# Costava/heightmap-ray-marcher

Hardware: AMD Instinct MI355X
Metric: ray-steps/s at 3840x2160, 4096^2 heightmap (higher is better)
Workload: dtype f64; 1 GPU; C3: 4096x4096 heightmap, 3840x2160, spherical hfov 180, step_dist 0.25, grid_width 1; ray_steps_per_frame=1197030646, rays_per_frame=8294400, hits_per_frame=1006074, parallelism=1 GPU, launches back to back on one stream

## Files before the change

### heightmap-ray-marcher_amd/__init__.py

```python
from .lib import (
    Camera, Config, HmrmError, Scene, SceneParams, Stats,
    Ray, RayHit, TraceParams, SegmentParams, Sun, CellMapParams, CellRect, MAP_TOWARDS_POINT, MAP_WEIGHT, MAP_DIFFUSE, MAP_NO_SHADOWS, RAY_END, TRACE_INTERIOR, SHADE_DIFFUSE, SHADE_NO_SHADOWS, RAY_DTYPE, RAY_HIT_DTYPE, RAY_MISS, RAY_HIT, RAY_CAPPED, MAX_RAYS, as_rays,
    PERSPECTIVE, SPHERICAL, ORTHOGRAPHIC, NEAREST, BILINEAR, NEAREST_F32,
    HMRM_OK, HMRM_E_ARG, HMRM_E_IO, HMRM_E_IMAGE, HMRM_E_CONFIG, HMRM_E_DEVICE, HMRM_E_NOTERM,
    EXPORTED_SYMBOLS, LIB_PATH, NO_PROBE, AA_FACTORS, aa_flags,
    band_local_rows, debug_frame, degrees_to_rads, device_count, image_load, image_load_memory, kernel_src_sha,
    last_error, mip_layout, level_state, calibrate, pick_kernel, plan_order, rcp_error, orbit_camera, orbit_frame_owner, png_encode, record_orbit, record_orbit_multi, record_orbit_shaded, shade_flags, map_flags, render_multi, set_device, write_png, write_ppm,
)
from . import synth
```

### heightmap-ray-marcher_amd/csrc/api.cpp

```cpp
#include <hip/hip_runtime_api.h>

#include <algorithm>
#include <cmath>
#include <cstddef>
#include <cstdio>
#include <cstdlib>
#include <cstring>
#include <fstream>
#include <mutex>
#include <new>
#include <sstream>
#include <string>
#include <vector>

#include "../../include/hmrm.h"
#include "config.hpp"
#include "frame.hpp"
#include "host_pool.hpp"
#include "image_io.hpp"
#include "launch_order.hpp"
#include "render.hpp"

namespace {

thread_local std::string g_error;
thread_local double g_last_kernel_ms = -1.0;

int fail(int code, const std::string &msg) {
	g_error = msg;
	return code;
}

}

namespace hmrm {
int set_error(int code, const char *msg) { return fail(code, msg ? msg : ""); }
}

namespace {

#define HIP_TRY(expr)                                                                         \
	do {                                                                                      \
		hipError_t e_ = (expr);                                                               \
		if (e_ != hipSuccess)                                                                 \
			return fail(HMRM_E_DEVICE, std::string(#expr) + ": " + hipGetErrorString(e_));    \
	} while (0)

struct Knobs {
	int64_t step_cap = (int64_t)1 << 26;
	int kernel = 0;
	bool tile_order = true;
	int order_mode = 2;
	int diag_mode = 0;
	int min_level = -1;
	int finest_pause = -1;
	bool order_verbose = false;
	bool try_group = true;
	int min_plane_shift = 0;
	int seg_n = 0;
	int seg_b[3] = {0, 0, 0}, seg_c[3] = {0, 0, 0};
};

Knobs read_knobs() {
	Knobs k;
	if (const char *s = getenv("HMRM_STEP_CAP")) {
		const long long v = atoll(s);
		if (v > 0) k.step_cap = v > 0x7fffffffLL ? 0x7fffffffLL : (int64_t)v;
	}
	if (const char *s = getenv("HMRM_KERNEL")) k.kernel = strcmp(s, "simple") == 0 ? 2 : (strcmp(s, "group") == 0 ? 1 : (strcmp(s, "rec") == 0 ? 3 : 0));
	if (const char *s = getenv("HMRM_TILE_ORDER")) {
		k.tile_order = s[0] != '0';
		if (s[0] == '1' || s[0] == '2') k.order_mode = s[0] - '0';
	}
	if (const char *s = getenv("HMRM_DIAG_ITERS")) k.diag_mode = atoi(s);
	if (const char *s = getenv("HMRM_ORDER_VERBOSE")) k.order_verbose = s[0] == '1';
	if (const char *s = getenv("HMRM_TRY_GROUP")) k.try_group = s[0] != '0';
	if (const char *s = getenv("HMRM_TILE_SEGMENTS")) {
		int b = 0, c = 0, used = 0;
		while (k.seg_n < 3 && sscanf(s, "%d:%d%n", &b, &c, &used) == 2 && b >= 0 && c > 0) {
			k.seg_b[k.seg_n] = b;
			k.seg_c[k.seg_n] = c;
			++k.seg_n;
			s += used;
			if (*s != ',') break;
			++s;
		}
	}
	if (const char *s = getenv("HMRM_DEBUG_PLANE_SHIFT")) {
		const int v = atoi(s);
		if (v > 0 && v <= 28) k.min_plane_shift = v;
	}
	if (const char *s = getenv("HMRM_MIN_LEVEL"))
		if (s[0] >= '0' && s[0] < '0' + hmrm::kMipLevels) k.min_level = s[0] - '0';
	if (const char *s = getenv("HMRM_FINEST_PAUSE"))
		if (s[0] >= '0' && s[0] <= '9') k.finest_pause = s[0] - '0';
	return k;
}

}

using hmrm::kCostRows;
constexpr int kFrameSlots = 64;
constexpr int kMaxMeasRows = 512;
constexpr int kProbeAfterFrames = 6;
constexpr int kMaxStreamCtx = 32;

struct FrameSlot {
	bool valid = false;
	uint64_t stamp = 0;
	hmrm_camera cam{};
	hmrm_scene_params params{};
	uint64_t thr_max_bits = 0;
	hmrm::DevFrame frame{};
	std::vector<float> row_cost;
	double *d_tables = nullptr;
	double *h_tables = nullptr;
	hipEvent_t uploaded = nullptr;
	hmrm::OrderCalibration cal;
	int meas_rows = 0;
	hipEvent_t measured = nullptr;
};

struct StreamCtx {
	hipStream_t stream = nullptr;
	bool scene_owned = false;
	uint64_t stamp = 0;
	FrameSlot slots[kFrameSlots];
	double *d_arena = nullptr, *h_arena = nullptr;
	double *h_arena_dev = nullptr;
	unsigned long long *d_meas = nullptr, *h_meas = nullptr, *h_meas_dev = nullptr;
	FrameSlot *meas_owner = nullptr;
	size_t arena_n = 0;
	unsigned long long *d_counters = nullptr;
	bool probe_in_flight = false;
	unsigned long long capped_seen = 0;
};

struct RingFrame {
	StreamCtx *ctx = nullptr;
	uint32_t *d_frame = nullptr;
	uint8_t *h_frame = nullptr;
	unsigned long long *h_capped = nullptr;
	size_t px = 0;
	int32_t width = 0, height = 0;
	hipEvent_t kernel_done = nullptr, copy_done = nullptr;
	bool busy = false;
};
constexpr int kMaxRing = 64;
constexpr int kLanes = 3;
struct DevTicket {
	StreamCtx *ctx = nullptr;
	hipEvent_t done = nullptr;
	unsigned long long *h_capped = nullptr;
	bool busy = false;
};

struct hmrm_scene {
	int device = 0;
	int32_t map_w = 0, map_h = 0;
	hmrm_scene_params params{};
	Knobs knobs;
	uint8_t *d_rgb = nullptr;
	uint32_t *d_cmap = nullptr;
	double *d_thr = nullptr;
	float *d_thr32 = nullptr;
	double thr_max = 0.0;
	double thr_max_bil = 0.0;
	bool bil_valid = false;
	bool records_valid = false;
	float *d_mipbuf_bil = nullptr;
	float *d_mipbuf = nullptr;
	hmrm::WindowRecord *d_records = nullptr;
	int32_t mip_w[hmrm::kMipLevels] = {}, mip_h[hmrm::kMipLevels] = {};
	int32_t mip_row = 0, mip_plane_shift = 0;
	size_t mip_floats() const { return (size_t)(hmrm::kMipLevels + 1) << mip_plane_shift; }
	float *plane(float *buf, int l) const { return buf + ((size_t)l << mip_plane_shift); }
	hipStream_t stream = nullptr;
	hipStream_t copy_stream = nullptr;
	hipStream_t lanes[kLanes] = {};
	uint32_t lane_next = 0;
	std::vector<RingFrame *> ring;
	std::vector<DevTicket *> dev_tickets;
	hipEvent_t ev0 = nullptr, ev1 = nullptr;
	unsigned long long *d_maxkey = nullptr;
	uint32_t *d_frame = nullptr;
	size_t frame_px = 0;
	uint8_t *h_stage = nullptr;
	size_t h_stage_bytes = 0;
	uint32_t *d_steps = nullptr;
	double *d_entry = nullptr;
	size_t stats_px = 0;
	hmrm::BatchRay *d_rays = nullptr;
	hmrm::BatchHit *d_hits = nullptr;
	size_t batch_cap = 0;
	uint32_t *d_limits = nullptr;
	size_t limits_cap = 0;
	uint8_t *d_cells = nullptr;
	size_t cells_cap = 0;
	std::mutex mu;
	std::vector<StreamCtx *> ctxs;
	uint64_t clock = 0;
	struct SettledOrder {
		hmrm_camera cam;
		hmrm_scene_params params;
		uint64_t thr_max_bits;
		hmrm::OrderTrial order;
	};
	hmrm::KernelChoice choice;
	bool probe_pending = false;
	uint32_t probe_epoch = 0, probe_epoch_launched = 0;
	int probe_rows = 0;
	StreamCtx *probe_ctx = nullptr;
	hipEvent_t probe_done = nullptr;
	unsigned long long *h_probe = nullptr, *h_probe_dev = nullptr;
	hipEvent_t measure_fence = nullptr;
	StreamCtx *measure_fence_ctx = nullptr;
	std::vector<SettledOrder> settled;
};

static_assert(sizeof(hmrm_ray) == sizeof(hmrm::BatchRay) && sizeof(hmrm_ray_hit) == sizeof(hmrm::BatchHit) &&
                  offsetof(hmrm_ray_hit, entry_d) == offsetof(hmrm::BatchHit, entry_d) &&
                  offsetof(hmrm_ray_hit, steps) == offsetof(hmrm::BatchHit, steps) &&
                  offsetof(hmrm_ray_hit, rgba) == offsetof(hmrm::BatchHit, rgba) &&
                  offsetof(hmrm_ray_hit, status) == offsetof(hmrm::BatchHit, status) && sizeof(hmrm_trace_params) == 16 &&
                  sizeof(hmrm_segment_params) == 24 && offsetof(hmrm_segment_params, flags) == 12 &&
                  offsetof(hmrm_segment_params, max_steps) == 16 && offsetof(hmrm_segment_params, reserved) == 20,
              "the kernels' mirrors of hmrm_ray / hmrm_ray_hit (frame.hpp)");
static_assert(sizeof(hmrm_cell_map_params) == 56 && offsetof(hmrm_cell_map_params, max_steps) == 40 &&
                  offsetof(hmrm_cell_map_params, sampling) == 48 && sizeof(hmrm_cell_rect) == 16 &&
                  HMRM_MAP_TOWARDS_POINT == hmrm::kMapTowardsPoint && HMRM_MAP_WEIGHT == hmrm::kMapWeight &&
                  HMRM_MAP_DIFFUSE == hmrm::kMapDiffuse && HMRM_MAP_NO_SHADOWS == hmrm::kMapNoShadows,
              "hmrm_cell_map_params and the kernels' flag bits (frame.hpp CellRules)");
static_assert(sizeof(hmrm_sun) == 48, "hmrm_sun has padding");
static_assert(sizeof(hmrm_camera) == 3 * sizeof(int32_t) + 4 + 8 * sizeof(double), "hmrm_camera has padding");
static_assert(sizeof(hmrm_scene_params) == 6 * sizeof(double), "hmrm_scene_params has padding");

struct hmrm_config {
	hmrm::Config cfg;
	std::string log_cache, warn_cache;
};

namespace {

void destroy_ctx(StreamCtx *c) {
	if (!c) return;
	for (FrameSlot &sl : c->slots) {
		if (sl.uploaded) (void)hipEventDestroy(sl.uploaded);
		if (sl.measured) (void)hipEventDestroy(sl.measured);
	}
	if (c->d_meas) (void)hipFree(c->d_meas);
	if (c->h_meas) (void)hipHostFree(c->h_meas);
	if (c->d_arena) (void)hipFree(c->d_arena);
	if (c->h_arena) (void)hipHostFree(c->h_arena);
	if (c->d_counters) (void)hipFree(c->d_counters);
	delete c;
}

int ctx_for(hmrm_scene *s, hipStream_t stream, StreamCtx **out) {
	for (StreamCtx *c : s->ctxs)
		if (c->stream == stream) {
			c->stamp = ++s->clock;
			*out = c;
			return HMRM_OK;
		}
	if ((int)s->ctxs.size() >= kMaxStreamCtx) {
		size_t victim = 0;
		for (size_t i = 1; i < s->ctxs.size(); ++i)
			if (!s->ctxs[i]->scene_owned && (victim == 0 || s->ctxs[i]->stamp < s->ctxs[victim]->stamp)) victim = i;
		if (victim == 0) return fail(HMRM_E_ARG, "too many streams");
		(void)hipDeviceSynchronize();
		if (s->probe_ctx == s->ctxs[victim]) s->probe_ctx = nullptr;
		if (s->measure_fence_ctx == s->ctxs[victim]) s->measure_fence_ctx = nullptr;
		destroy_ctx(s->ctxs[victim]);
		s->ctxs.erase(s->ctxs.begin() + (long)victim);
	}
	StreamCtx *c = new (std::nothrow) StreamCtx();
	if (!c) return fail(HMRM_E_ARG, "out of memory");
	c->stream = stream;
	c->scene_owned = stream == s->stream;
	for (hipStream_t lane : s->lanes) c->scene_owned = c->scene_owned || (lane && stream == lane);
	c->stamp = ++s->clock;
	hipError_t e = hipMalloc((void **)&c->d_counters, 16 * sizeof(unsigned long long));
	if (e == hipSuccess) e = hipMemsetAsync(c->d_counters, 0, 16 * sizeof(unsigned long long), s->stream);
	if (e == hipSuccess) e = hipStreamSynchronize(s->stream);
	if (e != hipSuccess) {
		destroy_ctx(c);
		return fail(HMRM_E_DEVICE, std::string("stream context: ") + hipGetErrorString(e));
	}
	s->ctxs.push_back(c);
	*out = c;
	return HMRM_OK;
}

int check_camera(const hmrm_camera *cam) {
	if (!cam) return fail(HMRM_E_ARG, "camera is NULL");
	if (cam->width <= 0 || cam->height <= 0) return fail(HMRM_E_ARG, "resolution must be positive");
	if ((int64_t)cam->width * cam->height > ((int64_t)1 << 31) / 4)
		return fail(HMRM_E_ARG, "resolution too large (the reference indexes the framebuffer with int)");
	if (cam->projection < 1 || cam->projection > 3) return fail(HMRM_E_ARG, "projection must be 1, 2 or 3");
	if (cam->sampling > HMRM_NEAREST_F32) return fail(HMRM_E_ARG, "sampling must be 0 (nearest), 1 (bilinear) or 2 (nearest, float heights)");
	return HMRM_OK;
}

int check_antialias(const hmrm_camera *cam, int32_t factor, hmrm_camera *super, int *shift) {
	const int sh = factor == 1 ? 0 : factor == 2 ? 1 : factor == 4 ? 2 : factor == 8 ? 3 : -1;
	if (sh < 0) return fail(HMRM_E_ARG, "antialias factor must be 1, 2, 4 or 8 (got " + std::to_string(factor) + ")");
	if ((int64_t)cam->width * cam->height * ((int64_t)1 << (2 * sh)) > ((int64_t)1 << 31) / 4)
		return fail(HMRM_E_ARG, "antialias: the " + std::to_string(factor) + "x super frame has more than 2^29 samples (the reference "
		                        "indexes the framebuffer with int)");
	*super = *cam;
	super->width = cam->width << sh;
	super->height = cam->height << sh;
	*shift = sh;
	return HMRM_OK;
}

int antialias_of_flags(uint32_t flags, int32_t *factor) {
	if (flags & ~(HMRM_NO_PROBE | HMRM_AA_MASK))
		return fail(HMRM_E_ARG, "flags: unknown bits (defined: HMRM_NO_PROBE and the antialias factor HMRM_AA(n))");
	const int32_t n = (int32_t)((flags & HMRM_AA_MASK) >> 8);
	*factor = n == 0 ? 1 : n;
	return HMRM_OK;
}

int ensure_bilinear_pyramid(hmrm_scene *s);
int ensure_records(hmrm_scene *s);

void to_host_camera(const hmrm_camera *cam, hmrm::HostCamera *hc) {
	*hc = hmrm::HostCamera{};
	hc->width = cam->width;
	hc->height = cam->height;
	hc->projection = cam->projection;
	hc->bg_r = cam->bg_r;
	hc->bg_g = cam->bg_g;
// ... 41 lines not shown
				for (FrameSlot &sl : c->slots) {
					if (sl.cam.projection == HMRM_SPHERICAL) sl.valid = false;
					sl.d_tables = sl.h_tables = nullptr;
				}
				const size_t per = (n + 31) & ~(size_t)31;
				HIP_TRY(hipMalloc((void **)&c->d_arena, per * kFrameSlots * sizeof(double)));
				HIP_TRY(hipHostMalloc((void **)&c->h_arena, per * kFrameSlots * sizeof(double), hipHostMallocMapped));
				HIP_TRY(hipHostGetDevicePointer((void **)&c->h_arena_dev, c->h_arena, 0));
				c->arena_n = per;
			}
			const size_t idx = (size_t)(slot - c->slots);
			slot->d_tables = c->d_arena + idx * c->arena_n;
			slot->h_tables = c->h_arena + idx * c->arena_n;
			if (!slot->uploaded) HIP_TRY(hipEventCreateWithFlags(&slot->uploaded, hipEventDisableTiming));
			else HIP_TRY(hipEventSynchronize(slot->uploaded));
			cc = slot->h_tables;
			cs = cc + W;
			rs = cs + W;
			rc = rs + H;
		}
		hmrm::DevFrame &fr = slot->frame;
		hmrm::build_frame(hc, s->map_w, s->map_h, s->params.min_height, s->params.max_height, s->params.grid_width,
		                  &fr, nullptr, nullptr, nullptr, nullptr);
		if (cam->projection == HMRM_SPHERICAL) {
			const FrameSlot *row_donor = nullptr, *col_donor = nullptr;
			for (const FrameSlot &o : c->slots) {
				if (!o.valid || &o == slot || o.cam.projection != HMRM_SPHERICAL || !o.h_tables) continue;
				if (o.cam.width != cam->width || o.cam.hfov != cam->hfov) continue;
				if (!col_donor && o.cam.hang == cam->hang) col_donor = &o;
				if (!row_donor && o.cam.height == cam->height && o.cam.vang == cam->vang) row_donor = &o;
			}
			if (col_donor) memcpy(cc, col_donor->h_tables, 2 * W * sizeof(double));
			if (row_donor) memcpy(rs, row_donor->h_tables + 2 * (size_t)row_donor->cam.width, 2 * H * sizeof(double));
			const int nc = col_donor ? 0 : cam->width, nr = row_donor ? 0 : cam->height;
			if (nc + nr > 0)
				hmrm::parallel_ranges(nc + nr, 1024, [&](int b, int e) {
					if (b < nc) hmrm::fill_col_tables(hc, b, std::min(e, nc), cc, cs);
					if (e > nc) hmrm::fill_row_tables(hc, std::max(b, nc) - nc, e - nc, rs, rc);
				});
		}
		slot->row_cost.assign(((size_t)cam->height + kCostRows - 1) / kCostRows, 0.0f);
		hmrm::estimate_row_costs(fr, cc, cs, rs, rc, kCostRows, slot->row_cost.data());
		if (cam->projection == HMRM_SPHERICAL) {
			HIP_TRY(hmrm::launch_upload_tables(c->h_arena_dev + (slot->h_tables - c->h_arena), slot->d_tables, 2 * W + 2 * H, c->stream));
			HIP_TRY(hipEventRecord(slot->uploaded, c->stream));
			fr.col_cos_ha = slot->d_tables;
			fr.col_sin_ha = slot->d_tables + W;
			fr.row_sin_va = slot->d_tables + 2 * W;
			fr.row_cos_va = slot->d_tables + 2 * W + H;
		}
		if (cam->sampling == HMRM_BILINEAR) {
			const int rc2 = ensure_bilinear_pyramid(s);
			if (rc2 != HMRM_OK) return rc2;
		}
		fr.thr_max = cam->sampling == HMRM_BILINEAR ? s->thr_max_bil : s->thr_max;
		fr.min_level = 0;
		while (fr.min_level < hmrm::kMipLevels - 1 && hmrm::win_cells(fr.min_level) < fr.min_window)
			++fr.min_level;
		fr.mipbuf = s->d_mipbuf;
		fr.mipbuf_bil = s->d_mipbuf_bil;
		fr.mip_row = s->mip_row;
		fr.mip_plane_shift = s->mip_plane_shift;
		slot->cam = *cam;
		slot->params = s->params;
		slot->thr_max_bits = thr_bits;
		slot->valid = true;
		for (size_t k = s->settled.size(); k-- > 0;) {
			const hmrm_scene::SettledOrder &so = s->settled[k];
			if (memcmp(&so.cam, cam, sizeof *cam) != 0 || memcmp(&so.params, &s->params, sizeof s->params) != 0 || so.thr_max_bits != thr_bits) continue;
			slot->cal.adopt(so.order);
			break;
		}
	}
	slot->stamp = ++s->clock;
	*f = slot->frame;
	f->step_cap = s->knobs.step_cap;
	f->diag_mode = s->knobs.diag_mode;
	if (s->knobs.min_level >= 0) f->min_level = s->knobs.min_level;
	if (s->knobs.finest_pause >= 0) f->finest_pause = s->knobs.finest_pause;
	if (slot_out) *slot_out = slot;
	return HMRM_OK;
}

int ensure_meas(StreamCtx *c) {
	if (!c->d_meas) HIP_TRY(hipMalloc((void **)&c->d_meas, (size_t)kMaxMeasRows * hmrm::kMeasureStride * sizeof(unsigned long long)));
	if (!c->h_meas) {
		const size_t n = (size_t)kFrameSlots * 2 * kMaxMeasRows * sizeof(unsigned long long);
		HIP_TRY(hipHostMalloc((void **)&c->h_meas, n, hipHostMallocMapped));
		HIP_TRY(hipHostGetDevicePointer((void **)&c->h_meas_dev, c->h_meas, 0));
	}
	return HMRM_OK;
}

bool others_idle(hmrm_scene *s, StreamCtx *c) {
	for (StreamCtx *o : s->ctxs) {
		if (o == c || !o->scene_owned) continue;
		const hipError_t e = hipStreamQuery(o->stream);
		if (e == hipSuccess) continue;
		if (e == hipErrorNotReady) (void)hipGetLastError();
		return false;
	}
	return true;
}

int wait_for_measure_fence(hmrm_scene *s, StreamCtx *c) {
	if (!s->measure_fence_ctx || s->measure_fence_ctx == c) return HMRM_OK;
	if (hipEventQuery(s->measure_fence) == hipSuccess) s->measure_fence_ctx = nullptr;
	else HIP_TRY(hipStreamWaitEvent(c->stream, s->measure_fence, 0));
	return HMRM_OK;
}

int raise_measure_fence(hmrm_scene *s, StreamCtx *c) {
	if (!s->measure_fence) HIP_TRY(hipEventCreateWithFlags(&s->measure_fence, hipEventDisableTiming));
	HIP_TRY(hipEventRecord(s->measure_fence, c->stream));
	s->measure_fence_ctx = c;
	return HMRM_OK;
}

void poll_measured(hmrm_scene *s, StreamCtx *c, FrameSlot *slot, int tiles_y, int rot) {
	if (slot->cal.in_flight >= 0 && slot->meas_rows == tiles_y && hipEventQuery(slot->measured) == hipSuccess) {
		const int trial = slot->cal.in_flight;
		const unsigned long long *h_rec = c->h_meas + (size_t)(slot - c->slots) * 2 * kMaxMeasRows;
		const bool settled = slot->cal.on_measured(h_rec, tiles_y, rot, s->knobs.kernel == 0 && s->knobs.try_group, s->choice);
		if (s->knobs.order_verbose) {
			const hmrm::OrderTrial &t = slot->cal.trials[trial];
			fprintf(stderr, "hmrm order: trial %d of %d tile rows measured, makespan %.1f us:", trial, tiles_y, t.makespan / 100.0);
			for (int k = 0; k < t.n; ++k) fprintf(stderr, " [%d,%d)", t.b[k], t.b[k] + t.c[k]);
			fprintf(stderr, "%s\n", t.group ? " plain groups, rotation" : (t.n ? "" : " rotation"));
			if (settled) fprintf(stderr, "hmrm order: settled on trial %d\n", slot->cal.best);
		}
		if (settled) {
			if (s->settled.size() >= 256) s->settled.erase(s->settled.begin());
			s->settled.push_back(hmrm_scene::SettledOrder{slot->cam, slot->params, slot->thr_max_bits, slot->cal.trials[slot->cal.best]});
		}
	}
	if (c->meas_owner && (c->meas_owner->cal.in_flight < 0 || hipEventQuery(c->meas_owner->measured) == hipSuccess)) c->meas_owner = nullptr;
}

void poll_shadow_probe(hmrm_scene *s) {
	if (!s->probe_pending || hipEventQuery(s->probe_done) != hipSuccess) return;
	s->probe_pending = false;
	if (s->probe_ctx) s->probe_ctx->probe_in_flight = false;
	if (s->probe_epoch_launched != s->probe_epoch) return;
	hmrm::fold_shadow_probe(s->choice, s->h_probe, s->h_probe + 2 * kMaxMeasRows, s->probe_rows);
	if (s->knobs.order_verbose)
		fprintf(stderr, "hmrm probe: production kernel %.1f us, the other kernel %.1f us -> %s\n", hmrm::measured_makespan(s->h_probe, s->probe_rows) / 100.0,
		        hmrm::measured_makespan(s->h_probe + 2 * kMaxMeasRows, s->probe_rows) / 100.0, s->choice.use_group ? (s->choice.with_records ? "groups + window records" : "plain groups") : "production kernel");
}

int launch_shadow_probe(hmrm_scene *s, StreamCtx *c, const hmrm::DevFrame &f, const hmrm::RowMap &rows_in_order, int tiles_y,
                        uint32_t *d_out, int64_t out_stride_px) {
	if (!s->h_probe) {
		HIP_TRY(hipHostMalloc((void **)&s->h_probe, (size_t)4 * kMaxMeasRows * sizeof(unsigned long long), hipHostMallocMapped));
		HIP_TRY(hipHostGetDevicePointer((void **)&s->h_probe_dev, s->h_probe, 0));
		HIP_TRY(hipEventCreateWithFlags(&s->probe_done, hipEventDisableTiming));
	}
	const int rc_m = ensure_meas(c);
	if (rc_m) return rc_m;
	hmrm::RowMap measured = rows_in_order;
	measured.measure = c->d_meas;
	const bool records_ok = f.sampling == 0 && s->d_records;
	s->choice.with_records = records_ok;
	if (records_ok) {
		const int rc_r = ensure_records(s);
		if (rc_r) return rc_r;
	}
	for (int pass = 0; pass < 2; ++pass) {
		HIP_TRY(hmrm::launch_measure_init(measured.measure, tiles_y, c->stream));
		HIP_TRY(hmrm::launch_render_fast(f, measured, s->d_thr, s->d_thr32, s->d_cmap, d_out, out_stride_px,
		                                 c->d_counters + (pass ? 8 : 0), nullptr, nullptr, false,
		                                 pass == 0 ? hmrm::kLeaps : (records_ok ? hmrm::kRecords : hmrm::kPlainGroups), s->d_records, c->stream));
		HIP_TRY(hmrm::launch_measure_readback(measured.measure, s->h_probe_dev + (size_t)pass * 2 * kMaxMeasRows, tiles_y, c->stream));
	}
	HIP_TRY(hipEventRecord(s->probe_done, c->stream));
	s->probe_pending = true;
	s->choice.probed = true;
	s->probe_rows = tiles_y;
	s->probe_epoch_launched = s->probe_epoch;
	s->probe_ctx = c;
	c->probe_in_flight = true;
	return raise_measure_fence(s, c);
}

struct LitFrame {
	hmrm::SunRules sun;
	bool primary_interior;
	uint32_t shade_flags;
};
hmrm::SunRules shade_sun(const LitFrame &lit) {
	hmrm::SunRules sun = lit.sun;
	if (!(lit.shade_flags & HMRM_SHADE_DIFFUSE)) sun.ambient = 255u;
	return sun;
}
int launch_kernel(hmrm_scene *s, StreamCtx *c, const hmrm::DevFrame &f, const hmrm::RowMap &rows_in_order, uint32_t *d_out,
                  int64_t out_stride_px, uint32_t *d_steps, double *d_entry, bool stats, bool use_group, bool interior = false,
                  const LitFrame *lit = nullptr) {
	const bool huge_side = s->map_w >= (1 << 24) || s->map_h >= (1 << 24);
	if (huge_side && f.sampling != 0)
		return fail(HMRM_E_ARG, "maps with a side of 2^24 cells or more support nearest sampling only");
	if ((s->knobs.kernel == 2 || huge_side) && f.sampling == 0) {
		if (lit && lit->shade_flags) {
			const bool shadows = !(lit->shade_flags & HMRM_SHADE_NO_SHADOWS);
			if (f.aa_shift) {
				HIP_TRY(hmrm::launch_render_shaded_literal_aa(f, rows_in_order, s->d_thr, s->d_cmap, d_out, out_stride_px, c->d_counters,
				                                              shadows ? lit->sun : shade_sun(*lit), lit->primary_interior, shadows, c->stream));
				return HMRM_OK;
			}
			HIP_TRY(hmrm::launch_render_shaded_literal(f, rows_in_order, s->d_thr, s->d_cmap, d_out, out_stride_px, c->d_counters,
			                                           shadows ? lit->sun : shade_sun(*lit), lit->primary_interior, shadows, c->stream));
			return HMRM_OK;
		}
		if (lit && f.aa_shift) {
			HIP_TRY(hmrm::launch_render_lit_literal_aa(f, rows_in_order, s->d_thr, s->d_cmap, d_out, out_stride_px, c->d_counters, lit->sun,
			                                           lit->primary_interior, c->stream));
			return HMRM_OK;
		}
		if (lit) {
			HIP_TRY(hmrm::launch_render_lit_literal(f, rows_in_order, s->d_thr, s->d_cmap, d_out, out_stride_px, c->d_counters, lit->sun,
			                                        lit->primary_interior, c->stream));
			return HMRM_OK;
		}
		if (interior) {
			HIP_TRY(hmrm::launch_render_interior_literal(f, rows_in_order, s->d_thr, s->d_cmap, d_out, out_stride_px, c->d_counters, c->stream));
			return HMRM_OK;
		}
		HIP_TRY(hmrm::launch_render(f, rows_in_order, s->d_thr, s->d_cmap, d_out, out_stride_px, c->d_counters, d_steps,
		                            d_entry, stats, c->stream));
	} else {
		const hmrm::FastKernel k = (hmrm::FastKernel)hmrm::pick_fast_kernel(s->knobs.kernel, use_group, f.sampling == 0 && s->d_records, s->choice);
		if (k == hmrm::kRecords) {
			const int rc_r = ensure_records(s);
			if (rc_r) return rc_r;
		}
		if (lit && f.aa_shift) {
			const auto launch = (lit->shade_flags & HMRM_SHADE_NO_SHADOWS) ? hmrm::launch_render_shaded_aa
			                    : lit->shade_flags                         ? hmrm::launch_render_lit_shaded_aa
			                                                               : hmrm::launch_render_lit_aa;
			HIP_TRY(launch(f, rows_in_order, s->d_thr, s->d_thr32, s->d_cmap, d_out, out_stride_px, c->d_counters, k, s->d_records,
			               (lit->shade_flags & HMRM_SHADE_NO_SHADOWS) ? shade_sun(*lit) : lit->sun, lit->primary_interior, c->stream));
			return HMRM_OK;
		}
		if (lit && (lit->shade_flags & HMRM_SHADE_NO_SHADOWS)) {
			HIP_TRY(hmrm::launch_render_shaded(f, rows_in_order, s->d_thr, s->d_thr32, s->d_cmap, d_out, out_stride_px, c->d_counters, k,
			                                   s->d_records, shade_sun(*lit), lit->primary_interior, c->stream));
			return HMRM_OK;
		}
		if (lit && lit->shade_flags) {
			HIP_TRY(hmrm::launch_render_lit_shaded(f, rows_in_order, s->d_thr, s->d_thr32, s->d_cmap, d_out, out_stride_px, c->d_counters, k,
			                                       s->d_records, lit->sun, lit->primary_interior, c->stream));
			return HMRM_OK;
		}
		if (lit) {
			HIP_TRY(hmrm::launch_render_lit(f, rows_in_order, s->d_thr, s->d_thr32, s->d_cmap, d_out, out_stride_px, c->d_counters, k,
			                                s->d_records, lit->sun, lit->primary_interior, c->stream));
			return HMRM_OK;
		}
		if (interior) {
			HIP_TRY(hmrm::launch_render_interior(f, rows_in_order, s->d_thr, s->d_thr32, s->d_cmap, d_out, out_stride_px, c->d_counters, k,
			                                     s->d_records, c->stream));
			return HMRM_OK;
		}
		HIP_TRY(hmrm::launch_render_fast(f, rows_in_order, s->d_thr, s->d_thr32, s->d_cmap, d_out, out_stride_px,
		                                 c->d_counters, d_steps, d_entry, stats, k, s->d_records, c->stream));
	}
	return HMRM_OK;
}

int launch_maybe_measured(hmrm_scene *s, StreamCtx *c, const hmrm::DevFrame &f, FrameSlot *slot, hmrm::RowMap &rows_in_order, int tiles_y,
                          bool measure_now, uint32_t *d_out, int64_t out_stride_px, uint32_t *d_steps, double *d_entry, bool stats, bool use_group,
                          bool interior = false, const LitFrame *lit = nullptr) {
	if (measure_now) {
		const int rc_m = ensure_meas(c);
		if (rc_m) return rc_m;
		if (!slot->measured) HIP_TRY(hipEventCreateWithFlags(&slot->measured, hipEventDisableTiming));
		rows_in_order.measure = c->d_meas;
		HIP_TRY(hmrm::launch_measure_init(rows_in_order.measure, tiles_y, c->stream));
	}
	const int rc_k = launch_kernel(s, c, f, rows_in_order, d_out, out_stride_px, d_steps, d_entry, stats, use_group, interior, lit);
	if (rc_k || !measure_now) return rc_k;
	const size_t idx = (size_t)(slot - c->slots);
	HIP_TRY(hmrm::launch_measure_readback(rows_in_order.measure, c->h_meas_dev + idx * 2 * kMaxMeasRows, tiles_y, c->stream));
	HIP_TRY(hipEventRecord(slot->measured, c->stream));
	slot->meas_rows = tiles_y;
	c->meas_owner = slot;
	return raise_measure_fence(s, c);
}

int launch_frame(hmrm_scene *s, StreamCtx *c, const hmrm::DevFrame &f, FrameSlot *slot, const hmrm::RowMap &rows,
                 uint32_t *d_out, int64_t out_stride_px, uint32_t *d_steps, double *d_entry, bool stats, bool no_probe = false,
                 int interior = 0, const LitFrame *lit = nullptr) {
	hmrm::RowMap rows_in_order = rows;
	int tile_w = 1, tile_h = 1;
	hmrm::render_tile_shape(&tile_w, &tile_h);
	const int tiles_y = (rows.local_rows + tile_h - 1) / tile_h;
	const bool pieces = s->knobs.seg_n > 0 && rows.band_rows == 0 && rows.row_begin == 0;
	const int rot = hmrm::choose_tile_rot(s->knobs.tile_order, slot->row_cost, rows, tile_h);
	const bool may_probe = !stats && !interior && !lit && s->knobs.kernel == 0 && s->knobs.try_group;
	const bool eligible = !pieces && !stats && !interior && !lit && s->knobs.tile_order && s->knobs.order_mode == 2 && s->knobs.kernel != 2 &&
	                      rows.band_rows == 0 && rows.row_begin == 0 && rows.local_rows == f.screen_h && tiles_y >= 12 &&
	                      tiles_y <= kMaxMeasRows && s->map_w < (1 << 24) && s->map_h < (1 << 24);
	int rc = wait_for_measure_fence(s, c);
	if (rc) return rc;
	poll_shadow_probe(s);
	hmrm::OrderTrial order;
	if (pieces) {
		order.n = s->knobs.seg_n;
		for (int k = 0; k < 3; ++k) { order.b[k] = s->knobs.seg_b[k]; order.c[k] = s->knobs.seg_c[k]; }
	}
	bool use_group = may_probe && s->choice.use_group;
	if (interior || lit) use_group = s->knobs.kernel == 0 && s->knobs.try_group && s->choice.use_group;
	bool measure_now = false;
	if (eligible) {
		poll_measured(s, c, slot, tiles_y, rot);
		const bool probe_open = may_probe && !no_probe && !s->choice.probed && !s->probe_pending;
		const bool quiet = (slot->cal.wants_measure() || probe_open) && c->meas_owner == nullptr && !c->probe_in_flight && others_idle(s, c);
		const hmrm::LaunchPlan p = slot->cal.plan(quiet, s->choice);
		order = slot->cal.trials[p.trial];
		use_group = p.use_group;
		measure_now = p.measure;
		if (!measure_now && probe_open && quiet && slot->cal.in_flight < 0 && ++s->choice.unprobed_frames >= (unsigned)kProbeAfterFrames) {
			hmrm::set_tile_order(&rows_in_order, tiles_y, rot, order.n, order.b, order.c);
			return launch_shadow_probe(s, c, f, rows_in_order, tiles_y, d_out, out_stride_px);
		}
	}
	hmrm::set_tile_order(&rows_in_order, tiles_y, rot, order.n, order.b, order.c);
	if ((rc = launch_maybe_measured(s, c, f, slot, rows_in_order, tiles_y, measure_now, d_out, out_stride_px, d_steps, d_entry, stats, use_group, interior == 2, lit))) {
		if (measure_now) slot->cal.drop_in_flight();
		return rc;
	}
	return HMRM_OK;
}

bool mip_layout(int32_t map_w, int32_t map_h, int32_t *mip_w, int32_t *mip_h, int32_t *mip_row, int32_t *plane_shift, int32_t min_shift = 0) {
	for (int l = 0; l < hmrm::kMipLevels; ++l) {
		const int stride = 1 << hmrm::mip_stride_shift(l);
		mip_w[l] = (map_w + stride - 1) / stride;
		mip_h[l] = (map_h + stride - 1) / stride;
	}
	*mip_row = mip_w[0];
	*plane_shift = min_shift;
	while (((size_t)1 << *plane_shift) < (size_t)hmrm::mip_index(mip_w[0] - 1, mip_h[0] - 1, *mip_row) + 1) ++*plane_shift;
	return ((uint64_t)(hmrm::kMipLevels + 1) << *plane_shift) <= ((uint64_t)1 << 30);
}

int next_lane(hmrm_scene *s, StreamCtx **out) {
	const uint32_t i = s->lane_next++ % kLanes;
	if (!s->lanes[i]) HIP_TRY(hipStreamCreateWithFlags(&s->lanes[i], hipStreamNonBlocking));
	return ctx_for(s, s->lanes[i], out);
}

int ensure_frame(hmrm_scene *s, size_t px) {
	if (px <= s->frame_px) return HMRM_OK;
	if (s->d_frame) (void)hipFree(s->d_frame);
	s->d_frame = nullptr;
	s->frame_px = 0;
	HIP_TRY(hipMalloc((void **)&s->d_frame, px * sizeof(uint32_t)));
	s->frame_px = px;
	return HMRM_OK;
}

int ensure_stats(hmrm_scene *s, size_t px) {
	if (px <= s->stats_px) return HMRM_OK;
	if (s->d_steps) (void)hipFree(s->d_steps);
	if (s->d_entry) (void)hipFree(s->d_entry);
	s->d_steps = nullptr;
	s->d_entry = nullptr;
	s->stats_px = 0;
	HIP_TRY(hipMalloc((void **)&s->d_steps, px * sizeof(uint32_t)));
	HIP_TRY(hipMalloc((void **)&s->d_entry, px * sizeof(double)));
	s->stats_px = px;
	return HMRM_OK;
}

int ensure_records(hmrm_scene *s) {
	if (s->records_valid) return HMRM_OK;
	if (!s->d_records) return fail(HMRM_E_ARG, "this scene has no window records");
	HIP_TRY(hmrm::launch_build_records(s->d_thr, s->map_w, s->map_h, s->d_records, s->stream));
	HIP_TRY(hipStreamSynchronize(s->stream));
	s->records_valid = true;
	return HMRM_OK;
}

int ensure_bilinear_pyramid(hmrm_scene *s) {
	if (s->bil_valid) return HMRM_OK;
	const int64_t n = (int64_t)s->map_w * s->map_h;
	if (!s->d_mipbuf_bil) HIP_TRY(hipMalloc((void **)&s->d_mipbuf_bil, s->mip_floats() * sizeof(float)));
	double *tmp = nullptr;
	HIP_TRY(hipMalloc((void **)&tmp, (size_t)n * sizeof(double)));
	hipError_t e = hmrm::launch_dilate3x3(s->d_thr, s->map_w, s->map_h, tmp, s->stream);
	if (e == hipSuccess)
		e = hmrm::launch_build_mip0(tmp, s->map_w, s->map_h, s->plane(s->d_mipbuf_bil, 0), s->mip_w[0], s->mip_h[0],
		                            s->mip_row, s->stream);
	for (int l = 1; l < hmrm::kMipLevels && e == hipSuccess; ++l)
		e = hmrm::launch_build_mip_up(s->plane(s->d_mipbuf_bil, l - 1), s->mip_w[l - 1], s->mip_h[l - 1],
		                              s->plane(s->d_mipbuf_bil, l), s->mip_w[l], s->mip_h[l], s->mip_row, l - 1, s->stream);
	const int top = hmrm::kMipLevels - 1;
	const size_t top_span = (size_t)hmrm::mip_index(s->mip_w[top] - 1, s->mip_h[top] - 1, s->mip_row) + 1;
	std::vector<float> coarse(top_span);
	if (e == hipSuccess)
		e = hipMemcpyAsync(coarse.data(), s->plane(s->d_mipbuf_bil, top), top_span * sizeof(float), hipMemcpyDeviceToHost, s->stream);
	if (e == hipSuccess) e = hipStreamSynchronize(s->stream);
	(void)hipFree(tmp);
	if (e != hipSuccess) return fail(HMRM_E_DEVICE, std::string("bilinear pyramid: ") + hipGetErrorString(e));
	float m = -__builtin_huge_valf();
	for (int iy = 0; iy < s->mip_h[top]; ++iy)
		for (int ix = 0; ix < s->mip_w[top]; ++ix) {
			const float v = coarse[hmrm::mip_index(ix, iy, s->mip_row)];
			if (v > m) m = v;
		}
	e = hipMemcpyAsync(s->plane(s->d_mipbuf_bil, hmrm::kMipLevels), &m, sizeof m, hipMemcpyHostToDevice, s->stream);
	if (e == hipSuccess) e = hipStreamSynchronize(s->stream);
	if (e != hipSuccess) return fail(HMRM_E_DEVICE, std::string("bilinear pyramid: ") + hipGetErrorString(e));
	s->thr_max_bil = (double)m;
	s->bil_valid = true;
	return HMRM_OK;
}

int run_update_heights(hmrm_scene *s) {
	const int64_t n = (int64_t)s->map_w * s->map_h;
	for (StreamCtx *c : s->ctxs)
		if (c->scene_owned && c->stream != s->stream) HIP_TRY(hipStreamSynchronize(c->stream));
	if (s->copy_stream) HIP_TRY(hipStreamSynchronize(s->copy_stream));
	HIP_TRY(hipMemsetAsync(s->d_maxkey, 0, sizeof(unsigned long long), s->stream));
	HIP_TRY(hmrm::launch_prepare_heights(s->d_rgb, s->d_thr, n, s->params.lum_r, s->params.lum_g,
	                                     s->params.lum_b, s->params.min_height, s->params.max_height,
	                                     false, s->d_maxkey, s->stream));
	HIP_TRY(hmrm::launch_thr_to_float(s->d_thr, s->d_thr32, n, s->stream));
	HIP_TRY(hmrm::launch_build_mip0(s->d_thr, s->map_w, s->map_h, s->plane(s->d_mipbuf, 0), s->mip_w[0], s->mip_h[0],
	                                s->mip_row, s->stream));
	for (int l = 1; l < hmrm::kMipLevels; ++l)
		HIP_TRY(hmrm::launch_build_mip_up(s->plane(s->d_mipbuf, l - 1), s->mip_w[l - 1], s->mip_h[l - 1],
		                                  s->plane(s->d_mipbuf, l), s->mip_w[l], s->mip_h[l], s->mip_row, l - 1, s->stream));
	s->bil_valid = false;
	s->records_valid = false;
	for (StreamCtx *c : s->ctxs)
		for (FrameSlot &sl : c->slots) sl.valid = false;
	s->settled.clear();
	s->choice.reset();
	++s->probe_epoch;
	unsigned long long key = 0;
	HIP_TRY(hipMemcpyAsync(&key, s->d_maxkey, sizeof key, hipMemcpyDeviceToHost, s->stream));
	HIP_TRY(hipStreamSynchronize(s->stream));
	s->thr_max = key ? hmrm::max_key_to_double(key) : -__builtin_huge_val();
	const float top = hmrm::round_up_to_float_host(s->thr_max);
	HIP_TRY(hipMemcpyAsync(s->plane(s->d_mipbuf, hmrm::kMipLevels), &top, sizeof top, hipMemcpyHostToDevice, s->stream));
	HIP_TRY(hipStreamSynchronize(s->stream));
	return HMRM_OK;
}

constexpr int64_t kMaxBatch = (int64_t)1 << 29;
int noterm(unsigned long long capped);

int check_trace(const hmrm_trace_params *p, const void *rays, int64_t n, const void *hits) {
	if (n < 0) return fail(HMRM_E_ARG, "trace: n must not be negative (got " + std::to_string(n) + ")");
	if (n > kMaxBatch) return fail(HMRM_E_ARG, "trace: at most 2^29 rays per batch (got " + std::to_string(n) + ")");
	if (n > 0 && (!p || !rays || !hits)) return fail(HMRM_E_ARG, "trace: NULL params, rays or hits");
	if (p && p->sampling > HMRM_NEAREST_F32)
		return fail(HMRM_E_ARG, "trace: sampling must be 0 (nearest), 1 (bilinear) or 2 (nearest, float heights)");
	return HMRM_OK;
}

int check_segments(const hmrm_segment_params *p, const void *rays, int64_t n, const void *hits, hmrm_trace_params *plain) {
	if (p) *plain = hmrm_trace_params{p->step_dist, p->bg_r, p->bg_g, p->bg_b, p->sampling};
	const int rc = check_trace(p ? plain : nullptr, rays, n, hits);
	if (rc) return rc;
	if (p && (p->flags & ~(uint32_t)HMRM_TRACE_INTERIOR)) return fail(HMRM_E_ARG, "trace: unknown flag bits (defined: HMRM_TRACE_INTERIOR)");
	if (p && p->reserved != 0u) return fail(HMRM_E_ARG, "trace: hmrm_segment_params.reserved must be 0");
	return HMRM_OK;
}

int ensure_limits(hmrm_scene *s, size_t n) {
	if (n <= s->limits_cap) return HMRM_OK;
	if (s->d_limits) (void)hipFree(s->d_limits);
	s->d_limits = nullptr;
	s->limits_cap = 0;
	HIP_TRY(hipMalloc((void **)&s->d_limits, n * sizeof(uint32_t)));
	s->limits_cap = n;
	return HMRM_OK;
}

int ensure_batch(hmrm_scene *s, size_t n) {
	if (n <= s->batch_cap) return HMRM_OK;
	if (s->d_rays) (void)hipFree(s->d_rays);
	if (s->d_hits) (void)hipFree(s->d_hits);
	s->d_rays = nullptr;
	s->d_hits = nullptr;
	s->batch_cap = 0;
	HIP_TRY(hipMalloc((void **)&s->d_rays, n * sizeof(hmrm::BatchRay)));
	HIP_TRY(hipMalloc((void **)&s->d_hits, n * sizeof(hmrm::BatchHit)));
	s->batch_cap = n;
	return HMRM_OK;
}

int cameraless_frame(hmrm_scene *s, double step_dist, int sampling, hmrm::DevFrame *out) {
	const bool huge_side = s->map_w >= (1 << 24) || s->map_h >= (1 << 24);
	if (huge_side && sampling != 0) return fail(HMRM_E_ARG, "maps with a side of 2^24 cells or more support nearest sampling only");
	if (sampling == HMRM_BILINEAR) {
		const int rc_b = ensure_bilinear_pyramid(s);
		if (rc_b) return rc_b;
	}
	hmrm::DevFrame f = hmrm::DevFrame();
	hmrm::fill_scene_fields(s->map_w, s->map_h, s->params.min_height, s->params.max_height, s->params.grid_width, step_dist, &f);
	f.bg[3] = 255;
	f.sampling = sampling;
	f.thr_max = sampling == HMRM_BILINEAR ? s->thr_max_bil : s->thr_max;
	f.mipbuf = s->d_mipbuf;
	f.mipbuf_bil = s->d_mipbuf_bil;
	f.mip_row = s->mip_row;
	f.mip_plane_shift = s->mip_plane_shift;
	f.step_cap = s->knobs.step_cap;
	f.min_window = 4;
	f.min_level = s->knobs.min_level >= 0 ? s->knobs.min_level : 0;
	f.finest_pause = s->knobs.finest_pause >= 0 ? s->knobs.finest_pause : 0;
	*out = f;
	return HMRM_OK;
}
int cameraless_kernel(hmrm_scene *s, int sampling, bool *literal, hmrm::FastKernel *k) {
	const bool huge_side = s->map_w >= (1 << 24) || s->map_h >= (1 << 24);
	*literal = (s->knobs.kernel == 2 || huge_side) && sampling == 0;
	*k = hmrm::kLeaps;
// ... 147 lines not shown
	s->params = *params;
	s->knobs = read_knobs();
	int rc = HMRM_OK;
	auto body = [&]() -> int {
		HIP_TRY(hipGetDevice(&s->device));
		HIP_TRY(hipStreamCreateWithFlags(&s->stream, hipStreamNonBlocking));
		HIP_TRY(hipStreamCreateWithFlags(&s->copy_stream, hipStreamNonBlocking));
		HIP_TRY(hipEventCreate(&s->ev0));
		HIP_TRY(hipEventCreate(&s->ev1));
		HIP_TRY(hipMalloc((void **)&s->d_rgb, n * 3));
		HIP_TRY(hipMalloc((void **)&s->d_cmap, n * 4));
		HIP_TRY(hipMalloc((void **)&s->d_thr, n * (sizeof(double) + sizeof(float))));
		s->d_thr32 = reinterpret_cast<float *>(s->d_thr + n);
		(void)mip_layout(map_w, map_h, s->mip_w, s->mip_h, &s->mip_row, &s->mip_plane_shift, s->knobs.min_plane_shift);
		HIP_TRY(hipMalloc((void **)&s->d_mipbuf, s->mip_floats() * sizeof(float)));
		if ((map_h + 3) / 4 <= 65535 * 16)
			HIP_TRY(hipMalloc((void **)&s->d_records, (size_t)hmrm::rec_row(map_w) * (size_t)((map_h + 3) / 4) * sizeof(hmrm::WindowRecord)));
		HIP_TRY(hipMalloc((void **)&s->d_maxkey, sizeof(unsigned long long)));
		HIP_TRY(hipMemcpyAsync(s->d_rgb, height_rgb, n * 3, hipMemcpyHostToDevice, s->stream));
		HIP_TRY(hipMemcpyAsync(s->d_cmap, color_rgba, n * 4, hipMemcpyHostToDevice, s->stream));
		StreamCtx *own = nullptr;
		const int rc2 = ctx_for(s, s->stream, &own);
		if (rc2) return rc2;
		return run_update_heights(s);
	};
	rc = body();
	if (rc != HMRM_OK) {
		std::string keep = g_error;
		hmrm_scene_destroy(s);
		g_error = keep;
		return rc;
	}
	*out = s;
	return HMRM_OK;
}

int hmrm_scene_update(hmrm_scene *s, const hmrm_scene_params *params) {
	if (!s || !params) return fail(HMRM_E_ARG, "NULL argument");
	HIP_TRY(hipSetDevice(s->device));
	std::lock_guard<std::mutex> lk(s->mu);
	s->params = *params;
	return run_update_heights(s);
}

void hmrm_scene_destroy(hmrm_scene *s) {
	if (!s) return;
	(void)hipSetDevice(s->device);
	for (StreamCtx *c : s->ctxs) {
		if (c->scene_owned && c->stream) (void)hipStreamSynchronize(c->stream);
		destroy_ctx(c);
	}
	s->ctxs.clear();
	if (s->copy_stream) (void)hipStreamSynchronize(s->copy_stream);
	for (RingFrame *r : s->ring) {
		if (r->d_frame) (void)hipFree(r->d_frame);
		if (r->h_frame) (void)hipHostFree(r->h_frame);
		if (r->h_capped) (void)hipHostFree(r->h_capped);
		if (r->kernel_done) (void)hipEventDestroy(r->kernel_done);
		if (r->copy_done) (void)hipEventDestroy(r->copy_done);
		delete r;
	}
	s->ring.clear();
	for (DevTicket *t : s->dev_tickets) {
		if (t->done) (void)hipEventDestroy(t->done);
		if (t->h_capped) (void)hipHostFree(t->h_capped);
		delete t;
	}
	s->dev_tickets.clear();
	for (hipStream_t &lane : s->lanes)
		if (lane) {
			(void)hipStreamDestroy(lane);
			lane = nullptr;
		}
	if (s->copy_stream) (void)hipStreamDestroy(s->copy_stream);
	if (s->d_rgb) (void)hipFree(s->d_rgb);
	if (s->d_cmap) (void)hipFree(s->d_cmap);
	if (s->d_thr) (void)hipFree(s->d_thr);
	if (s->d_mipbuf) (void)hipFree(s->d_mipbuf);
	if (s->d_records) (void)hipFree(s->d_records);
	if (s->d_mipbuf_bil) (void)hipFree(s->d_mipbuf_bil);
	if (s->d_maxkey) (void)hipFree(s->d_maxkey);
	if (s->d_frame) (void)hipFree(s->d_frame);
	if (s->h_stage) (void)hipHostFree(s->h_stage);
	if (s->h_probe) (void)hipHostFree(s->h_probe);
	if (s->probe_done) (void)hipEventDestroy(s->probe_done);
	if (s->measure_fence) (void)hipEventDestroy(s->measure_fence);
	if (s->d_steps) (void)hipFree(s->d_steps);
	if (s->d_entry) (void)hipFree(s->d_entry);
	if (s->d_rays) (void)hipFree(s->d_rays);
	if (s->d_hits) (void)hipFree(s->d_hits);
	if (s->d_limits) (void)hipFree(s->d_limits);
	if (s->d_cells) (void)hipFree(s->d_cells);
	if (s->ev0) (void)hipEventDestroy(s->ev0);
	if (s->ev1) (void)hipEventDestroy(s->ev1);
	if (s->stream) (void)hipStreamDestroy(s->stream);
	delete s;
}

int hmrm_debug_kernel_choice(const hmrm_scene *s) {
	if (!s) return fail(HMRM_E_ARG, "NULL argument");
	std::lock_guard<std::mutex> lk(const_cast<hmrm_scene *>(s)->mu);
	if (s->knobs.kernel != 0) return s->knobs.kernel;
	return s->choice.use_group ? (s->choice.with_records ? 3 : 1) : 0;
}

int hmrm_debug_reload_env(hmrm_scene *s) {
	if (!s) return fail(HMRM_E_ARG, "NULL argument");
	HIP_TRY(hipSetDevice(s->device));
	std::lock_guard<std::mutex> lk(s->mu);
	s->knobs = read_knobs();
	s->settled.clear();
	s->choice.reset();
	++s->probe_epoch;
	for (StreamCtx *c : s->ctxs)
		for (FrameSlot &sl : c->slots) {
			if (sl.cal.in_flight >= 0 && sl.measured) HIP_TRY(hipEventSynchronize(sl.measured));
			sl.cal.reset();
			if (c->meas_owner == &sl) c->meas_owner = nullptr;
		}
	return HMRM_OK;
}

int hmrm_scene_read_heights(const hmrm_scene *cs, double *out) {
	hmrm_scene *s = const_cast<hmrm_scene *>(cs);
	if (!s || !out) return fail(HMRM_E_ARG, "NULL argument");
	HIP_TRY(hipSetDevice(s->device));
	const int64_t n = (int64_t)s->map_w * s->map_h;
	double *tmp = nullptr;
	HIP_TRY(hipMalloc((void **)&tmp, (size_t)n * sizeof(double)));
	hipError_t e = hmrm::launch_prepare_heights(s->d_rgb, tmp, n, s->params.lum_r, s->params.lum_g,
	                                            s->params.lum_b, s->params.min_height,
	                                            s->params.max_height, true, nullptr, s->stream);
	if (e == hipSuccess)
		e = hipMemcpyAsync(out, tmp, (size_t)n * sizeof(double), hipMemcpyDeviceToHost, s->stream);
	if (e == hipSuccess) e = hipStreamSynchronize(s->stream);
	(void)hipFree(tmp);
	if (e != hipSuccess) return fail(HMRM_E_DEVICE, std::string("read_heights: ") + hipGetErrorString(e));
	return HMRM_OK;
}

static int render_common(hmrm_scene *s, const hmrm_camera *cam, uint8_t *rgba, size_t stride_bytes,
                         hmrm_stats *stats, uint32_t *steps_pp, double *entry_d, bool want_stats, int32_t aa_factor = 1,
                         bool interior = false, const LitFrame *lit = nullptr) {
	int rc = check_camera(cam);
	if (rc) return rc;
	hmrm_camera super;
	int aa_shift = 0;
	if ((rc = check_antialias(cam, aa_factor, &super, &aa_shift))) return rc;
	if (!s || !rgba) return fail(HMRM_E_ARG, "NULL argument");
	const size_t W = (size_t)cam->width, H = (size_t)cam->height;
	if (stride_bytes < W * 4) return fail(HMRM_E_ARG, "stride_bytes < width*4");
	HIP_TRY(hipSetDevice(s->device));
	std::lock_guard<std::mutex> lk(s->mu);
	if ((rc = ensure_frame(s, W * H))) return rc;
	if (want_stats && aa_shift == 0 && (rc = ensure_stats(s, W * H))) return rc;
	StreamCtx *c = nullptr;
	if ((rc = ctx_for(s, s->stream, &c))) return rc;
	hmrm::DevFrame f;
	FrameSlot *slot = nullptr;
	if ((rc = prepare_frame(s, c, &super, &f, &slot))) return rc;
	f.aa_shift = aa_shift;
	hmrm::RowMap rows{0, super.height, 0, 0, 1, {}, {}, nullptr};
	int interior_mode = 0;
	if (interior) {
		const double *o = f.cam;
		const bool cam_inside = f.c0[0] < o[0] && o[0] < f.c1[0] && f.c1[1] < o[1] && o[1] < f.c0[1] && f.c0[2] < o[2] && o[2] < f.c1[2];
		interior_mode = (cam->projection == HMRM_ORTHOGRAPHIC || cam_inside) ? 2 : 1;
	}
	if (want_stats) {
		HIP_TRY(hipMemsetAsync(c->d_counters, 0, 2 * sizeof(unsigned long long), s->stream));
		HIP_TRY(hipMemsetAsync(c->d_counters + 4, 0, 4 * sizeof(unsigned long long), s->stream));
	}
	HIP_TRY(hipEventRecord(s->ev0, s->stream));
	const bool per_pixel = want_stats && aa_shift == 0;
	if ((rc = launch_frame(s, c, f, slot, rows, s->d_frame, (int64_t)W, per_pixel ? s->d_steps : nullptr,
	                       per_pixel ? s->d_entry : nullptr, want_stats, false, interior_mode, lit)))
		return rc;
	HIP_TRY(hipEventRecord(s->ev1, s->stream));
	HIP_TRY(hipMemcpy2DAsync(rgba, stride_bytes, s->d_frame, W * 4, W * 4, H, hipMemcpyDeviceToHost,
	                         s->stream));
	unsigned long long counters[8] = {0, 0, 0, 0, 0, 0, 0, 0};
	HIP_TRY(hipMemcpyAsync(counters, c->d_counters, sizeof counters, hipMemcpyDeviceToHost, s->stream));
	if (per_pixel && steps_pp)
		HIP_TRY(hipMemcpyAsync(steps_pp, s->d_steps, W * H * sizeof(uint32_t), hipMemcpyDeviceToHost, s->stream));
	if (per_pixel && entry_d)
		HIP_TRY(hipMemcpyAsync(entry_d, s->d_entry, W * H * sizeof(double), hipMemcpyDeviceToHost, s->stream));
	HIP_TRY(hipStreamSynchronize(s->stream));
	float ms = 0.f;
	HIP_TRY(hipEventElapsedTime(&ms, s->ev0, s->ev1));
	g_last_kernel_ms = ms;
	const unsigned long long capped = counters[2] - c->capped_seen;
	c->capped_seen = counters[2];
	if (stats) {
		stats->rays = (uint64_t)super.width * (uint64_t)super.height;
		stats->steps = counters[0];
		stats->hits = counters[1];
		stats->capped = capped;
		stats->leap_attempts = counters[4];
		stats->leaps = counters[5];
		stats->groups = counters[6];
		stats->leaped_steps = counters[7];
	}
// ... 773 lines not shown
	if (rc) return rc;
	if (!s) return fail(HMRM_E_ARG, "NULL argument");
	hmrm_cell_rect r;
	if ((rc = check_cell_rect(s, rect, stride_bytes, &r))) return rc;
	HIP_TRY(hipSetDevice(s->device));
	std::lock_guard<std::mutex> lk(s->mu);
	StreamCtx *c = nullptr;
	if ((rc = ctx_for(s, (hipStream_t)hip_stream, &c))) return rc;
	return launch_cells(s, c, p, r, static_cast<uint8_t *>(d_out), stride_bytes);
}

int hmrm_pick(const hmrm_scene *scene, const hmrm_camera *cam, int32_t px, int32_t py, hmrm_ray_hit *hit) {
	hmrm_scene *s = const_cast<hmrm_scene *>(scene);
	int rc = check_camera(cam);
	if (rc) return rc;
	if (!s || !hit) return fail(HMRM_E_ARG, "NULL argument");
	if (px < 0 || py < 0 || px >= cam->width || py >= cam->height) return fail(HMRM_E_ARG, "pixel out of range");
	HIP_TRY(hipSetDevice(s->device));
	std::lock_guard<std::mutex> lk(s->mu);
	const size_t W = (size_t)cam->width, H = (size_t)cam->height;
	const bool spherical = cam->projection == HMRM_SPHERICAL;
	if ((rc = ensure_stats(s, 8 + (spherical ? 2 * W + 2 * H : 0)))) return rc;
	if ((rc = ensure_batch(s, 1))) return rc;
	StreamCtx *c = nullptr;
	if ((rc = ctx_for(s, s->stream, &c))) return rc;
	hmrm::HostCamera hc;
	to_host_camera(cam, &hc);
	std::vector<double> tables(spherical ? 2 * W + 2 * H : 0);
	double *t = tables.data();
	hmrm::DevFrame f;
	hmrm::build_frame(hc, s->map_w, s->map_h, s->params.min_height, s->params.max_height, s->params.grid_width, &f,
	                  spherical ? t : nullptr, spherical ? t + W : nullptr, spherical ? t + 2 * W : nullptr,
	                  spherical ? t + 2 * W + H : nullptr);
	if (spherical) {
		double *d_t = s->d_entry + 8;
		HIP_TRY(hipMemcpyAsync(d_t, t, tables.size() * sizeof(double), hipMemcpyHostToDevice, s->stream));
		f.col_cos_ha = d_t;
		f.col_sin_ha = d_t + W;
		f.row_sin_va = d_t + 2 * W;
		f.row_cos_va = d_t + 2 * W + H;
	}
	HIP_TRY(hmrm::launch_probe(f, px, py, s->d_entry, s->stream));
	const uint8_t bg[3] = {cam->bg_r, cam->bg_g, cam->bg_b};
	if ((rc = launch_batch(s, c, cam->step_dist, bg, cam->sampling, reinterpret_cast<const hmrm::BatchRay *>(s->d_entry), 1, s->d_hits)))
		return rc;
	return finish_batch(s, c, hit, 1, nullptr);
}

int hmrm_debug_ray(const hmrm_scene *scene, const hmrm_camera *cam, int32_t px, int32_t py,
                   double pos[3], double dir[3], double *entry_d) {
	hmrm_scene *s = const_cast<hmrm_scene *>(scene);
	int rc = check_camera(cam);
	if (rc) return rc;
	if (!s || !pos || !dir || !entry_d) return fail(HMRM_E_ARG, "NULL argument");
	if (px < 0 || py < 0 || px >= cam->width || py >= cam->height) return fail(HMRM_E_ARG, "pixel out of range");
	HIP_TRY(hipSetDevice(s->device));
	std::lock_guard<std::mutex> lk(s->mu);
	if ((rc = ensure_stats(s, 8))) return rc;
	StreamCtx *c = nullptr;
	if ((rc = ctx_for(s, s->stream, &c))) return rc;
	hmrm::DevFrame f;
	if ((rc = prepare_frame(s, c, cam, &f, nullptr))) return rc;
	HIP_TRY(hmrm::launch_probe(f, px, py, s->d_entry, s->stream));
	double host[7];
	HIP_TRY(hipMemcpyAsync(host, s->d_entry, sizeof host, hipMemcpyDeviceToHost, s->stream));
	HIP_TRY(hipStreamSynchronize(s->stream));
	for (int i = 0; i < 3; ++i) { pos[i] = host[i]; dir[i] = host[3 + i]; }
	*entry_d = host[6];
	return HMRM_OK;
}

int hmrm_debug_plan_order(const uint64_t *records, int32_t tile_rows, int32_t rot, int32_t pieces_begin[3],
                          int32_t pieces_count[3], int32_t *tile_row_of_grid_row) {
	if (!records || !pieces_begin || !pieces_count || tile_rows <= 0 || rot < 0 || rot >= tile_rows) return fail(HMRM_E_ARG, "bad argument");
	int b[3] = {0, 0, 0}, c[3] = {0, 0, 0};
	const int n = hmrm::plan_order_from_measurement((const unsigned long long *)records, tile_rows, rot, b, c);
	for (int k = 0; k < 3; ++k) {
		pieces_begin[k] = k < n ? b[k] : 0;
		pieces_count[k] = k < n ? c[k] : 0;
	}
	if (tile_row_of_grid_row) {
		hmrm::RowMap r{};
		hmrm::set_tile_order(&r, tile_rows, rot, n, b, c);
		for (int gy = 0; gy < tile_rows; ++gy) {
			int delta = r.seg_delta[0];
			for (int k = 1; k < hmrm::kOrderSegs; ++k) delta = (unsigned)gy >= (unsigned)r.seg_first[k - 1] ? r.seg_delta[k] : delta;
			unsigned ty = (unsigned)gy + (unsigned)delta;
			if (ty >= (unsigned)tile_rows) ty -= (unsigned)tile_rows;
			tile_row_of_grid_row[gy] = (int32_t)ty;
		}
	}
	return n;
}

int hmrm_debug_rcp_error(int32_t mode, uint64_t count, uint64_t seed, int32_t exp_lo, int32_t exp_hi,
                         double *max_rel_err, uint64_t *hist64) {
	if (!max_rel_err) return fail(HMRM_E_ARG, "NULL argument");
	if (mode < 0 || mode > 2 || count == 0 || count > ((uint64_t)1 << 40) || exp_lo > exp_hi || exp_lo < -1000 || exp_hi > 1000)
		return fail(HMRM_E_ARG, "hmrm_debug_rcp_error: bad mode, count or exponent range");
	unsigned long long *d = nullptr, host[65] = {};
	HIP_TRY(hipMalloc((void **)&d, sizeof host));
	hipError_t e = hipMemset(d, 0, sizeof host);
	if (e == hipSuccess) e = hmrm::launch_rcp_error(mode, count, seed, exp_lo, exp_hi, d, nullptr);
	if (e == hipSuccess) e = hipMemcpy(host, d, sizeof host, hipMemcpyDeviceToHost);
	(void)hipFree(d);
	if (e != hipSuccess) return fail(HMRM_E_DEVICE, std::string("rcp probe: ") + hipGetErrorString(e));
	memcpy(max_rel_err, &host[0], sizeof(double));
	if (hist64)
		for (int i = 0; i < 64; ++i) hist64[i] = host[1 + i];
	return HMRM_OK;
}

int hmrm_debug_frame(const hmrm_camera *cam, const hmrm_scene_params *params, int32_t map_w,
                     int32_t map_h, double *out25, double *tables) {
	int rc = check_camera(cam);
	if (rc) return rc;
	if (!params || !out25) return fail(HMRM_E_ARG, "NULL argument");
	if (cam->projection == HMRM_SPHERICAL && !tables) return fail(HMRM_E_ARG, "tables required for spherical");
	hmrm::HostCamera hc{};
	hc.width = cam->width; hc.height = cam->height; hc.projection = cam->projection;
	hc.bg_r = cam->bg_r; hc.bg_g = cam->bg_g; hc.bg_b = cam->bg_b; hc.sampling = cam->sampling;
	hc.hfov = cam->hfov; hc.hang = cam->hang; hc.vang = cam->vang;
	hc.pos[0] = cam->pos[0]; hc.pos[1] = cam->pos[1]; hc.pos[2] = cam->pos[2];
	hc.ortho_width = cam->ortho_width; hc.step_dist = cam->step_dist;
	const size_t W = (size_t)cam->width, H = (size_t)cam->height;
	hmrm::DevFrame f;
	hmrm::build_frame(hc, map_w, map_h, params->min_height, params->max_height, params->grid_width, &f, nullptr, nullptr,
	                  nullptr, nullptr);
	if (cam->projection == HMRM_SPHERICAL) {
		double *cc = tables, *cs = tables + W, *rs = tables + 2 * W, *rc2 = tables + 2 * W + H;
		const int nc = cam->width, nr = cam->height;
		hmrm::parallel_ranges(nc + nr, 1024, [&](int b, int e) {
			if (b < nc) hmrm::fill_col_tables(hc, b, std::min(e, nc), cc, cs);
			if (e > nc) hmrm::fill_row_tables(hc, std::max(b, nc) - nc, e - nc, rs, rc2);
		});
	}
	double *o = out25;
	for (int i = 0; i < 3; ++i) *o++ = f.cam[i];
	for (int i = 0; i < 3; ++i) *o++ = f.upper_left[i];
	for (int i = 0; i < 3; ++i) *o++ = f.plane_right[i];
	for (int i = 0; i < 3; ++i) *o++ = f.plane_down[i];
	for (int i = 0; i < 3; ++i) *o++ = f.look[i];
	for (int i = 0; i < 3; ++i) *o++ = f.c0[i];
	for (int i = 0; i < 3; ++i) *o++ = f.c1[i];
	*o++ = f.nudge;
	*o++ = f.step_dist;
	*o++ = (double)f.grid_pow2;
	*o++ = f.inv_grid_width;
	return HMRM_OK;
}

int hmrm_debug_mip_layout(int32_t map_w, int32_t map_h, int32_t *mip_row, int32_t *plane_shift, int32_t *levels) {
	if (map_w <= 0 || map_h <= 0 || (int64_t)map_w * map_h > ((int64_t)1 << 31) / 4) return fail(HMRM_E_ARG, "bad map dimensions");
	int32_t w[hmrm::kMipLevels], h[hmrm::kMipLevels], row = 0, shift = 0;
	const bool fits = mip_layout(map_w, map_h, w, h, &row, &shift);
	if (mip_row) *mip_row = row;
	if (plane_shift) *plane_shift = shift;
	if (levels) *levels = hmrm::kMipLevels;
	return fits ? 1 : 0;
}

int hmrm_debug_pick_kernel(int32_t forced, int32_t use_other, int32_t records_ok, int32_t scene_verdict, int32_t scene_with_records,
                           int32_t *with_records_after) {
	hmrm::KernelChoice choice;
	choice.use_group = scene_verdict != 0;
	choice.probed = choice.use_group;
	choice.with_records = scene_with_records != 0;
	const int k = hmrm::pick_fast_kernel(forced, use_other != 0, records_ok != 0, choice);
	if (with_records_after) *with_records_after = choice.with_records ? 1 : 0;
	return k;
}

int hmrm_debug_read_records(const hmrm_scene *cs, void *records_out, double *thr_out) {
	hmrm_scene *s = const_cast<hmrm_scene *>(cs);
	if (!s) return fail(HMRM_E_ARG, "NULL argument");
	std::lock_guard<std::mutex> lk(s->mu);
	HIP_TRY(hipSetDevice(s->device));
	HIP_TRY(hipStreamSynchronize(s->stream));
	if (records_out) {
		if (!s->d_records) return fail(HMRM_E_ARG, "this scene has no window records (map too tall)");
		const int rc_r = ensure_records(s);
		if (rc_r) return rc_r;
		HIP_TRY(hipMemcpy(records_out, s->d_records, (size_t)hmrm::rec_row(s->map_w) * (size_t)((s->map_h + 3) / 4) * sizeof(hmrm::WindowRecord),
		                  hipMemcpyDeviceToHost));
	}
	if (thr_out) HIP_TRY(hipMemcpy(thr_out, s->d_thr, (size_t)s->map_w * (size_t)s->map_h * sizeof(double), hipMemcpyDeviceToHost));
	return HMRM_OK;
}

int hmrm_debug_level_state(int32_t level, int32_t young, int32_t min_level, int32_t out[8]) {
	if (!out || level < 0 || level > hmrm::kMipLevels || min_level < 0 || min_level >= hmrm::kMipLevels)
		return fail(HMRM_E_ARG, "hmrm_debug_level_state: bad argument");
	const uint32_t b = (uint32_t)(hmrm::level_state_table() >> (8 * level)) & 0xffu;
	const int hs = (int)(b & 31u), back = (int)(b >> 5);
	const int lstep = hmrm::level_step(young ? 0 : -1);
	out[0] = hs;
	out[1] = back;
	out[2] = (back + 1) << hs;
	out[3] = lstep;
	out[4] = hmrm::level_coarser(level, lstep);
	out[5] = hmrm::level_finer(level, lstep, min_level);
	out[6] = level == min_level ? 1 : 0;
	out[7] = (int32_t)b;
	return hmrm::kMipLevels;
}

int hmrm_debug_calibrate(const uint64_t *records, int32_t launches, int32_t tile_rows, int32_t rot, int32_t may_probe,
                         int32_t scene_already_probed, const uint8_t *can_measure, int32_t *trial_used, int32_t *measured,
                         int32_t *group_kernel, int32_t *n_trials, int32_t *best, int32_t *scene_use_group, int32_t *settled_at_launch) {
	if (!records || launches <= 0 || tile_rows <= 0 || tile_rows > kMaxMeasRows || rot < 0 || rot >= tile_rows)
		return fail(HMRM_E_ARG, "hmrm_debug_calibrate: bad argument");
	hmrm::OrderCalibration cal;
	hmrm::KernelChoice choice;
	choice.probed = scene_already_probed != 0;
	int settled_at = -1;
	for (int32_t i = 0; i < launches; ++i) {
		const hmrm::LaunchPlan p = cal.plan(!can_measure || can_measure[i] != 0, choice);
		if (trial_used) trial_used[i] = p.trial;
		if (measured) measured[i] = p.measure ? 1 : 0;
		if (group_kernel) group_kernel[i] = p.use_group ? 1 : 0;
		if (p.measure && cal.on_measured((const unsigned long long *)records + (size_t)i * 2 * (size_t)tile_rows, tile_rows, rot, may_probe != 0, choice))
			settled_at = i;
	}
	if (n_trials) *n_trials = cal.n_trials;
	if (best) *best = cal.best;
	if (scene_use_group) *scene_use_group = choice.use_group ? 1 : 0;
	if (settled_at_launch) *settled_at_launch = settled_at;
	return HMRM_OK;
}

int32_t hmrm_band_local_rows(int32_t height, int32_t band_rows, int32_t band_index, int32_t band_count) {
	if (height <= 0 || band_rows <= 0 || band_count <= 0 || band_index < 0 || band_index >= band_count) return 0;
	int64_t local = 0;
	for (int64_t b = band_index; b * band_rows < height; b += band_count) local += band_rows;
	return (int32_t)local;
}

}

namespace hmrm {
int check_shaded_args(const hmrm_sun *sun, uint32_t shade_flags) { return check_shaded(sun, shade_flags); }
}
```

### heightmap-ray-marcher_amd/csrc/device_common.hpp

```cpp
#pragma once
#include <hip/hip_runtime.h>
#include <stdint.h>

#include "frame.hpp"

#pragma clang fp contract(off)

namespace hmrm {

struct DevRay {
	double px, py, pz;
	double dx, dy, dz;
};

template <int PROJ>
__device__ __forceinline__ DevRay make_ray(const DevFrame &f, int px, int py) {
	DevRay r;
	if (PROJ == 2) {
		const double sva = f.row_sin_va[py], cva = f.row_cos_va[py];
		const double cha = f.col_cos_ha[px], sha = f.col_sin_ha[px];
		r.px = f.cam[0]; r.py = f.cam[1]; r.pz = f.cam[2];
		r.dx = sva * cha;
		r.dy = sva * sha;
		r.dz = cva;
// ... 200 lines not shown
	if (PROJ == 1 || PROJ == 2) {
#pragma unroll
		for (int i = 0; i < 3; ++i) {
			if (!f.box_side_known[i]) continue;
			const uint32_t hd = (uint32_t)((unsigned long long)__double_as_longlong(rd[i]) >> 32);
			away = away | ((((hd >> 20) & 0x7ffu) - 523u) < 1000u & ((f.box_side[i] ^ hd) >> 31) != 0u);
		}
		return away;
	}
#pragma unroll
	for (int i = 0; i < 3; ++i) {
		const uint32_t h0 = (uint32_t)((unsigned long long)__double_as_longlong(f.c0[i] - ro[i]) >> 32);
		const uint32_t h1 = (uint32_t)((unsigned long long)__double_as_longlong(f.c1[i] - ro[i]) >> 32);
		const uint32_t hd = (uint32_t)((unsigned long long)__double_as_longlong(rd[i]) >> 32);
		const bool moderate = (((h0 >> 20) & 0x7ffu) - 523u) < 1000u && (((h1 >> 20) & 0x7ffu) - 523u) < 1000u &&
		                      (((hd >> 20) & 0x7ffu) - 523u) < 1000u;
		away = away || (moderate && ((h0 ^ h1) >> 31) == 0u && ((h0 ^ hd) >> 31) != 0u);
	}
	return away;
}

__device__ __forceinline__ uint32_t pack_rgba(uint32_t r, uint32_t g, uint32_t b) {
	return r | (g << 8) | (b << 16) | 0xff000000u;
}

__device__ __forceinline__ uint32_t sky_channel_literal(double v) {
	if (v < 0.0) v = 0.0;
	else if (v > 255.0) v = 255.0;
	return (uint32_t)(int)__builtin_floor(v);
}
__device__ __forceinline__ uint32_t sky_channel(double v) {
	return (uint32_t)__builtin_fmin(v, 255.0);
}

struct StatsOut {
	unsigned long long *counters;
	uint32_t *steps_per_pixel;
	double *entry_d;
};


__device__ __forceinline__ uint32_t shade_miss(const DevFrame &f, double dz) {
	if (dz > 0.0) {
		const double zz = dz * dz;
		const double r_ = 220.0 * zz + (double)f.bg[0];
		const double g_ = 240.0 * zz + (double)f.bg[1];
		const double b_ = 255.0 * dz + (double)f.bg[2];
		return pack_rgba(sky_channel(r_), sky_channel(g_), sky_channel(b_));
	}
	return pack_rgba(f.bg[0], f.bg[1], f.bg[2]);
}

__device__ __forceinline__ uint32_t shade_hit(const DevFrame &f, uint32_t texel) {
	return ((texel >> 24) == 0) ? pack_rgba(f.bg[0], f.bg[1], f.bg[2]) : (texel | 0xff000000u);
}

#ifndef HMRM_WAVE_W
#define HMRM_WAVE_W 8
#endif
#ifndef HMRM_WAVES_X
#define HMRM_WAVES_X 1
#endif
#ifndef HMRM_WAVES_Y
#define HMRM_WAVES_Y 2
#endif
constexpr int kWaveW = HMRM_WAVE_W, kWaveH = 64 / HMRM_WAVE_W;
constexpr int kWavesX = HMRM_WAVES_X, kWavesY = HMRM_WAVES_Y;
constexpr int kBlockThreads = 64 * kWavesX * kWavesY;
constexpr int kTileW = kWavesX * kWaveW, kTileH = kWavesY * kWaveH;
static_assert(kBatchW == kWaveW, "a wave's 64 lanes hold 64 consecutive rays of a batch (frame.hpp RayBatch)");
struct PixelId {
	int px, py, lrow;
	int tile_y;
	bool live;
};
__device__ __forceinline__ int frame_row_of(const RowMap &rows, int lrow) {
	if (rows.band_rows > 0) {
		const int band = lrow / rows.band_rows, within = lrow - band * rows.band_rows;
		return (rows.band_index + band * rows.band_count) * rows.band_rows + within;
	}
	return rows.row_begin + lrow;
}

__device__ __forceinline__ PixelId pixel_of_tile_lane(const DevFrame &f, const RowMap &rows, int tiles_y, int tile_x, unsigned gy,
                                                      int wave, int lane) {
	const bool row_exists = gy < (unsigned)tiles_y;
	int delta = rows.seg_delta[0];
#pragma unroll
	for (int k = 1; k < kOrderSegs; ++k) delta = gy >= (unsigned)rows.seg_first[k - 1] ? rows.seg_delta[k] : delta;
	unsigned ty = gy + (unsigned)delta;
	if (ty >= (unsigned)tiles_y) ty -= (unsigned)tiles_y;
	const int tile_y = (int)ty;
	PixelId p;
	p.tile_y = row_exists ? tile_y : -1;
	p.px = tile_x * kTileW + (wave % kWavesX) * kWaveW + (lane % kWaveW);
	p.lrow = tile_y * kTileH + (wave / kWavesX) * kWaveH + (lane / kWaveW);
	p.py = frame_row_of(rows, p.lrow);
	p.live = row_exists && p.px < f.screen_w && p.lrow < rows.local_rows && p.py < f.screen_h;
	return p;
}
__device__ __forceinline__ PixelId pixel_of_lane(const DevFrame &f, const RowMap &rows, int tiles_y) {
	return pixel_of_tile_lane(f, rows, tiles_y, (int)blockIdx.x, blockIdx.z * 32768u + blockIdx.y, (int)(threadIdx.x >> 6),
	                          (int)(threadIdx.x & 63));
}

template <bool STATS>
__device__ __forceinline__ void publish_counters(const StatsOut &st, unsigned long long steps,
                                                 uint32_t hit, uint32_t cap) {
	if (STATS) {
		unsigned long long s = steps, h = hit, c = cap;
		for (int off = 32; off > 0; off >>= 1) {
			s += __shfl_xor(s, off);
			h += __shfl_xor(h, off);
			c += __shfl_xor(c, off);
		}
		if ((threadIdx.x & 63) == 0) {
			if (s) atomicAdd(&st.counters[0], s);
			if (h) atomicAdd(&st.counters[1], h);
			if (c) atomicAdd(&st.counters[2], c);
		}
	} else if (cap) {
		atomicAdd(&st.counters[2], 1ull);
	}
}

__device__ __forceinline__ void store_box_filtered(uint32_t *__restrict__ out, int64_t out_stride_px, int shift, int lane,
                                                   int px, int lrow, bool live, uint32_t rgba) {
	static_assert(kWaveW == 8 && kWaveH == 8, "an n x n block (n <= 8) must lie inside one wave's pixels");
	uint32_t rb = rgba & 0x00ff00ffu, g = (rgba >> 8) & 0xffu;
#pragma unroll
	for (int k = 0; k < 3; ++k) {
		if (shift > k) {
			rb += (uint32_t)__shfl_xor((int)rb, 1 << k);
			g += (uint32_t)__shfl_xor((int)g, 1 << k);
		}
	}
#pragma unroll
	for (int k = 0; k < 3; ++k) {
		if (shift > k) {
			rb += (uint32_t)__shfl_xor((int)rb, kWaveW << k);
			g += (uint32_t)__shfl_xor((int)g, kWaveW << k);
		}
	}
	const int s2 = 2 * shift;
	const uint32_t half = (1u << s2) >> 1;
	const uint32_t r = ((rb & 0xffffu) + half) >> s2, b = ((rb >> 16) + half) >> s2, gg = (g + half) >> s2;
	const int corner = ((1 << shift) - 1) * (kWaveW + 1);
	if (live && (lane & corner) == 0)
		out[(uint64_t)(uint32_t)(lrow >> shift) * (uint64_t)out_stride_px + (uint32_t)(px >> shift)] = pack_rgba(r, gg, b);
}

}
```

### heightmap-ray-marcher_amd/csrc/frame.hpp

```cpp
#pragma once
#include <stdint.h>

namespace hmrm {

struct DevFrame {
	int32_t screen_w, screen_h;
	int32_t projection;
	int32_t map_w, map_h;
	uint8_t bg[4];
	double cam[3];
	double upper_left[3], plane_right[3], plane_down[3];
	double look[3];
	const double *col_cos_ha, *col_sin_ha;
	const double *row_sin_va, *row_cos_va;
	double c0[3], c1[3];
	double grid_width;
	double nudge;
	double step_dist;
	double inv_grid_width;
	int32_t grid_pow2;
	int32_t grid_mode;
	double thr_max;
	int64_t step_cap;
	const float *mipbuf;
	const float *mipbuf_bil;
	int32_t mip_row;
	int32_t mip_plane_shift;
	uint32_t box_side[3];
	int32_t box_side_known[3];
	int32_t diag_mode;
	int32_t sampling;
	int32_t min_level;
	int32_t min_window;
	int32_t finest_pause;
	int32_t aa_shift;
};

#ifndef HMRM_LEVEL_STEP
#define HMRM_LEVEL_STEP 1
#endif
constexpr int kLevelStep = HMRM_LEVEL_STEP;
#ifndef HMRM_MIP_LEVELS
#define HMRM_MIP_LEVELS (HMRM_LEVEL_STEP == 2 ? 4 : 7)
#endif
constexpr int kMipLevels = HMRM_MIP_LEVELS;
#ifndef HMRM_DENSE_FROM
#define HMRM_DENSE_FROM 1
#endif
constexpr int kDenseFrom = HMRM_DENSE_FROM;
#if defined(__HIPCC__)
__host__ __device__
#endif
constexpr int win_strides(int l) { return l < kDenseFrom ? 2 : 4; }
#if defined(__HIPCC__)
__host__ __device__
#endif
constexpr int win_cells(int l) { return 4 << (kLevelStep * l); }
#if defined(__HIPCC__)
__host__ __device__
#endif
constexpr int mip_stride_shift(int l) { return kLevelStep * l + (l < kDenseFrom ? 1 : 0); }
#if defined(__HIPCC__)
__host__ __device__
#endif
constexpr uint32_t level_state_byte(int l) {
	return l >= kMipLevels ? (28u | (3u << 5)) : ((uint32_t)mip_stride_shift(l) | ((uint32_t)(win_strides(l) - 1) << 5));
}
#if defined(__HIPCC__)
__host__ __device__
#endif
constexpr uint64_t level_state_table() {
	uint64_t k = 0;
	for (int l = 0; l <= kMipLevels; ++l) k |= (uint64_t)level_state_byte(l) << (8 * l);
	return k;
}
static_assert(kMipLevels + 1 <= 8 && mip_stride_shift(kMipLevels - 1) < 28, "level state: one byte per level, eight levels");
constexpr bool level_state_table_ok() {
	for (int l = 0; l <= kMipLevels; ++l) {
		const uint32_t b = (uint32_t)(level_state_table() >> (8 * l)) & 0xffu;
		const int hs = (int)(b & 31u), back = (int)(b >> 5);
		if (l < kMipLevels && (hs != mip_stride_shift(l) || back + 1 != win_strides(l) || ((back + 1) << hs) != win_cells(l))) return false;
		if (l == kMipLevels && (hs != 28 || ((back + 1) << hs) != (1 << 30))) return false;
	}
	return true;
}
static_assert(level_state_table_ok(), "level state bytes disagree with win_strides / win_cells / mip_stride_shift");

#ifndef HMRM_ADAPT_AFTER
#define HMRM_ADAPT_AFTER 8
#endif
constexpr int kAdaptAfter = (kLevelStep == 1) ? HMRM_ADAPT_AFTER : 0;
constexpr bool kAdaptive = kAdaptAfter > 0;
#if defined(__HIPCC__)
__host__ __device__
#endif
constexpr int level_step(int young_left) { return kAdaptive ? 2 + (young_left >> 31) : 1; }
#if defined(__HIPCC__)
__host__ __device__
#endif
constexpr int level_coarser(int lev, int lstep) { return lev + lstep > kMipLevels - 1 ? kMipLevels - 1 : lev + lstep; }
#if defined(__HIPCC__)
__host__ __device__
#endif
constexpr int level_finer(int lev, int drop, int minlev) {
	return lev == kMipLevels ? kMipLevels - 1 : (lev - drop > minlev ? lev - drop : minlev);
}
#if defined(__HIPCC__)
__host__ __device__
#endif
inline unsigned mip_index(int ix, int iy, int pitch) { return (unsigned)(iy * pitch + ix); }

constexpr int kRecLevel = 2;
constexpr int kRecCells = 8;
struct WindowRecord {
	float max2;
	uint32_t spare0;
	uint32_t xs[2], ys[2];
	uint32_t spare1[2];
};
static_assert(sizeof(WindowRecord) == 32, "two 16-byte loads");
static_assert(kRecLevel >= kDenseFrom && kLevelStep == 1, "the record level's windows: 16 cells, every 4");
#if defined(__HIPCC__)
__host__ __device__
#endif
inline int rec_row(int map_w) { return (map_w + 3) >> 2; }

struct RowMap {
	int32_t row_begin;
	int32_t local_rows;
	int32_t band_rows;
	int32_t band_index, band_count;
	int32_t seg_first[3];
	int32_t seg_delta[4];
	unsigned long long *measure;
};
constexpr int kMeasureStride = 33;
constexpr int kOrderSegs = 4;

static_assert(sizeof(DevFrame) == 352,"DevFrame must not grow");

struct BatchRay { double pos[3], dir[3]; };
struct BatchHit {
	double point[3];
	double entry_d;
	uint32_t steps;
	int32_t cell_x, cell_y;
	uint8_t rgba[4];
	uint32_t status;
	uint32_t reserved;
};
static_assert(sizeof(BatchRay) == 48 && sizeof(BatchHit) == 56, "hmrm_ray / hmrm_ray_hit");
struct RayBatch {
	const BatchRay *rays;
	BatchHit *hits;
	int64_t n;
};
constexpr int kBatchW = 8;

struct SegRules {
	const uint32_t *max_steps;
	uint32_t limit;
	uint32_t interior;
};

struct SunRules {
	double dir[3];
	double step_dist;
	uint32_t max_steps;
	uint32_t ambient;
};

struct CellRules {
	double target[3];
	double lift;
	int32_t x0, y0;
	uint32_t max_steps;
	uint32_t flags;
	uint32_t ambient;
};
constexpr uint32_t kMapTowardsPoint = 1u, kMapWeight = 2u, kMapDiffuse = 4u, kMapNoShadows = 8u;

struct HostCamera {
	int32_t width, height, projection;
	uint8_t bg_r, bg_g, bg_b, sampling;
	double hfov, hang, vang, pos[3], ortho_width, step_dist;
};

void build_frame(const HostCamera &cam, int32_t map_w, int32_t map_h,
                 double min_height, double max_height, double grid_width,
                 DevFrame *out,
                 double *col_cos_ha, double *col_sin_ha,
                 double *row_sin_va, double *row_cos_va);

void fill_scene_fields(int32_t map_w, int32_t map_h, double min_height, double max_height, double grid_width,
                       double step_dist, DevFrame *out);

void fill_col_tables(const HostCamera &cam, int32_t begin, int32_t end, double *col_cos_ha, double *col_sin_ha);
void fill_row_tables(const HostCamera &cam, int32_t begin, int32_t end, double *row_sin_va, double *row_cos_va);

void estimate_row_costs(const DevFrame &f, const double *col_cos_ha, const double *col_sin_ha,
                        const double *row_sin_va, const double *row_cos_va, int rows_per_sample, float *out);

}
```

### heightmap-ray-marcher_amd/csrc/launch_order.cpp

```cpp
#include "launch_order.hpp"

#include <algorithm>

namespace hmrm {

int choose_tile_rot(bool enabled, const std::vector<float> &row_cost, const RowMap &rows, int tile_h) {
	if (!enabled || rows.band_rows > 0 || row_cost.empty()) return 0;
	const int tiles_y = (rows.local_rows + tile_h - 1) / tile_h;
	if (tiles_y <= 1) return 0;
	auto tile_cost = [&](int t) {
		float c = 0.0f;
		const int r0 = rows.row_begin + t * tile_h, r1 = r0 + tile_h - 1;
		for (int k = r0 / kCostRows; k <= r1 / kCostRows && k < (int)row_cost.size(); ++k)
			if (row_cost[(size_t)k] > c) c = row_cost[(size_t)k];
		return c;
	};
	float top = 0.0f;
	for (int t = 0; t < tiles_y; ++t) top = std::max(top, tile_cost(t));
	if (!(top > 0.0f)) return 0;
	for (int t = 0; t < tiles_y; ++t)
		if (tile_cost(t) >= 0.1f * top) return t;
	return 0;
}

// ... 40 lines not shown
		qmax = std::max(qmax, q[(size_t)i]);
	}
	for (int i = 0; i + 1 < N; ++i) D[(size_t)i] = st[(size_t)i + 1] - st[(size_t)i];
	D[(size_t)N - 1] = N > 1 ? D[(size_t)N - 2] : 0.0;
	int n = 0;
	for (int i = 0; i < N - rot; ++i)
		if (q[(size_t)i] >= 0.05 * qmax) n = i + 1;
	if (n < 12) return 0;
	std::vector<double> cum((size_t)n + 1, 0.0), g((size_t)n), g2((size_t)n), pm((size_t)n + 1, 0.0), sm((size_t)n + 1, -1e300),
	    pm2((size_t)n + 1, 0.0), sm2((size_t)n + 1, -1e300);
	double floor_ms = 0.0;
	for (int i = n; i < N; ++i) floor_ms = std::max(floor_ms, st[(size_t)i] + q[(size_t)i]);
	double span = floor_ms;
	for (int i = 0; i < n; ++i) span = std::max(span, st[(size_t)i] + q[(size_t)i]);
	for (int i = 0; i < n; ++i) {
		cum[(size_t)i + 1] = cum[(size_t)i] + D[(size_t)i];
		g[(size_t)i] = cum[(size_t)i] + q[(size_t)i];
		g2[(size_t)i] = q[(size_t)i] >= 0.85 * span ? -1e300 : g[(size_t)i];
		pm[(size_t)i + 1] = std::max(pm[(size_t)i], g[(size_t)i]);
		pm2[(size_t)i + 1] = std::max(pm2[(size_t)i], g2[(size_t)i]);
	}
	for (int i = n - 1; i >= 0; --i) {
		sm[(size_t)i] = std::max(sm[(size_t)i + 1], g[(size_t)i]);
		sm2[(size_t)i] = std::max(sm2[(size_t)i + 1], g2[(size_t)i]);
	}
	const double base = std::max(pm[(size_t)n], floor_ms), base2 = std::max(pm2[(size_t)n], 0.0);
	double best2 = base2;
	int best_a = 0, best_b = 0;
	const int step = std::max(1, n / 96);
	for (int a = 0; a < n; a += step) {
		double mid = -1e300, mid2 = -1e300;
		int scanned = a;
		for (int b2 = a + step; b2 < n; b2 += step) {
			for (; scanned < b2; ++scanned) {
				mid = std::max(mid, g[(size_t)scanned]);
				mid2 = std::max(mid2, g2[(size_t)scanned]);
			}
			const double shift_tail = cum[(size_t)a] - cum[(size_t)b2], shift_mid = cum[(size_t)n] - cum[(size_t)b2];
			const double m1 = std::max(std::max(pm[(size_t)a], sm[(size_t)b2] + shift_tail), std::max(mid + shift_mid, floor_ms));
			if (m1 > 1.001 * base) continue;
			const double m2 = std::max(pm2[(size_t)a], std::max(sm2[(size_t)b2] + shift_tail, mid2 + shift_mid));
			if (m2 < best2) {
				best2 = m2;
				best_a = a;
				best_b = b2;
			}
		}
	}
	if (!(best2 < 0.95 * base2) || best_b <= best_a) return 0;
	int k = 0;
	if (best_a > 0) { pb[k] = rot; pc[k] = best_a; ++k; }
	pb[k] = rot + best_b; pc[k] = n - best_b; ++k;
	pb[k] = rot + best_a; pc[k] = best_b - best_a; ++k;
	return k;
}

void set_tile_order(RowMap *r, int tiles_y, int rot, int n, const int *b, const int *c) {
	for (int k = 0; k < 3; ++k) r->seg_first[k] = 0x7fffffff;
	for (int k = 0; k < 4; ++k) r->seg_delta[k] = 0;
	r->seg_delta[0] = rot;
	if (n <= 0 || tiles_y >= 32768) return;
	int lo = tiles_y, hi = 0, total = 0;
	for (int k = 0; k < n; ++k) {
		if (b[k] < 0 || c[k] <= 0 || b[k] + c[k] > tiles_y) return;
		for (int j = 0; j < k; ++j)
			if (b[k] < b[j] + c[j] && b[j] < b[k] + c[k]) return;
		lo = std::min(lo, b[k]);
		hi = std::max(hi, b[k] + c[k]);
		total += c[k];
	}
	if (hi - lo != total) return;
	int first = 0;
	for (int k = 0; k < n; ++k) {
		if (k > 0) r->seg_first[k - 1] = first;
		r->seg_delta[k] = b[k] - first;
		first += c[k];
	}
	if (total < tiles_y) {
		r->seg_first[n - 1] = first;
		r->seg_delta[n] = hi - first;
	}
}

bool OrderCalibration::probing() const {
	for (int k = 1; k < n_trials; ++k)
		if (trials[k].group) return true;
	return false;
}

bool OrderCalibration::wants_measure() const {
	if (best >= 0 || in_flight >= 0 || uses + 1 < 2) return false;
	for (int k = 0; k < n_trials; ++k)
		if (trials[k].samples < kOrderSamples) return true;
	return false;
}

void OrderCalibration::adopt(const OrderTrial &settled) {
	trials[1] = settled;
	trials[1].makespan = 0.0;
	trials[1].samples = 0;
	n_trials = 2;
	best = 1;
	in_flight = -1;
}

LaunchPlan OrderCalibration::plan(bool can_measure, const KernelChoice &scene) {
	++uses;
	LaunchPlan p;
	p.trial = best >= 0 ? best : 0;
	if (best < 0 && in_flight < 0 && uses >= 2 && can_measure)
		for (int k = 0; k < n_trials; ++k)
			if (trials[k].samples < kOrderSamples) {
				p.trial = k;
				p.measure = true;
				in_flight = k;
				break;
			}
	p.use_group = (probing() && (best >= 0 || p.measure)) ? trials[p.trial].group : scene.use_group;
	return p;
}

bool OrderCalibration::on_measured(const unsigned long long *rec, int tiles_y, int rot, bool may_probe, KernelChoice &scene) {
	if (in_flight < 0 || in_flight >= n_trials) return false;
	OrderTrial &t = trials[in_flight];
	const double span = std::max(1.0, measured_makespan(rec, tiles_y));
	t.makespan = t.samples == 0 ? span : std::min(t.makespan, span);
	++t.samples;
	if (in_flight == 0 && t.samples == 1) {
		OrderTrial &model = trials[n_trials];
		model = OrderTrial();
		model.n = plan_order_from_measurement(rec, tiles_y, rot, model.b, model.c);
		if (model.n > 0) ++n_trials;
		OrderTrial &split = trials[n_trials];
		split = OrderTrial();
		split.n = split_hot_range(rec, tiles_y, rot, 0.45, 0.25, split.b, split.c);
		bool same = n_trials > 1 && split.n == model.n;
		for (int k = 0; same && k < 3; ++k) same = split.b[k] == model.b[k] && split.c[k] == model.c[k];
		if (split.n > 0 && !same) ++n_trials;
		if (may_probe && !scene.probed) {
			scene.probed = true;
			OrderTrial &g = trials[n_trials];
			g = OrderTrial();
			g.group = true;
			++n_trials;
		}
	}
	in_flight = -1;
	for (int k = 0; k < n_trials; ++k)
		if (trials[k].samples < kOrderSamples) return false;
	int b = 0;
	for (int k = 1; k < n_trials; ++k)
		if (!trials[k].group && trials[k].makespan < 0.99 * trials[0].makespan && trials[k].makespan < trials[b].makespan) b = k;
	for (int k = 1; k < n_trials; ++k)
		if (trials[k].group && trials[k].makespan < 0.97 * trials[b].makespan) b = k;
	best = b;
	if (probing()) scene.use_group = trials[b].group;
	return true;
}

int pick_fast_kernel(int forced, bool use_other, bool records_ok, KernelChoice &scene) {
	const int other = records_ok ? 2 : 0;
	if (forced == 1) return 0;
	if (forced == 3) return other;
	if (!use_other) return 1;
	if (scene.use_group) return scene.with_records == records_ok ? other : 1;
	scene.with_records = records_ok;
	return other;
}

void fold_shadow_probe(KernelChoice &scene, const unsigned long long *leap_rec, const unsigned long long *group_rec, int tiles_y) {
	const double leap_span = std::max(1.0, measured_makespan(leap_rec, tiles_y));
	const double group_span = std::max(1.0, measured_makespan(group_rec, tiles_y));
	scene.use_group = group_span < 0.97 * leap_span;
}

}
```

### heightmap-ray-marcher_amd/csrc/launch_order.hpp

```cpp
#pragma once
#include <vector>

#include "frame.hpp"

namespace hmrm {

constexpr int kCostRows = 16;

int choose_tile_rot(bool enabled, const std::vector<float> &row_cost, const RowMap &rows, int tile_h);

void set_tile_order(RowMap *r, int tiles_y, int rot, int n, const int *b, const int *c);

double measured_makespan(const unsigned long long *rec, int tiles_y);
int plan_order_from_measurement(const unsigned long long *rec, int tiles_y, int rot, int *pb, int *pc);
int split_hot_range(const unsigned long long *rec, int tiles_y, int rot, double head_frac, double tail_frac, int *pb, int *pc);

constexpr int kOrderSamples = 2;

struct OrderTrial {
	int n = 0, b[3] = {0, 0, 0}, c[3] = {0, 0, 0};
	bool group = false;
	double makespan = 0.0;
	int samples = 0;
};

struct KernelChoice {
	bool probed = false;
	bool use_group = false;
	bool with_records = false;
	unsigned unprobed_frames = 0;
	void reset() { *this = KernelChoice(); }
};

struct LaunchPlan {
	int trial = 0;
	bool measure = false;
	bool use_group = false;
};

struct OrderCalibration {
	OrderTrial trials[4];
	int n_trials = 1;
	int in_flight = -1;
	int best = -1;
	unsigned uses = 0;

	void reset() { *this = OrderCalibration(); }
	bool probing() const;
	bool wants_measure() const;
	void adopt(const OrderTrial &settled);
	LaunchPlan plan(bool can_measure, const KernelChoice &scene);
	bool on_measured(const unsigned long long *rec, int tiles_y, int rot, bool may_probe, KernelChoice &scene);
	void drop_in_flight() { in_flight = -1; }
};

int pick_fast_kernel(int forced, bool use_other, bool records_ok, KernelChoice &scene);

void fold_shadow_probe(KernelChoice &scene, const unsigned long long *leap_rec, const unsigned long long *group_rec, int tiles_y);

}
```

### heightmap-ray-marcher_amd/csrc/march_frame.hpp

```cpp
#pragma once
#include "march.hpp"

namespace hmrm {

#ifdef HMRM_TIMELINE
__device__ __forceinline__ void timeline_wave_done(unsigned long long t0);
static void timeline_before_launch(dim3 grid, int tiles_y, const RowMap &rows);
#endif

template <int PROJ, bool STATS, int GWM, int LEAP, int SAMP, bool AA>
__global__ __launch_bounds__(kBlockThreads, HMRM_MIN_WAVES) HMRM_OCCUPANCY_ATTR void k_render_fast(const DevFrame f, const RowMap rows,
                                                     const double *__restrict__ thr,
                                                     const uint32_t *__restrict__ cmap,
                                                     uint32_t *__restrict__ out, int64_t out_stride_px,
                                                     int tiles_y, StatsOut st) {
#ifdef HMRM_TIMELINE
	const unsigned long long tl_t0 = __builtin_amdgcn_s_memrealtime();
#endif
	unsigned long long wave_t0 = 0;
	if (!STATS && rows.measure) wave_t0 = __builtin_amdgcn_s_memrealtime();
	const int tile_y = render_wave_tile<PROJ, STATS, GWM, LEAP, SAMP, AA>(f, rows, thr, cmap, out, out_stride_px, tiles_y, st, (int)blockIdx.x,
	                                                                  blockIdx.z * 32768u + blockIdx.y, (int)(threadIdx.x >> 6),
	                                                                  (int)(threadIdx.x & 63), RayBatch{});
	if (!STATS && rows.measure && tile_y >= 0 && (threadIdx.x & 63) == 0) {
		const unsigned long long took = __builtin_amdgcn_s_memrealtime() - wave_t0;
		unsigned long long *rec = rows.measure + (size_t)tile_y * kMeasureStride;
		if (blockIdx.x == 0 && threadIdx.x == 0) rec[0] = wave_t0;
		atomicMax(&rec[1 + (blockIdx.x & 31u)], took);
	}
#ifdef HMRM_TIMELINE
	if (!STATS) timeline_wave_done(tl_t0);
#endif
}

template <bool AA>
static hipError_t launch_fast(const DevFrame &f, const RowMap &rows, const double *d_thr_f64, const float *d_thr32,
                              const uint32_t *d_cmap, uint32_t *d_out, int64_t out_stride_px,
                              unsigned long long *d_counters, uint32_t *d_steps, double *d_entry, bool stats,
                              FastKernel kernel, const WindowRecord *d_records, hipStream_t stream) {
	DevFrame fr = f;
	const double *d_thr = nullptr;
	if (const hipError_t e = select_tables(&fr, kernel, d_thr_f64, d_thr32, d_records, &d_thr); e != hipSuccess) return e;
	const LaunchGrid g = tile_grid(f, rows);
	if (g.tiles_y == 0) return g.err;
	const StatsOut st{d_counters, d_steps, d_entry};
#ifdef HMRM_TIMELINE
	if (!stats) timeline_before_launch(g.grid, g.tiles_y, rows);
#endif
	auto launch = [&](auto instrumented) {
		dispatch_march(f.projection, f.grid_mode, kernel, f.sampling, [&](auto proj, auto gwm, auto leap, auto samp) {
			hipLaunchKernelGGL((k_render_fast<proj(), decltype(instrumented)::value, gwm(), leap(), samp(), AA>), g.grid,
			                   dim3(kBlockThreads), 0, stream, fr, rows, d_thr, d_cmap, d_out, out_stride_px, g.tiles_y, st);
		});
	};
	if (stats) launch(std::true_type{});
	else launch(std::false_type{});
	return hipGetLastError();
}

}
```

### heightmap-ray-marcher_amd/csrc/render.hpp

```cpp
#pragma once
#include <hip/hip_runtime_api.h>
#include <stdint.h>

#include "frame.hpp"
#include "march_dispatch.hpp"

namespace hmrm {

hipError_t launch_prepare_heights(const uint8_t *d_rgb, double *d_out, int64_t n, double lum_r,
                                  double lum_g, double lum_b, double min_h, double max_h, bool plain,
                                  unsigned long long *d_max_key, hipStream_t stream);
double max_key_to_double(unsigned long long key);

hipError_t launch_render(const DevFrame &f, const RowMap &rows, const double *d_thr,
                         const uint32_t *d_cmap, uint32_t *d_out, int64_t out_stride_px,
                         unsigned long long *d_counters, uint32_t *d_steps, double *d_entry,
                         bool stats, hipStream_t stream);

hipError_t launch_render_fast(const DevFrame &f, const RowMap &rows, const double *d_thr, const float *d_thr32,
                              const uint32_t *d_cmap, uint32_t *d_out, int64_t out_stride_px,
                              unsigned long long *d_counters, uint32_t *d_steps, double *d_entry, bool stats,
                              FastKernel kernel, const WindowRecord *d_records, hipStream_t stream);
hipError_t launch_render_fast_aa(const DevFrame &f, const RowMap &rows, const double *d_thr, const float *d_thr32,
                                 const uint32_t *d_cmap, uint32_t *d_out, int64_t out_stride_px,
                                 unsigned long long *d_counters, uint32_t *d_steps, double *d_entry, bool stats,
                                 FastKernel kernel, const WindowRecord *d_records, hipStream_t stream);
hipError_t launch_trace_rays(const DevFrame &f, const double *d_thr, const float *d_thr32, const uint32_t *d_cmap,
                             const RayBatch &batch, unsigned long long *d_counters, FastKernel kernel,
                             const WindowRecord *d_records, hipStream_t stream);
hipError_t launch_trace_rays_literal(const DevFrame &f, const double *d_thr, const uint32_t *d_cmap, const RayBatch &batch,
                                     unsigned long long *d_counters, hipStream_t stream);
hipError_t launch_trace_segments(const DevFrame &f, const double *d_thr, const float *d_thr32, const uint32_t *d_cmap,
                                 const RayBatch &batch, const SegRules &seg, unsigned long long *d_counters, FastKernel kernel,
                                 const WindowRecord *d_records, hipStream_t stream);
hipError_t launch_trace_segments_literal(const DevFrame &f, const double *d_thr, const uint32_t *d_cmap, const RayBatch &batch,
                                         const SegRules &seg, unsigned long long *d_counters, hipStream_t stream);
hipError_t launch_cell_map(const DevFrame &f, const double *d_thr, const float *d_thr32, uint8_t *d_out, int64_t stride_bytes,
                           const CellRules &cells, unsigned long long *d_counters, FastKernel kernel, const WindowRecord *d_records,
                           hipStream_t stream);
hipError_t launch_cell_map_literal(const DevFrame &f, const double *d_thr, uint8_t *d_out, int64_t stride_bytes, const CellRules &cells,
                                   unsigned long long *d_counters, hipStream_t stream);
hipError_t launch_render_interior(const DevFrame &f, const RowMap &rows, const double *d_thr, const float *d_thr32,
                                  const uint32_t *d_cmap, uint32_t *d_out, int64_t out_stride_px, unsigned long long *d_counters,
                                  FastKernel kernel, const WindowRecord *d_records, hipStream_t stream);
hipError_t launch_render_interior_literal(const DevFrame &f, const RowMap &rows, const double *d_thr, const uint32_t *d_cmap,
                                          uint32_t *d_out, int64_t out_stride_px, unsigned long long *d_counters,
                                          hipStream_t stream);
hipError_t launch_render_lit(const DevFrame &f, const RowMap &rows, const double *d_thr, const float *d_thr32,
                             const uint32_t *d_cmap, uint32_t *d_out, int64_t out_stride_px, unsigned long long *d_counters,
                             FastKernel kernel, const WindowRecord *d_records, const SunRules &sun, bool primary_interior,
                             hipStream_t stream);
hipError_t launch_render_lit_literal(const DevFrame &f, const RowMap &rows, const double *d_thr, const uint32_t *d_cmap,
                                     uint32_t *d_out, int64_t out_stride_px, unsigned long long *d_counters, const SunRules &sun,
                                     bool primary_interior, hipStream_t stream);
hipError_t launch_render_shaded(const DevFrame &f, const RowMap &rows, const double *d_thr, const float *d_thr32,
                                const uint32_t *d_cmap, uint32_t *d_out, int64_t out_stride_px, unsigned long long *d_counters,
                                FastKernel kernel, const WindowRecord *d_records, const SunRules &sun, bool primary_interior,
                                hipStream_t stream);
hipError_t launch_render_lit_shaded(const DevFrame &f, const RowMap &rows, const double *d_thr, const float *d_thr32,
                                    const uint32_t *d_cmap, uint32_t *d_out, int64_t out_stride_px, unsigned long long *d_counters,
                                    FastKernel kernel, const WindowRecord *d_records, const SunRules &sun, bool primary_interior,
                                    hipStream_t stream);
hipError_t launch_render_shaded_literal(const DevFrame &f, const RowMap &rows, const double *d_thr, const uint32_t *d_cmap,
                                        uint32_t *d_out, int64_t out_stride_px, unsigned long long *d_counters, const SunRules &sun,
                                        bool primary_interior, bool shadows, hipStream_t stream);
hipError_t launch_render_lit_aa(const DevFrame &f, const RowMap &rows, const double *d_thr, const float *d_thr32,
                                const uint32_t *d_cmap, uint32_t *d_out, int64_t out_stride_px, unsigned long long *d_counters,
                                FastKernel kernel, const WindowRecord *d_records, const SunRules &sun, bool primary_interior,
                                hipStream_t stream);
hipError_t launch_render_shaded_aa(const DevFrame &f, const RowMap &rows, const double *d_thr, const float *d_thr32,
                                   const uint32_t *d_cmap, uint32_t *d_out, int64_t out_stride_px, unsigned long long *d_counters,
                                   FastKernel kernel, const WindowRecord *d_records, const SunRules &sun, bool primary_interior,
                                   hipStream_t stream);
hipError_t launch_render_lit_shaded_aa(const DevFrame &f, const RowMap &rows, const double *d_thr, const float *d_thr32,
                                       const uint32_t *d_cmap, uint32_t *d_out, int64_t out_stride_px, unsigned long long *d_counters,
                                       FastKernel kernel, const WindowRecord *d_records, const SunRules &sun, bool primary_interior,
                                       hipStream_t stream);
hipError_t launch_render_lit_literal_aa(const DevFrame &f, const RowMap &rows, const double *d_thr, const uint32_t *d_cmap,
                                        uint32_t *d_out, int64_t out_stride_px, unsigned long long *d_counters, const SunRules &sun,
                                        bool primary_interior, hipStream_t stream);
hipError_t launch_render_shaded_literal_aa(const DevFrame &f, const RowMap &rows, const double *d_thr, const uint32_t *d_cmap,
                                           uint32_t *d_out, int64_t out_stride_px, unsigned long long *d_counters, const SunRules &sun,
                                           bool primary_interior, bool shadows, hipStream_t stream);
hipError_t launch_build_records(const double *d_thr, int map_w, int map_h, WindowRecord *d_dst, hipStream_t stream);
hipError_t launch_thr_to_float(const double *d_thr, float *d_thr32, int64_t n, hipStream_t stream);
hipError_t launch_dilate3x3(const double *d_thr, int w, int h, double *d_dst, hipStream_t stream);
hipError_t launch_build_mip0(const double *d_thr, int map_w, int map_h, float *d_dst, int dst_w, int dst_h,
                             int pitch, hipStream_t stream);
hipError_t launch_build_mip_up(const float *d_src, int src_w, int src_h, float *d_dst, int dst_w, int dst_h,
                               int pitch, int src_level, hipStream_t stream);
float round_up_to_float_host(double v);

void render_tile_shape(int *tile_w, int *tile_h);

hipError_t launch_probe(const DevFrame &f, int px, int py, double *d_out7, hipStream_t stream);

hipError_t launch_measure_init(unsigned long long *d_rec, int tile_rows, hipStream_t stream);
hipError_t launch_measure_readback(const unsigned long long *d_rec, unsigned long long *h_pinned_dev, int tile_rows, hipStream_t stream);

hipError_t launch_upload_tables(const double *h_pinned, double *d_dst, size_t n, hipStream_t stream);

hipError_t launch_rcp_error(int mode, uint64_t count, uint64_t seed, int exp_lo, int exp_hi,
                            unsigned long long *d_out65, hipStream_t stream);

}
```

### heightmap-ray-marcher_amd/csrc/render_fast.hip

```cpp
#ifdef HMRM_TIMELINE
#include <cstdio>
#include <cstdlib>
#endif
#include "march_frame.hpp"

namespace hmrm {

#ifdef HMRM_TIMELINE
struct TimelineRec { unsigned long long t0, t1; unsigned int xcc, pad; };
__device__ TimelineRec *g_timeline = nullptr;
__device__ __forceinline__ void timeline_wave_done(unsigned long long t0) {
	if (!g_timeline || (threadIdx.x & 63) != 0) return;
	unsigned xcc;
	asm volatile("s_getreg_b32 %0, hwreg(HW_REG_XCC_ID)" : "=s"(xcc));
	const size_t wave = ((size_t)(blockIdx.z * gridDim.y + blockIdx.y) * gridDim.x + blockIdx.x) * (kBlockThreads / 64) + (threadIdx.x >> 6);
	g_timeline[wave] = TimelineRec{t0, (unsigned long long)__builtin_amdgcn_s_memrealtime(), xcc, 0u};
}
static void timeline_before_launch(dim3 grid, int tiles_y, const RowMap &rows) {
	static TimelineRec *host = nullptr, *devbuf = nullptr;
	static size_t cap = 0, used = 0;
	static int gx = 0, gy = 0, ty = 0, segs[7] = {0, 0, 0, 0, 0, 0, 0};
	const size_t waves = (size_t)grid.x * grid.y * grid.z * (kBlockThreads / 64);
	if (waves > cap) {
		(void)hipDeviceSynchronize();
// ... 104 lines not shown
                             int pitch, hipStream_t stream) {
	const int64_t n = (int64_t)dst_w * dst_h;
	hipLaunchKernelGGL(k_build_mip0, dim3((unsigned)((n + 255) / 256)), dim3(256), 0, stream, d_thr, map_w,
	                   map_h, d_dst, dst_w, dst_h, pitch);
	return hipGetLastError();
}

hipError_t launch_build_mip_up(const float *d_src, int src_w, int src_h, float *d_dst, int dst_w, int dst_h,
                               int pitch, int src_level, hipStream_t stream) {
	const int64_t n = (int64_t)dst_w * dst_h;
	const int stride_ratio = 1 << (mip_stride_shift(src_level + 1) - mip_stride_shift(src_level));
	hipLaunchKernelGGL(k_build_mip_up, dim3((unsigned)((n + 255) / 256)), dim3(256), 0, stream, d_src, src_w,
	                   src_h, d_dst, dst_w, dst_h, pitch, stride_ratio, win_strides(src_level));
	return hipGetLastError();
}

__global__ __launch_bounds__(256) void k_build_records(const double *__restrict__ thr, int map_w, int map_h,
                                                       WindowRecord *__restrict__ dst, int rw, int rh) {
	const int ix = (int)(blockIdx.x * 16u + (threadIdx.x & 15u)), iy = (int)(blockIdx.y * 16u + (threadIdx.x >> 4));
	if (ix >= rw || iy >= rh) return;
	constexpr int S = win_cells(kRecLevel), N = kRecCells + 1;
	const int wx0 = ix << mip_stride_shift(kRecLevel), wy0 = iy << mip_stride_shift(kRecLevel);
	double t[N];
	uint32_t at[N];
#pragma unroll
	for (int j = 0; j < N; ++j) {
		t[j] = -__builtin_huge_val();
		at[j] = 0xffffu;
	}
	const int cols = min(S, map_w - wx0);
	for (int r = 0; r < S && wy0 + r < map_h; ++r) {
		const double *row = thr + (size_t)(wy0 + r) * (size_t)map_w + wx0;
		double v[S];
#pragma unroll
		for (int c = 0; c < S; ++c) {
			const double x = row[c < cols ? c : cols - 1];
			v[c] = c < cols ? x : -__builtin_huge_val();
		}
		double m = v[0];
#pragma unroll
		for (int c = 1; c < S; ++c) m = __builtin_fmax(m, v[c]);
		if (!(m > t[N - 1])) continue;
#pragma unroll
		for (int c = 0; c < S; ++c) {
			if (!(v[c] > t[N - 1])) continue;
			t[N - 1] = v[c];
			at[N - 1] = (uint32_t)(r << 8 | c);
#pragma unroll
			for (int j = N - 1; j > 0; --j) {
				const bool up = t[j] > t[j - 1];
				const double tv = t[j];
				const uint32_t ta = at[j];
				t[j] = up ? t[j - 1] : t[j];
				at[j] = up ? at[j - 1] : at[j];
				t[j - 1] = up ? tv : t[j - 1];
				at[j - 1] = up ? ta : at[j - 1];
			}
		}
	}
	WindowRecord rec;
	rec.max2 = round_up_to_float(t[N - 1]);
	rec.spare0 = 0u;
	rec.spare1[0] = rec.spare1[1] = 0u;
	uint32_t xs[2] = {0u, 0u}, ys[2] = {0u, 0u};
#pragma unroll
	for (int j = 0; j < kRecCells; ++j) {
		const bool keep = t[j] > t[N - 1];
		xs[j >> 2] |= (keep ? (at[j] & 0xffu) : 0xffu) << (8 * (j & 3));
		ys[j >> 2] |= (keep ? (at[j] >> 8) : 0xffu) << (8 * (j & 3));
	}
	rec.xs[0] = xs[0]; rec.xs[1] = xs[1];
	rec.ys[0] = ys[0]; rec.ys[1] = ys[1];
	dst[(size_t)iy * (size_t)rw + ix] = rec;
}

hipError_t launch_build_records(const double *d_thr, int map_w, int map_h, WindowRecord *d_dst, hipStream_t stream) {
	const int rw = rec_row(map_w), rh = (map_h + 3) >> 2;
	const dim3 grid((unsigned)((rw + 15) / 16), (unsigned)((rh + 15) / 16));
	if (grid.y > 65535u) return hipErrorInvalidValue;
	hipLaunchKernelGGL(k_build_records, grid, dim3(256), 0, stream, d_thr, map_w, map_h, d_dst, rw, rh);
	return hipGetLastError();
}

__global__ __launch_bounds__(256) void k_measure_init(unsigned long long *rec, int n_words) {
	const int i = (int)(blockIdx.x * blockDim.x + threadIdx.x);
	if (i < n_words) rec[i] = 0ull;
}
__global__ __launch_bounds__(256) void k_measure_readback(const unsigned long long *__restrict__ rec, unsigned long long *__restrict__ host_dst, int tile_rows) {
	const int t = (int)(blockIdx.x * blockDim.x + threadIdx.x);
	if (t >= tile_rows) return;
	const unsigned long long *r = rec + (size_t)t * kMeasureStride;
	unsigned long long m = 0;
	for (int k = 1; k < kMeasureStride; ++k) m = r[k] > m ? r[k] : m;
	host_dst[2 * t] = r[0];
	host_dst[2 * t + 1] = m;
}
hipError_t launch_measure_init(unsigned long long *d_rec, int tile_rows, hipStream_t stream) {
	const int n = tile_rows * kMeasureStride;
	hipLaunchKernelGGL(k_measure_init, dim3((unsigned)((n + 255) / 256)), dim3(256), 0, stream, d_rec, n);
	return hipGetLastError();
}
hipError_t launch_measure_readback(const unsigned long long *d_rec, unsigned long long *h_pinned_dev, int tile_rows, hipStream_t stream) {
	hipLaunchKernelGGL(k_measure_readback, dim3((unsigned)((tile_rows + 255) / 256)), dim3(256), 0, stream, d_rec, h_pinned_dev, tile_rows);
	return hipGetLastError();
}

__global__ __launch_bounds__(256) void k_thr_to_float(const double *__restrict__ thr, float *__restrict__ dst, int64_t n) {
	const int64_t stride = (int64_t)gridDim.x * blockDim.x;
	for (int64_t i = (int64_t)blockIdx.x * blockDim.x + threadIdx.x; i < n; i += stride) dst[i] = (float)thr[i];
}

hipError_t launch_thr_to_float(const double *d_thr, float *d_thr32, int64_t n, hipStream_t stream) {
	int64_t blocks = (n + 255) / 256;
	if (blocks > 256 * 16) blocks = 256 * 16;
	hipLaunchKernelGGL(k_thr_to_float, dim3((unsigned)(blocks < 1 ? 1 : blocks)), dim3(256), 0, stream, d_thr, d_thr32, n);
	return hipGetLastError();
}

hipError_t launch_render_fast(const DevFrame &f, const RowMap &rows, const double *d_thr_f64, const float *d_thr32,
                              const uint32_t *d_cmap, uint32_t *d_out, int64_t out_stride_px,
                              unsigned long long *d_counters, uint32_t *d_steps, double *d_entry, bool stats,
                              FastKernel kernel, const WindowRecord *d_records, hipStream_t stream) {
	if (f.aa_shift)
		return launch_render_fast_aa(f, rows, d_thr_f64, d_thr32, d_cmap, d_out, out_stride_px, d_counters, d_steps, d_entry,
		                             stats, kernel, d_records, stream);
	return launch_fast<false>(f, rows, d_thr_f64, d_thr32, d_cmap, d_out, out_stride_px, d_counters, d_steps, d_entry, stats,
	                          kernel, d_records, stream);
}

void render_tile_shape(int *tile_w, int *tile_h) {
	*tile_w = kTileW;
	*tile_h = kTileH;
}

}
```

### heightmap-ray-marcher_amd/lib.py

```python
from __future__ import annotations

import ctypes as C
import os

import numpy as np

_HERE = os.path.dirname(os.path.abspath(__file__))
LIB_PATH = os.path.join(_HERE, "libhmrm.so")

HMRM_OK = 0
HMRM_E_ARG, HMRM_E_IO, HMRM_E_IMAGE, HMRM_E_CONFIG, HMRM_E_DEVICE, HMRM_E_NOTERM = -1, -2, -3, -4, -5, -6
PERSPECTIVE, SPHERICAL, ORTHOGRAPHIC = 1, 2, 3
NEAREST, BILINEAR, NEAREST_F32 = 0, 1, 2
_PROJ_NAMES = {"perspective": 1, "spherical": 2, "orthographic": 3}


NO_PROBE = 1
AA_FACTORS = (1, 2, 4, 8)


def aa_flags(n: int) -> int:
    return (int(n) & 15) << 8


# ... 85 lines not shown
    def make(cls, dir, step_dist, max_steps=0, ambient=128, interior=False):
        if not 0 <= int(ambient) <= 255:
            raise ValueError("ambient must be 0..255")
        return cls((C.c_double * 3)(*(float(v) for v in dir)), float(step_dist), int(max_steps),
                   TRACE_INTERIOR if interior else 0, int(ambient), (C.c_uint8 * 7)())


assert C.sizeof(Sun) == 48

MAP_TOWARDS_POINT, MAP_WEIGHT, MAP_DIFFUSE, MAP_NO_SHADOWS = 1, 2, 4, 8


class CellMapParams(C.Structure):
    _fields_ = [("target", C.c_double * 3), ("step_dist", C.c_double), ("lift", C.c_double), ("max_steps", C.c_uint32),
                ("flags", C.c_uint32), ("sampling", C.c_uint8), ("ambient", C.c_uint8), ("reserved", C.c_uint8 * 6)]

    @classmethod
    def make(cls, target, step_dist, lift=0.0, max_steps=0, flags=0, sampling=NEAREST, ambient=128):
        if not 0 <= int(ambient) <= 255:
            raise ValueError("ambient must be 0..255")
        return cls((C.c_double * 3)(*(float(v) for v in target)), float(step_dist), float(lift), int(max_steps), int(flags),
                   int(sampling), int(ambient), (C.c_uint8 * 6)())


class CellRect(C.Structure):
    _fields_ = [("x0", C.c_int32), ("y0", C.c_int32), ("w", C.c_int32), ("h", C.c_int32)]


assert C.sizeof(CellMapParams) == 56 and C.sizeof(CellRect) == 16

RAY_DTYPE = np.dtype([("pos", np.float64, 3), ("dir", np.float64, 3)])
RAY_HIT_DTYPE = np.dtype([("point", np.float64, 3), ("entry_d", np.float64), ("steps", np.uint32),
                          ("cell_x", np.int32), ("cell_y", np.int32), ("rgba", np.uint8, 4),
                          ("status", np.uint32), ("reserved", np.uint32)])
assert RAY_DTYPE.itemsize == C.sizeof(Ray) == 48 and RAY_HIT_DTYPE.itemsize == C.sizeof(RayHit) == 56


def as_rays(rays) -> np.ndarray:
    a = np.asarray(rays)
    if a.dtype == RAY_DTYPE:
        return np.ascontiguousarray(a).reshape(-1)
    a = np.ascontiguousarray(a, dtype=np.float64)
    if a.ndim != 2 or a.shape[1] != 6:
        raise ValueError("rays must be an (n, 6) float64 array (pos, dir) or an array of RAY_DTYPE")
    return a.view(RAY_DTYPE).reshape(-1)


def degrees_to_rads(deg: float) -> float:
    return (float(deg) / 180.0) * float(np.pi)


def _load():
    if not os.path.exists(LIB_PATH):
        raise ImportError(
            f"{LIB_PATH} not found: build it with `python -c 'import __graft_entry__ as g; g.build()'` "
            "or `make -C heightmap-ray-marcher_amd/csrc` (there is no fallback path)")
    if os.environ.get("HMRM_NO_TORCH_PRELOAD", "") == "":
        try:
            import torch
        except ImportError:
            pass
    lib = C.CDLL(LIB_PATH)
    u8p, dp, u32p = C.POINTER(C.c_uint8), C.POINTER(C.c_double), C.POINTER(C.c_uint32)
    vp, i32 = C.c_void_p, C.c_int32
    sig = {
        "hmrm_abi_version": (C.c_int, []),
        "hmrm_last_error": (C.c_char_p, []),
        "hmrm_device_count": (C.c_int, []),
        "hmrm_set_device": (C.c_int, [C.c_int]),
        "hmrm_scene_create": (C.c_int, [vp, vp, i32, i32, C.POINTER(SceneParams), C.POINTER(vp)]),
        "hmrm_scene_update": (C.c_int, [vp, C.POINTER(SceneParams)]),
        "hmrm_scene_destroy": (None, [vp]),
        "hmrm_scene_read_heights": (C.c_int, [vp, vp]),
        "hmrm_render": (C.c_int, [vp, C.POINTER(Camera), vp, C.c_size_t]),
        "hmrm_render_cycle": (C.c_int, [vp, C.POINTER(Camera), vp, C.c_size_t, i32, i32]),
        "hmrm_render_multi": (C.c_int, [C.POINTER(vp), i32, C.POINTER(Camera), vp, C.c_size_t]),
        "hmrm_render_rows_device": (C.c_int, [vp, C.POINTER(Camera), vp, C.c_size_t, i32, i32, i32, i32, i32, vp]),
        "hmrm_scene_take_capped": (C.c_int, [vp, vp, C.POINTER(C.c_uint64)]),
        "hmrm_debug_reload_env": (C.c_int, [vp]),
        "hmrm_debug_kernel_choice": (C.c_int, [vp]),
        "hmrm_debug_read_records": (C.c_int, [vp, vp, vp]),
        "hmrm_debug_pick_kernel": (C.c_int, [i32, i32, i32, i32, i32, C.POINTER(i32)]),
        "hmrm_debug_calibrate": (C.c_int, [vp, i32, i32, i32, i32, i32, vp, vp, vp, vp, C.POINTER(i32), C.POINTER(i32), C.POINTER(i32), C.POINTER(i32)]),
        "hmrm_debug_mip_layout": (C.c_int, [i32, i32, C.POINTER(i32), C.POINTER(i32), C.POINTER(i32)]),
        "hmrm_debug_level_state": (C.c_int, [i32, i32, i32, C.POINTER(i32)]),
        "hmrm_band_local_rows": (i32, [i32, i32, i32, i32]),
        "hmrm_render_stats": (C.c_int, [vp, C.POINTER(Camera), vp, C.c_size_t, C.POINTER(Stats), vp, vp]),
        "hmrm_render_aa": (C.c_int, [vp, C.POINTER(Camera), i32, vp, C.c_size_t, C.POINTER(Stats)]),
        "hmrm_trace_rays": (C.c_int, [vp, C.POINTER(TraceParams), vp, C.c_int64, vp, C.POINTER(Stats)]),
        "hmrm_trace_rays_device": (C.c_int, [vp, C.POINTER(TraceParams), vp, C.c_int64, vp, vp]),
        "hmrm_trace_segments": (C.c_int, [vp, C.POINTER(SegmentParams), vp, vp, C.c_int64, vp, C.POINTER(Stats)]),
        "hmrm_trace_segments_device": (C.c_int, [vp, C.POINTER(SegmentParams), vp, vp, C.c_int64, vp, vp]),
        "hmrm_cell_map": (C.c_int, [vp, C.POINTER(CellMapParams), C.POINTER(CellRect), vp, C.c_size_t]),
        "hmrm_cell_map_device": (C.c_int, [vp, C.POINTER(CellMapParams), C.POINTER(CellRect), vp, C.c_size_t, vp]),
        "hmrm_render_interior": (C.c_int, [vp, C.POINTER(Camera), vp, C.c_size_t]),
        "hmrm_render_lit": (C.c_int, [vp, C.POINTER(Camera), C.POINTER(Sun), vp, C.c_size_t]),
        "hmrm_render_shaded": (C.c_int, [vp, C.POINTER(Camera), C.POINTER(Sun), C.c_uint32, vp, C.c_size_t]),
        "hmrm_render_shaded_aa": (C.c_int, [vp, C.POINTER(Camera), C.POINTER(Sun), C.c_uint32, i32, vp, C.c_size_t]),
        "hmrm_render_shaded_begin": (C.c_int, [vp, C.POINTER(Camera), C.POINTER(Sun), C.c_uint32, C.c_uint32, C.POINTER(i32)]),
        "hmrm_render_shaded_device_begin": (C.c_int, [vp, C.POINTER(Camera), C.POINTER(Sun), C.c_uint32, vp, C.c_size_t, C.c_uint32,
                                                      C.POINTER(i32)]),
        "hmrm_pick": (C.c_int, [vp, C.POINTER(Camera), i32, i32, C.POINTER(RayHit)]),
        "hmrm_debug_ray": (C.c_int, [vp, C.POINTER(Camera), i32, i32, dp, dp, dp]),
        "hmrm_debug_frame": (C.c_int, [C.POINTER(Camera), C.POINTER(SceneParams), i32, i32, vp, vp]),
        "hmrm_debug_plan_order": (C.c_int, [vp, i32, i32, C.POINTER(i32), C.POINTER(i32), vp]),
        "hmrm_debug_rcp_error": (C.c_int, [i32, C.c_uint64, C.c_uint64, i32, i32, dp, C.POINTER(C.c_uint64)]),
        "hmrm_last_kernel_ms": (C.c_double, []),
        "hmrm_bench_kernel_ms": (C.c_double, [vp, C.POINTER(Camera), i32]),
        "hmrm_orbit_camera": (None, [C.POINTER(Camera), C.c_double, C.c_double, C.c_double, C.c_double, i32, i32,
                                     C.POINTER(Camera)]),
        "hmrm_record_orbit": (C.c_int, [vp, C.POINTER(Camera), C.c_double, C.c_double, C.c_double, C.c_double, i32,
                                        C.c_char_p, C.c_longlong, i32, i32]),
        "hmrm_config_record_mode": (i32, [vp]),
        "hmrm_config_devices": (i32, [vp]),
        "hmrm_config_antialias": (i32, [vp]),
        "hmrm_config_interior": (i32, [vp]),
        "hmrm_config_shadows": (i32, [vp]),
        "hmrm_config_shading": (i32, [vp]),
        "hmrm_config_sun_scope": (i32, [vp]),
        "hmrm_config_sun_map_path": (C.c_char_p, [vp]),
        "hmrm_config_sun_map_lift": (C.c_double, [vp]),
        "hmrm_config_get_sun": (None, [vp, C.POINTER(Sun)]),
        "hmrm_record_orbit_multi": (C.c_int, [C.POINTER(vp), i32, C.POINTER(Camera), C.c_double, C.c_double, C.c_double,
                                              C.c_double, i32, C.c_char_p, C.c_longlong, i32, i32]),
        "hmrm_record_orbit_flags": (C.c_int, [C.POINTER(vp), i32, C.POINTER(Camera), C.c_double, C.c_double, C.c_double,
                                              C.c_double, i32, C.c_char_p, C.c_longlong, i32, i32, C.c_uint32]),
        "hmrm_record_orbit_shaded": (C.c_int, [C.POINTER(vp), i32, C.POINTER(Camera), C.c_double, C.c_double, C.c_double,
                                               C.c_double, i32, C.c_char_p, C.c_longlong, i32, i32, C.c_uint32, C.POINTER(Sun),
                                               C.c_uint32]),
        "hmrm_orbit_frame_owner": (i32, [i32, i32]),
        "hmrm_render_begin": (C.c_int, [vp, C.POINTER(Camera), C.POINTER(i32)]),
        "hmrm_render_begin_flags": (C.c_int, [vp, C.POINTER(Camera), C.c_uint32, C.POINTER(i32)]),
        "hmrm_render_wait": (C.c_int, [vp, i32, C.POINTER(u8p), C.POINTER(C.c_size_t)]),
        "hmrm_render_release": (None, [vp, i32]),
        "hmrm_render_device_begin": (C.c_int, [vp, C.POINTER(Camera), vp, C.c_size_t, C.POINTER(i32)]),
        "hmrm_render_device_begin_flags": (C.c_int, [vp, C.POINTER(Camera), vp, C.c_size_t, C.c_uint32, C.POINTER(i32)]),
        "hmrm_render_device_wait": (C.c_int, [vp, i32]),
        "hmrm_config_create": (vp, []),
        "hmrm_config_destroy": (None, [vp]),
        "hmrm_config_consume_file": (C.c_int, [vp, C.c_char_p]),
        "hmrm_config_consume_string": (C.c_int, [vp, C.c_char_p]),
        "hmrm_config_log": (C.c_char_p, [vp]),
        "hmrm_config_warnings": (C.c_char_p, [vp]),
        "hmrm_config_get_camera": (None, [vp, C.POINTER(Camera)]),
        "hmrm_config_get_scene_params": (None, [vp, C.POINTER(SceneParams)]),
        "hmrm_config_cycle": (i32, [vp]),
        "hmrm_config_recording_frame_count": (i32, [vp]),
        "hmrm_config_heightmap_path": (C.c_char_p, [vp]),
        "hmrm_config_colormap_path": (C.c_char_p, [vp]),
        "hmrm_config_output_path": (C.c_char_p, [vp]),
        "hmrm_config_height_rgb": (u8p, [vp, C.POINTER(i32), C.POINTER(i32)]),
        "hmrm_config_color_rgba": (u8p, [vp, C.POINTER(i32), C.POINTER(i32)]),
        "hmrm_config_take_heightmap_dirty": (C.c_int, [vp]),
        "hmrm_config_create_scene": (C.c_int, [vp, C.POINTER(vp)]),
        "hmrm_image_load": (C.c_int, [C.c_char_p, i32, C.POINTER(u8p), C.POINTER(i32), C.POINTER(i32), C.POINTER(i32)]),
        "hmrm_image_load_memory": (C.c_int, [vp, C.c_size_t, i32, C.POINTER(u8p), C.POINTER(i32), C.POINTER(i32), C.POINTER(i32)]),
        "hmrm_image_free": (None, [vp]),
        "hmrm_write_png": (C.c_int, [C.c_char_p, i32, i32, i32, vp, C.c_size_t]),
        "hmrm_write_png_memory": (C.c_int, [i32, i32, i32, vp, C.c_size_t, C.POINTER(u8p), C.POINTER(C.c_size_t)]),
        "hmrm_write_ppm": (C.c_int, [C.c_char_p, i32, i32, i32, vp, C.c_size_t]),
    }
    for name, (res, args) in sig.items():
        fn = getattr(lib, name)
        fn.restype = res
        fn.argtypes = args
    del u32p
    return lib, tuple(sig.keys())


lib, EXPORTED_SYMBOLS = _load()


KERNEL_SOURCES = ("render_fast.hip", "render_rays.hip", "leap_common.hpp", "leap_diag.hpp", "render.hip", "device_common.hpp", "frame.hpp",
                  "render.hpp", "api.cpp", "launch_order.cpp", "launch_order.hpp", "camera.cpp", "Makefile",
                  "march.hpp", "march_frame.hpp", "march_dispatch.hpp", "launch_common.hpp")


def kernel_src_sha() -> str:
    import hashlib
    h = hashlib.sha256()
    for name in KERNEL_SOURCES:
        with open(os.path.join(_HERE, "csrc", name), "rb") as f:
            h.update(name.encode() + b"\0" + f.read())
    return h.hexdigest()[:16]


def last_error() -> str:
    return (lib.hmrm_last_error() or b"").decode("utf-8", "replace")


def _check(rc: int, allow=()):
    if rc != HMRM_OK and rc not in allow:
        raise HmrmError(rc, last_error())
    return rc


def _ptr(a: np.ndarray):
    return a.ctypes.data_as(C.c_void_p)


def device_count() -> int:
    n = lib.hmrm_device_count()
    if n < 0:
        raise HmrmError(n, last_error())
    return n


def set_device(i: int):
    _check(lib.hmrm_set_device(int(i)))


_ENV_KNOBS = ("HMRM_KERNEL", "HMRM_STEP_CAP", "HMRM_TILE_ORDER", "HMRM_DIAG_ITERS", "HMRM_MIN_LEVEL", "HMRM_FINEST_PAUSE", "HMRM_TILE_SEGMENTS", "HMRM_ORDER_VERBOSE", "HMRM_TRY_GROUP")


def shade_flags(diffuse=True, shadows=True) -> int:
    return (SHADE_DIFFUSE if diffuse else 0) | (0 if shadows else SHADE_NO_SHADOWS)


def map_flags(point=False, weight=False, diffuse=False, shadows=True) -> int:
    return ((MAP_TOWARDS_POINT if point else 0) | (MAP_WEIGHT if weight else 0) | (MAP_DIFFUSE if diffuse else 0)
            | (0 if shadows else MAP_NO_SHADOWS))


def _as_rect(rect):
    if rect is None or isinstance(rect, CellRect):
        return rect
    x0, y0, w, h = (int(v) for v in rect)
    return CellRect(x0, y0, w, h)


def _env_snapshot():
    return tuple(os.environ.get(k) for k in _ENV_KNOBS)


class Scene:

    def __init__(self, height_rgb: np.ndarray, color_rgba: np.ndarray, params: SceneParams):
        h_rgb = np.ascontiguousarray(height_rgb, dtype=np.uint8)
        c_rgba = np.ascontiguousarray(color_rgba, dtype=np.uint8)
        if h_rgb.ndim != 3 or h_rgb.shape[2] != 3:
            raise ValueError("height_rgb must be HxWx3 uint8")
        if c_rgba.shape != (h_rgb.shape[0], h_rgb.shape[1], 4):
            raise ValueError(f"heightmap dimensions ({h_rgb.shape[1]}x{h_rgb.shape[0]}) must match colormap "
                             f"dimensions ({c_rgba.shape[1]}x{c_rgba.shape[0]})")
        self.map_h, self.map_w = int(h_rgb.shape[0]), int(h_rgb.shape[1])
        self.params = params
        self._h = C.c_void_p()
        self._env = _env_snapshot()
        _check(lib.hmrm_scene_create(_ptr(h_rgb), _ptr(c_rgba), self.map_w, self.map_h,
                                     C.byref(params), C.byref(self._h)))

    def _sync_env(self):
        now = _env_snapshot()
        if now != getattr(self, "_env", None):
            _check(lib.hmrm_debug_reload_env(self._h))
            self._env = now

    @classmethod
    def _adopt(cls, handle, map_w, map_h, params):
        s = cls.__new__(cls)
        s._h, s.map_w, s.map_h, s.params = handle, map_w, map_h, params
        s._env = _env_snapshot()
        return s

    def close(self):
        if getattr(self, "_h", None) and lib is not None:
            lib.hmrm_scene_destroy(self._h)
            self._h = None

    __del__ = close

    def update(self, params: SceneParams):
        _check(lib.hmrm_scene_update(self._h, C.byref(params)))
        self.params = params

    def read_heights(self) -> np.ndarray:
        out = np.empty((self.map_h, self.map_w), dtype=np.float64)
        _check(lib.hmrm_scene_read_heights(self._h, _ptr(out)))
        return out

    def render(self, cam: Camera) -> np.ndarray:
        self._sync_env()
        fb = np.empty((cam.height, cam.width, 4), dtype=np.uint8)
        _check(lib.hmrm_render(self._h, C.byref(cam), _ptr(fb), cam.width * 4))
        return fb

    def render_interior(self, cam: Camera, allow_capped=False) -> np.ndarray:
        self._sync_env()
        fb = np.empty((cam.height, cam.width, 4), dtype=np.uint8)
        _check(lib.hmrm_render_interior(self._h, C.byref(cam), _ptr(fb), cam.width * 4),
               allow=(HMRM_E_NOTERM,) if allow_capped else ())
        return fb

    def render_lit(self, cam: Camera, sun: Sun, allow_capped=False, aa=1) -> np.ndarray:
        if aa != 1:
# ... 103 lines not shown
        hits = np.zeros(r.shape[0], dtype=RAY_HIT_DTYPE)
        p = TraceParams.make(step_dist, bg, sampling)
        st = Stats() if stats else None
        _check(lib.hmrm_trace_rays(self._h, C.byref(p), _ptr(r), r.shape[0], _ptr(hits), C.byref(st) if stats else None),
               allow=(HMRM_E_NOTERM,) if allow_capped else ())
        return (hits, st) if stats else hits

    def trace_rays_device(self, d_rays_ptr: int, n: int, d_hits_ptr: int, step_dist, bg=(0, 0, 0), sampling=NEAREST,
                          stream: int = 0):
        self._sync_env()
        p = TraceParams.make(step_dist, bg, sampling)
        _check(lib.hmrm_trace_rays_device(self._h, C.byref(p), C.c_void_p(d_rays_ptr), int(n), C.c_void_p(d_hits_ptr),
                                          C.c_void_p(stream)))

    def trace_segments(self, rays, step_dist, bg=(0, 0, 0), sampling=NEAREST, interior=False, max_steps=0,
                       per_ray_max_steps=None, stats=False, allow_capped=False):
        self._sync_env()
        r = as_rays(rays)
        hits = np.zeros(r.shape[0], dtype=RAY_HIT_DTYPE)
        lim = None
        if per_ray_max_steps is not None:
            lim = np.ascontiguousarray(per_ray_max_steps, dtype=np.uint32).reshape(-1)
            if lim.shape[0] != r.shape[0]:
                raise ValueError("per_ray_max_steps must hold one limit per ray")
        p = SegmentParams.make(step_dist, bg, sampling, interior, max_steps)
        st = Stats() if stats else None
        _check(lib.hmrm_trace_segments(self._h, C.byref(p), _ptr(r), _ptr(lim) if lim is not None else None, r.shape[0],
                                       _ptr(hits), C.byref(st) if stats else None),
               allow=(HMRM_E_NOTERM,) if allow_capped else ())
        return (hits, st) if stats else hits

    def trace_segments_device(self, d_rays_ptr: int, n: int, d_hits_ptr: int, step_dist, bg=(0, 0, 0), sampling=NEAREST,
                              interior=False, max_steps=0, d_max_steps_ptr: int = 0, stream: int = 0):
        self._sync_env()
        p = SegmentParams.make(step_dist, bg, sampling, interior, max_steps)
        _check(lib.hmrm_trace_segments_device(self._h, C.byref(p), C.c_void_p(d_rays_ptr),
                                              C.c_void_p(d_max_steps_ptr) if d_max_steps_ptr else None, int(n),
                                              C.c_void_p(d_hits_ptr), C.c_void_p(stream)))

    def cell_map(self, target, step_dist, lift=0.0, max_steps=0, point=False, weight=False, diffuse=False, shadows=True,
                 sampling=NEAREST, ambient=128, rect=None, allow_capped=False, stride_bytes=None) -> np.ndarray:
        self._sync_env()
        p = CellMapParams.make(target, step_dist, lift, max_steps, map_flags(point, weight, diffuse, shadows), sampling, ambient)
        r = _as_rect(rect)
        w, h = (r.w, r.h) if r is not None else (self.map_w, self.map_h)
        stride = w if stride_bytes is None else int(stride_bytes)
        out = np.full((max(h, 0), max(stride, 0)), 0xA5, dtype=np.uint8)
        _check(lib.hmrm_cell_map(self._h, C.byref(p), C.byref(r) if r is not None else None, _ptr(out), stride),
               allow=(HMRM_E_NOTERM,) if allow_capped else ())
        return out

    def cell_map_device(self, d_ptr: int, stride_bytes: int, target, step_dist, lift=0.0, max_steps=0, point=False, weight=False,
                        diffuse=False, shadows=True, sampling=NEAREST, ambient=128, rect=None, stream: int = 0):
        self._sync_env()
        p = CellMapParams.make(target, step_dist, lift, max_steps, map_flags(point, weight, diffuse, shadows), sampling, ambient)
        r = _as_rect(rect)
        _check(lib.hmrm_cell_map_device(self._h, C.byref(p), C.byref(r) if r is not None else None, C.c_void_p(d_ptr),
                                        int(stride_bytes), C.c_void_p(stream)))

    def pick(self, cam: Camera, px: int, py: int, allow_capped=False) -> np.ndarray:
        self._sync_env()
        hit = np.zeros(1, dtype=RAY_HIT_DTYPE)
        _check(lib.hmrm_pick(self._h, C.byref(cam), int(px), int(py), hit.ctypes.data_as(C.POINTER(RayHit))),
               allow=(HMRM_E_NOTERM,) if allow_capped else ())
        return hit[0]

    def debug_ray(self, cam: Camera, px: int, py: int):
        pos, dirv, d = (C.c_double * 3)(), (C.c_double * 3)(), C.c_double()
        _check(lib.hmrm_debug_ray(self._h, C.byref(cam), px, py, pos, dirv, C.byref(d)))
        return np.array(pos[:]), np.array(dirv[:]), d.value

    def read_records(self):
        rw, rh = (self.map_w + 3) // 4, (self.map_h + 3) // 4
        dt = np.dtype([("max2", np.float32), ("spare0", np.uint32), ("xs", np.uint8, 8), ("ys", np.uint8, 8), ("spare1", np.uint32, 2)])
        assert dt.itemsize == 32
        recs = np.empty((rh, rw), dtype=dt)
        thr = np.empty((self.map_h, self.map_w), dtype=np.float64)
        _check(lib.hmrm_debug_read_records(self._h, recs.ctypes.data_as(C.c_void_p), thr.ctypes.data_as(C.c_void_p)))
        return recs, thr

    def kernel_choice(self) -> int:
        return int(lib.hmrm_debug_kernel_choice(self._h))

    def bench_kernel_ms(self, cam: Camera, iters: int) -> float:
        self._sync_env()
        ms = lib.hmrm_bench_kernel_ms(self._h, C.byref(cam), int(iters))
        if ms < 0:
            raise HmrmError(HMRM_E_DEVICE, last_error())
        return ms


def debug_frame(cam: Camera, params: SceneParams, map_w: int, map_h: int):
    out = np.empty(25, dtype=np.float64)
    tables = np.empty(2 * cam.width + 2 * cam.height, dtype=np.float64)
    _check(lib.hmrm_debug_frame(C.byref(cam), C.byref(params), map_w, map_h, _ptr(out), _ptr(tables)))
    W, H = cam.width, cam.height
    rec = {"cam": out[0:3], "upper_left": out[3:6], "plane_right": out[6:9], "plane_down": out[9:12],
           "look": out[12:15], "c0": out[15:18], "c1": out[18:21], "nudge": out[21], "step_dist": out[22],
           "grid_pow2": int(out[23]), "inv_grid_width": out[24]}
    if cam.projection == SPHERICAL:
        rec.update(col_cos_ha=tables[0:W], col_sin_ha=tables[W:2 * W],
                   row_sin_va=tables[2 * W:2 * W + H], row_cos_va=tables[2 * W + H:])
    return rec


def mip_layout(map_w: int, map_h: int):
    row, shift, levels = C.c_int32(), C.c_int32(), C.c_int32()
    rc = lib.hmrm_debug_mip_layout(int(map_w), int(map_h), C.byref(row), C.byref(shift), C.byref(levels))
    if rc < 0:
        raise HmrmError(rc, last_error())
    return row.value, shift.value, levels.value, bool(rc)


def level_state(level: int, young: bool, min_level: int):
    out = (C.c_int32 * 8)()
    rc = lib.hmrm_debug_level_state(int(level), int(bool(young)), int(min_level), out)
    if rc < 0:
        raise HmrmError(rc, last_error())
    keys = ("stride_shift", "back", "cells", "lstep", "coarser", "finer", "at_finest", "byte")
    return dict(zip(keys, (int(v) for v in out))), int(rc)


def pick_kernel(forced=0, use_other=False, records_ok=True, verdict=False, verdict_with_records=False):
    after = C.c_int32()
    k = lib.hmrm_debug_pick_kernel(int(forced), int(use_other), int(records_ok), int(verdict), int(verdict_with_records), C.byref(after))
    return int(k), bool(after.value)


def calibrate(records: np.ndarray, rot: int, may_probe=True, scene_already_probed=False, can_measure=None):
    rec = np.ascontiguousarray(records, dtype=np.uint64)
    n, rows = int(rec.shape[0]), int(rec.shape[1])
    used, meas, grp = (np.zeros(n, dtype=np.int32) for _ in range(3))
    cm = None if can_measure is None else np.ascontiguousarray(can_measure, dtype=np.uint8)
    nt, best, verdict, at = C.c_int32(), C.c_int32(), C.c_int32(), C.c_int32()
    _check(lib.hmrm_debug_calibrate(_ptr(rec), n, rows, int(rot), int(bool(may_probe)), int(bool(scene_already_probed)),
                                    _ptr(cm) if cm is not None else None, _ptr(used), _ptr(meas), _ptr(grp), C.byref(nt), C.byref(best),
                                    C.byref(verdict), C.byref(at)))
    return {"settled_at": int(at.value), "trial": used.tolist(), "measured": meas.tolist(), "group": grp.tolist(), "n_trials": int(nt.value),
            "best": int(best.value), "scene_use_group": bool(verdict.value)}


def plan_order(records: np.ndarray, rot: int):
    rec = np.ascontiguousarray(records, dtype=np.uint64)
    n_rows = rec.shape[0]
    b, c = (C.c_int32 * 3)(), (C.c_int32 * 3)()
    perm = np.empty(n_rows, dtype=np.int32)
    n = lib.hmrm_debug_plan_order(_ptr(rec), n_rows, rot, b, c, _ptr(perm))
    if n < 0:
        raise HmrmError(n, last_error())
    return [(b[k], c[k]) for k in range(n)], perm


def rcp_error(mode: int, count: int, seed: int = 0, exp_lo: int = 0, exp_hi: int = 0):
    m = C.c_double()
    hist = (C.c_uint64 * 64)()
    _check(lib.hmrm_debug_rcp_error(mode, count, seed, exp_lo, exp_hi, C.byref(m), hist))
    return m.value, np.array(hist[:], dtype=np.uint64)


def orbit_camera(base: Camera, centre_x: float, centre_y: float, radius: float, hang0: float,
                 frame: int, frames: int) -> Camera:
    out = Camera()
    lib.hmrm_orbit_camera(C.byref(base), centre_x, centre_y, radius, hang0, frame, frames, C.byref(out))
    return out


def record_orbit(scene: "Scene", base: Camera, centre_x, centre_y, radius, hang0, frames, directory, rec_id,
                 encoder_threads=0, verbose=False, aa=1):
    if aa == 1:
        _check(lib.hmrm_record_orbit(scene._h, C.byref(base), centre_x, centre_y, radius, hang0, frames,
                                     os.fsencode(directory), rec_id, encoder_threads, int(verbose)),
               allow=(HMRM_E_NOTERM,))
    else:
        record_orbit_multi([scene], base, centre_x, centre_y, radius, hang0, frames, directory, rec_id,
                           encoder_threads, verbose, aa=aa)


def record_orbit_multi(scenes, base: Camera, centre_x, centre_y, radius, hang0, frames, directory, rec_id,
                       encoder_threads=0, verbose=False, aa=1):
    arr = (C.c_void_p * len(scenes))(*[s._h for s in scenes])
    if aa == 1:
        _check(lib.hmrm_record_orbit_multi(arr, len(scenes), C.byref(base), centre_x, centre_y, radius, hang0, frames,
                                           os.fsencode(directory), rec_id, encoder_threads, int(verbose)),
               allow=(HMRM_E_NOTERM,))
    else:
        _check(lib.hmrm_record_orbit_flags(arr, len(scenes), C.byref(base), centre_x, centre_y, radius, hang0, frames,
                                           os.fsencode(directory), rec_id, encoder_threads, int(verbose), aa_flags(aa)),
               allow=(HMRM_E_NOTERM,))


def record_orbit_shaded(scenes, base: Camera, centre_x, centre_y, radius, hang0, frames, directory, rec_id, sun,
                        diffuse=True, shadows=True, aa=1, encoder_threads=0, verbose=False):
    for s in scenes:
        s._sync_env()
    arr = (C.c_void_p * len(scenes))(*[s._h for s in scenes])
    _check(lib.hmrm_record_orbit_shaded(arr, len(scenes), C.byref(base), centre_x, centre_y, radius, hang0, frames,
                                        os.fsencode(directory), rec_id, encoder_threads, int(verbose), aa_flags(aa),
                                        C.byref(sun) if sun is not None else None,
                                        shade_flags(diffuse, shadows) if sun is not None else 0),
           allow=(HMRM_E_NOTERM,))


def render_multi(scenes, cam: Camera, allow_capped=False) -> np.ndarray:
    for s in scenes:
        s._sync_env()
    arr = (C.c_void_p * len(scenes))(*[s._h for s in scenes])
    fb = np.empty((cam.height, cam.width, 4), dtype=np.uint8)
    _check(lib.hmrm_render_multi(arr, len(scenes), C.byref(cam), _ptr(fb), cam.width * 4),
           allow=(HMRM_E_NOTERM,) if allow_capped else ())
    return fb


def orbit_frame_owner(frame: int, n_devices: int) -> int:
    return int(lib.hmrm_orbit_frame_owner(frame, n_devices))


def band_local_rows(height, band_rows, band_index, band_count) -> int:
    return int(lib.hmrm_band_local_rows(height, band_rows, band_index, band_count))


class Config:

    def __init__(self):
        self._h = C.c_void_p(lib.hmrm_config_create())
# ... 156 lines not shown
```

### include/hmrm.h

```cpp
#ifndef HMRM_H
#define HMRM_H

#include <stddef.h>
#include <stdint.h>

#ifdef __cplusplus
extern "C" {
#endif

#define HMRM_ABI_VERSION 1

enum {
	HMRM_OK          =  0,
	HMRM_E_ARG       = -1,
	HMRM_E_IO        = -2,
	HMRM_E_IMAGE     = -3,
	HMRM_E_CONFIG    = -4,
	HMRM_E_DEVICE    = -5,
	HMRM_E_NOTERM    = -6
};

enum {
	HMRM_PERSPECTIVE  = 1,
	HMRM_SPHERICAL    = 2,
// ... 113 lines not shown
	double  step_dist;
	uint8_t bg_r, bg_g, bg_b;
	uint8_t sampling;
} hmrm_trace_params;

int hmrm_trace_rays(const hmrm_scene *scene, const hmrm_trace_params *p, const hmrm_ray *rays, int64_t n,
                    hmrm_ray_hit *hits, hmrm_stats *stats );
int hmrm_trace_rays_device(const hmrm_scene *scene, const hmrm_trace_params *p, const void *d_rays, int64_t n,
                           void *d_hits, void *hip_stream);
#define HMRM_TRACE_INTERIOR 1u
enum { HMRM_RAY_END = 3 };
typedef struct hmrm_segment_params {
	double  step_dist;
	uint8_t bg_r, bg_g, bg_b;
	uint8_t sampling;
	uint32_t flags;
	uint32_t max_steps;
	uint32_t reserved;
} hmrm_segment_params;
int hmrm_trace_segments(const hmrm_scene *scene, const hmrm_segment_params *p, const hmrm_ray *rays,
                        const uint32_t *max_steps , int64_t n, hmrm_ray_hit *hits,
                        hmrm_stats *stats );
int hmrm_trace_segments_device(const hmrm_scene *scene, const hmrm_segment_params *p, const void *d_rays,
                               const void *d_max_steps , int64_t n, void *d_hits, void *hip_stream);
int hmrm_render_interior(const hmrm_scene *scene, const hmrm_camera *cam, uint8_t *rgba, size_t stride_bytes);

typedef struct hmrm_sun {
	double   dir[3];
	double   step_dist;
	uint32_t max_steps;
	uint32_t flags;
	uint8_t  ambient;
	uint8_t  reserved[7];
} hmrm_sun;
int hmrm_render_lit(const hmrm_scene *scene, const hmrm_camera *cam, const hmrm_sun *sun, uint8_t *rgba, size_t stride_bytes);

#define HMRM_SHADE_DIFFUSE    1u
#define HMRM_SHADE_NO_SHADOWS 2u
int hmrm_render_shaded(const hmrm_scene *scene, const hmrm_camera *cam, const hmrm_sun *sun,
                       uint32_t shade_flags, uint8_t *rgba, size_t stride_bytes);

int hmrm_render_shaded_aa(const hmrm_scene *scene, const hmrm_camera *cam, const hmrm_sun *sun, uint32_t shade_flags,
                          int32_t factor, uint8_t *rgba, size_t stride_bytes);
int hmrm_render_shaded_begin(const hmrm_scene *scene, const hmrm_camera *cam, const hmrm_sun *sun, uint32_t shade_flags,
                             uint32_t flags, int32_t *ticket);
int hmrm_render_shaded_device_begin(const hmrm_scene *scene, const hmrm_camera *cam, const hmrm_sun *sun,
                                    uint32_t shade_flags, void *d_rgba, size_t stride_bytes, uint32_t flags, int32_t *ticket);

#define HMRM_MAP_TOWARDS_POINT 1u
#define HMRM_MAP_WEIGHT        2u
#define HMRM_MAP_DIFFUSE       4u
#define HMRM_MAP_NO_SHADOWS    8u
typedef struct hmrm_cell_map_params {
	double   target[3];
	double   step_dist;
	double   lift;
	uint32_t max_steps;
	uint32_t flags;
	uint8_t  sampling;
	uint8_t  ambient;
	uint8_t  reserved[6];
} hmrm_cell_map_params;
typedef struct hmrm_cell_rect { int32_t x0, y0, w, h; } hmrm_cell_rect;
int hmrm_cell_map(const hmrm_scene *scene, const hmrm_cell_map_params *p, const hmrm_cell_rect *rect ,
                  uint8_t *out, size_t stride_bytes);
int hmrm_cell_map_device(const hmrm_scene *scene, const hmrm_cell_map_params *p, const hmrm_cell_rect *rect,
                         void *d_out, size_t stride_bytes, void *hip_stream);

int hmrm_pick(const hmrm_scene *scene, const hmrm_camera *cam, int32_t px, int32_t py, hmrm_ray_hit *hit);

int hmrm_debug_ray(const hmrm_scene *scene, const hmrm_camera *cam,
                   int32_t px, int32_t py, double pos[3], double dir[3], double *entry_d);

int hmrm_debug_frame(const hmrm_camera *cam, const hmrm_scene_params *params,
                     int32_t map_w, int32_t map_h, double *out25, double *tables);

int hmrm_debug_plan_order(const uint64_t *records, int32_t tile_rows, int32_t rot, int32_t pieces_begin[3],
                          int32_t pieces_count[3], int32_t *tile_row_of_grid_row);

int hmrm_debug_calibrate(const uint64_t *records, int32_t launches, int32_t tile_rows, int32_t rot, int32_t may_probe,
                         int32_t scene_already_probed, const uint8_t *can_measure, int32_t *trial_used, int32_t *measured,
                         int32_t *group_kernel, int32_t *n_trials, int32_t *best, int32_t *scene_use_group,
                         int32_t *settled_at_launch);

int hmrm_debug_level_state(int32_t level, int32_t young, int32_t min_level, int32_t out[8]);

int hmrm_debug_rcp_error(int32_t mode, uint64_t count, uint64_t seed, int32_t exp_lo, int32_t exp_hi,
                         double *max_rel_err, uint64_t *hist64);

int hmrm_debug_mip_layout(int32_t map_w, int32_t map_h, int32_t *mip_row, int32_t *plane_shift, int32_t *levels);

int hmrm_debug_kernel_choice(const hmrm_scene *scene);

int hmrm_debug_read_records(const hmrm_scene *scene, void *records_out, double *thr_out);

int hmrm_debug_pick_kernel(int32_t forced, int32_t use_other, int32_t records_ok, int32_t scene_verdict, int32_t scene_with_records,
                           int32_t *with_records_after);

int hmrm_debug_reload_env(hmrm_scene *scene);

double hmrm_last_kernel_ms(void);

double hmrm_bench_kernel_ms(const hmrm_scene *scene, const hmrm_camera *cam, int32_t iters);

void hmrm_orbit_camera(const hmrm_camera *base, double centre_x, double centre_y, double radius,
                       double hang0, int32_t frame, int32_t frames, hmrm_camera *out);
int hmrm_record_orbit(const hmrm_scene *scene, const hmrm_camera *base, double centre_x, double centre_y,
                      double radius, double hang0, int32_t frames, const char *dir, long long id,
                      int32_t encoder_threads, int32_t verbose);
int hmrm_record_orbit_multi(hmrm_scene *const *scenes, int32_t n_scenes, const hmrm_camera *base,
                            double centre_x, double centre_y, double radius, double hang0, int32_t frames,
                            const char *dir, long long id, int32_t encoder_threads, int32_t verbose);
int hmrm_record_orbit_flags(hmrm_scene *const *scenes, int32_t n_scenes, const hmrm_camera *base,
                            double centre_x, double centre_y, double radius, double hang0, int32_t frames,
                            const char *dir, long long id, int32_t encoder_threads, int32_t verbose, uint32_t flags);
int hmrm_record_orbit_shaded(hmrm_scene *const *scenes, int32_t n_scenes, const hmrm_camera *base,
                             double centre_x, double centre_y, double radius, double hang0, int32_t frames,
                             const char *dir, long long id, int32_t encoder_threads, int32_t verbose, uint32_t flags,
                             const hmrm_sun *sun, uint32_t shade_flags);
int32_t hmrm_orbit_frame_owner(int32_t frame, int32_t n_devices);

hmrm_config *hmrm_config_create(void);
void         hmrm_config_destroy(hmrm_config *cfg);
int          hmrm_config_consume_file(hmrm_config *cfg, const char *path);
int          hmrm_config_consume_string(hmrm_config *cfg, const char *text);
const char  *hmrm_config_log(const hmrm_config *cfg);
const char  *hmrm_config_warnings(const hmrm_config *cfg);
void         hmrm_config_get_camera(const hmrm_config *cfg, hmrm_camera *out);
void         hmrm_config_get_scene_params(const hmrm_config *cfg, hmrm_scene_params *out);
int32_t      hmrm_config_cycle(const hmrm_config *cfg);
int32_t      hmrm_config_recording_frame_count(const hmrm_config *cfg);
const char  *hmrm_config_heightmap_path(const hmrm_config *cfg);
const char  *hmrm_config_colormap_path(const hmrm_config *cfg);
const char  *hmrm_config_output_path(const hmrm_config *cfg);
int32_t      hmrm_config_record_mode(const hmrm_config *cfg);
int32_t      hmrm_config_devices(const hmrm_config *cfg);
int32_t      hmrm_config_antialias(const hmrm_config *cfg);
int32_t      hmrm_config_interior(const hmrm_config *cfg);
int32_t      hmrm_config_shadows(const hmrm_config *cfg);
int32_t      hmrm_config_shading(const hmrm_config *cfg);
int32_t      hmrm_config_sun_scope(const hmrm_config *cfg);
const char  *hmrm_config_sun_map_path(const hmrm_config *cfg);
double       hmrm_config_sun_map_lift(const hmrm_config *cfg);
void         hmrm_config_get_sun(const hmrm_config *cfg, hmrm_sun *out);
const uint8_t *hmrm_config_height_rgb(const hmrm_config *cfg, int32_t *w, int32_t *h);
const uint8_t *hmrm_config_color_rgba(const hmrm_config *cfg, int32_t *w, int32_t *h);
int          hmrm_config_take_heightmap_dirty(hmrm_config *cfg);
int          hmrm_config_create_scene(const hmrm_config *cfg, hmrm_scene **out);

int  hmrm_image_load(const char *path, int32_t req_comp,
                     uint8_t **out, int32_t *w, int32_t *h, int32_t *comp_in_file);
int  hmrm_image_load_memory(const uint8_t *bytes, size_t len, int32_t req_comp,
                            uint8_t **out, int32_t *w, int32_t *h, int32_t *comp_in_file);
void hmrm_image_free(void *p);
int  hmrm_write_png(const char *path, int32_t w, int32_t h, int32_t comp,
                    const uint8_t *data, size_t stride_bytes);
int  hmrm_write_png_memory(int32_t w, int32_t h, int32_t comp, const uint8_t *data,
                           size_t stride_bytes, uint8_t **out, size_t *out_len);
int  hmrm_write_ppm(const char *path, int32_t w, int32_t h, int32_t comp,
                    const uint8_t *data, size_t stride_bytes);

#ifdef __cplusplus
}
#endif
#endif
```

Measured before the change: 11790 billion ray-steps/s.

## Add measured per-tile cost records and a calibrated tile permutation order

Extends the calibration measurement to record a per-tile cost during the first trial, then plans a full tile permutation (binned by cost, theta threshold) that is uploaded to device and used instead of the row rotation order when it wins calibration. The goal is better load balance and a shorter tail of the persistent tile scheduler across CUs. It adds per-tile readback buffers, device permutation storage, extra calibration trials and debug knobs, at the cost of more measurement overhead early on and a synchronous upload when an order is stored.

```diff
diff --git a/heightmap-ray-marcher_amd/__init__.py b/heightmap-ray-marcher_amd/__init__.py
--- a/heightmap-ray-marcher_amd/__init__.py
+++ b/heightmap-ray-marcher_amd/__init__.py
@@ -5,6 +5,6 @@
     HMRM_OK, HMRM_E_ARG, HMRM_E_IO, HMRM_E_IMAGE, HMRM_E_CONFIG, HMRM_E_DEVICE, HMRM_E_NOTERM,
     EXPORTED_SYMBOLS, LIB_PATH, NO_PROBE, AA_FACTORS, aa_flags,
     band_local_rows, debug_frame, degrees_to_rads, device_count, image_load, image_load_memory, kernel_src_sha,
-    last_error, mip_layout, level_state, calibrate, pick_kernel, plan_order, rcp_error, orbit_camera, orbit_frame_owner, png_encode, record_orbit, record_orbit_multi, record_orbit_shaded, shade_flags, map_flags, render_multi, set_device, write_png, write_ppm,
+    last_error, mip_layout, level_state, calibrate, calibrate_tiles, pick_kernel, plan_order, plan_tile_order, rcp_error, orbit_camera, orbit_frame_owner, png_encode, record_orbit, record_orbit_multi, record_orbit_shaded, shade_flags, map_flags, render_multi, set_device, write_png, write_ppm,
 )
 from . import synth
diff --git a/heightmap-ray-marcher_amd/csrc/api.cpp b/heightmap-ray-marcher_amd/csrc/api.cpp
--- a/heightmap-ray-marcher_amd/csrc/api.cpp
+++ b/heightmap-ray-marcher_amd/csrc/api.cpp
@@ -59,6 +59,13 @@
 	int min_plane_shift = 0;
 	int seg_n = 0;
 	int seg_b[3] = {0, 0, 0}, seg_c[3] = {0, 0, 0};
+	bool tile_perm = true;
+	double perm_theta = hmrm::kTileTheta;
+	int perm_bins = hmrm::kTileBins;
+	bool perm_on_plan = hmrm::kTileOnPlan;
+	bool perm_keep = false;
+	int perm_force = 0;
+	uint64_t perm_seed = 0;
 };
 
 Knobs read_knobs() {
@@ -86,6 +93,25 @@
 			++s;
 		}
 	}
+	if (const char *s = getenv("HMRM_TILE_PERM")) k.tile_perm = s[0] != '0';
+	if (const char *s = getenv("HMRM_TILE_PERM_THETA")) {
+		const double v = atof(s);
+		if (v > 0.0 && v <= 1.0) k.perm_theta = v;
+	}
+	if (const char *s = getenv("HMRM_TILE_PERM_BINS")) {
+		const int v = atoi(s);
+		if (v >= 1 && v <= 64) k.perm_bins = v;
+	}
+	if (const char *s = getenv("HMRM_TILE_PERM_BASE")) k.perm_on_plan = strcmp(s, "rotation") != 0;
+	if (const char *s = getenv("HMRM_TILE_PERM_KEEP")) k.perm_keep = s[0] == '1';
+	if (const char *s = getenv("HMRM_TILE_PERM_FORCE")) {
+		if (strcmp(s, "identity") == 0) k.perm_force = 1;
+		else if (strcmp(s, "reversed") == 0) k.perm_force = 2;
+		else if (strncmp(s, "shuffle:", 8) == 0) {
+			k.perm_force = 3;
+			k.perm_seed = strtoull(s + 8, nullptr, 10);
+		}
+	}
 	if (const char *s = getenv("HMRM_DEBUG_PLANE_SHIFT")) {
 		const int v = atoi(s);
 		if (v > 0 && v <= 28) k.min_plane_shift = v;
@@ -101,8 +127,10 @@
 
 using hmrm::kCostRows;
 constexpr int kFrameSlots = 64;
+constexpr int kMeasHostWords = 2 * 512 + 2;
 constexpr int kMaxMeasRows = 512;
 constexpr int kProbeAfterFrames = 6;
+constexpr int kMaxTileOrders = 32;
 constexpr int kMaxStreamCtx = 32;
 
 struct FrameSlot {
@@ -130,6 +158,11 @@
 	double *h_arena_dev = nullptr;
 	unsigned long long *d_meas = nullptr, *h_meas = nullptr, *h_meas_dev = nullptr;
 	FrameSlot *meas_owner = nullptr;
+	size_t meas_words = 0;
+	uint32_t *h_tiles = nullptr, *h_tiles_dev = nullptr;
+	size_t h_tiles_n = 0;
+	FrameSlot *tile_owner = nullptr;
+	int tile_owner_cols = 0;
 	size_t arena_n = 0;
 	unsigned long long *d_counters = nullptr;
 	bool probe_in_flight = false;
@@ -216,6 +249,13 @@
 	hipEvent_t measure_fence = nullptr;
 	StreamCtx *measure_fence_ctx = nullptr;
 	std::vector<SettledOrder> settled;
+	struct TileOrder {
+		uint32_t *d = nullptr;
+		size_t n = 0;
+	};
+	std::vector<TileOrder> tile_orders;
+	TileOrder forced_order;
+	int forced_cols = 0, forced_rows = 0;
 };
 
 static_assert(sizeof(hmrm_ray) == sizeof(hmrm::BatchRay) && sizeof(hmrm_ray_hit) == sizeof(hmrm::BatchHit) &&
@@ -250,6 +290,7 @@
 	}
 	if (c->d_meas) (void)hipFree(c->d_meas);
 	if (c->h_meas) (void)hipHostFree(c->h_meas);
+	if (c->h_tiles) (void)hipHostFree(c->h_tiles);
 	if (c->d_arena) (void)hipFree(c->d_arena);
 	if (c->h_arena) (void)hipHostFree(c->h_arena);
 	if (c->d_counters) (void)hipFree(c->d_counters);
@@ -457,14 +498,96 @@
 	return HMRM_OK;
 }
 
-int ensure_meas(StreamCtx *c) {
-	if (!c->d_meas) HIP_TRY(hipMalloc((void **)&c->d_meas, (size_t)kMaxMeasRows * hmrm::kMeasureStride * sizeof(unsigned long long)));
+int ensure_meas(StreamCtx *c, int tiles_y, size_t tiles, bool host_tiles) {
+	const size_t words = hmrm::measure_words(std::max(tiles_y, kMaxMeasRows), tiles);
+	if (words > c->meas_words) {
+		if (c->d_meas) (void)hipFree(c->d_meas);
+		c->d_meas = nullptr;
+		c->meas_words = 0;
+		HIP_TRY(hipMalloc((void **)&c->d_meas, words * sizeof(unsigned long long)));
+		c->meas_words = words;
+	}
 	if (!c->h_meas) {
-		const size_t n = (size_t)kFrameSlots * 2 * kMaxMeasRows * sizeof(unsigned long long);
+		const size_t n = (size_t)kFrameSlots * kMeasHostWords * sizeof(unsigned long long);
 		HIP_TRY(hipHostMalloc((void **)&c->h_meas, n, hipHostMallocMapped));
 		HIP_TRY(hipHostGetDevicePointer((void **)&c->h_meas_dev, c->h_meas, 0));
 	}
-	return HMRM_OK;
+	if (host_tiles && tiles > c->h_tiles_n) {
+		if (c->h_tiles) (void)hipHostFree(c->h_tiles);
+		c->h_tiles = c->h_tiles_dev = nullptr;
+		c->h_tiles_n = 0;
+		c->tile_owner = nullptr;
+		HIP_TRY(hipHostMalloc((void **)&c->h_tiles, tiles * sizeof(uint32_t), hipHostMallocMapped));
+		HIP_TRY(hipHostGetDevicePointer((void **)&c->h_tiles_dev, c->h_tiles, 0));
+		c->h_tiles_n = tiles;
+	}
+	return HMRM_OK;
+}
+
+int store_tile_order(hmrm_scene *s, StreamCtx *c, const std::vector<uint32_t> &perm, hmrm_scene::TileOrder *forced = nullptr) {
+	if (perm.empty() || (!forced && (int)s->tile_orders.size() >= kMaxTileOrders)) return 0;
+	hmrm_scene::TileOrder t;
+	uint32_t *h = nullptr, *h_dev = nullptr;
+	hipError_t e = hipMalloc((void **)&t.d, perm.size() * sizeof(uint32_t));
+	if (e == hipSuccess) e = hipHostMalloc((void **)&h, perm.size() * sizeof(uint32_t), hipHostMallocMapped);
+	if (e == hipSuccess) e = hipHostGetDevicePointer((void **)&h_dev, h, 0);
+	if (e == hipSuccess) {
+		memcpy(h, perm.data(), perm.size() * sizeof(uint32_t));
+		e = hmrm::launch_upload_words(h_dev, t.d, perm.size(), c->stream);
+	}
+	if (e == hipSuccess) e = hipStreamSynchronize(c->stream);
+	if (h) (void)hipHostFree(h);
+	if (e != hipSuccess) {
+		(void)hipGetLastError();
+		if (t.d) (void)hipFree(t.d);
+		return 0;
+	}
+	t.n = perm.size();
+	if (forced) {
+		*forced = t;
+		return 1;
+	}
+	s->tile_orders.push_back(t);
+	return (int)s->tile_orders.size();
+}
+
+void free_tile_orders(hmrm_scene *s) {
+	if (s->tile_orders.empty() && !s->forced_order.d) return;
+	(void)hipDeviceSynchronize();
+	for (hmrm_scene::TileOrder &t : s->tile_orders) (void)hipFree(t.d);
+	s->tile_orders.clear();
+	if (s->forced_order.d) (void)hipFree(s->forced_order.d);
+	s->forced_order = hmrm_scene::TileOrder();
+	s->forced_cols = s->forced_rows = 0;
+}
+
+const uint32_t *forced_tile_order(hmrm_scene *s, StreamCtx *c, int tiles_x, int tiles_y) {
+	if (tiles_x <= 0 || tiles_y <= 0 || tiles_y >= 32768 || tiles_x >= (1 << hmrm::kTileColBits)) return nullptr;
+	if (s->forced_order.d && s->forced_cols == tiles_x && s->forced_rows == tiles_y) return s->forced_order.d;
+	const size_t n = (size_t)tiles_x * (size_t)tiles_y;
+	std::vector<uint32_t> perm(n);
+	for (size_t i = 0; i < n; ++i) perm[i] = (uint32_t)(i / (size_t)tiles_x) << hmrm::kTileColBits | (uint32_t)(i % (size_t)tiles_x);
+	if (s->knobs.perm_force == 2) std::reverse(perm.begin(), perm.end());
+	if (s->knobs.perm_force == 3) {
+		uint64_t x = s->knobs.perm_seed * 0x9e3779b97f4a7c15ull + 0x2545f4914f6cdd1dull;
+		for (size_t i = n; i > 1; --i) {
+			x += 0x9e3779b97f4a7c15ull;
+			uint64_t z = x;
+			z = (z ^ (z >> 30)) * 0xbf58476d1ce4e5b9ull;
+			z = (z ^ (z >> 27)) * 0x94d049bb133111ebull;
+			z ^= z >> 31;
+			std::swap(perm[i - 1], perm[(size_t)(z % i)]);
+		}
+	}
+	if (s->forced_order.d) {
+		(void)hipDeviceSynchronize();
+		(void)hipFree(s->forced_order.d);
+		s->forced_order = hmrm_scene::TileOrder();
+	}
+	if (!store_tile_order(s, c, perm, &s->forced_order)) return nullptr;
+	s->forced_cols = tiles_x;
+	s->forced_rows = tiles_y;
+	return s->forced_order.d;
 }
 
 bool others_idle(hmrm_scene *s, StreamCtx *c) {
@@ -495,13 +618,30 @@
 void poll_measured(hmrm_scene *s, StreamCtx *c, FrameSlot *slot, int tiles_y, int rot) {
 	if (slot->cal.in_flight >= 0 && slot->meas_rows == tiles_y && hipEventQuery(slot->measured) == hipSuccess) {
 		const int trial = slot->cal.in_flight;
-		const unsigned long long *h_rec = c->h_meas + (size_t)(slot - c->slots) * 2 * kMaxMeasRows;
-		const bool settled = slot->cal.on_measured(h_rec, tiles_y, rot, s->knobs.kernel == 0 && s->knobs.try_group, s->choice);
+		const unsigned long long *h_rec = c->h_meas + (size_t)(slot - c->slots) * kMeasHostWords;
+		hmrm::TileRecords tiles;
+		const bool with_tiles = trial == 0 && slot->cal.trials[0].samples == 0 && c->tile_owner == slot && s->knobs.tile_perm;
+		if (with_tiles) {
+			tiles.rec = c->h_tiles;
+			tiles.tiles_x = c->tile_owner_cols;
+			tiles.theta = s->knobs.perm_theta;
+			tiles.bins = s->knobs.perm_bins;
+			tiles.on_plan = s->knobs.perm_on_plan;
+			tiles.keep = s->knobs.perm_keep;
+		}
+		if (c->tile_owner == slot) c->tile_owner = nullptr;
+		const bool settled = slot->cal.on_measured(h_rec, tiles_y, rot, s->knobs.kernel == 0 && s->knobs.try_group, s->choice, with_tiles ? &tiles : nullptr,
+		                                               (double)h_rec[2 * kMaxMeasRows]);
+		if (!slot->cal.pending_perm.empty()) {
+			const int handle = store_tile_order(s, c, slot->cal.pending_perm);
+			if (s->knobs.order_verbose) fprintf(stderr, "hmrm order: a tile order of %zu tiles%s\n", slot->cal.pending_perm.size(), handle ? "" : " could not be stored");
+			slot->cal.perm_stored(handle);
+		}
 		if (s->knobs.order_verbose) {
 			const hmrm::OrderTrial &t = slot->cal.trials[trial];
 			fprintf(stderr, "hmrm order: trial %d of %d tile rows measured, makespan %.1f us:", trial, tiles_y, t.makespan / 100.0);
 			for (int k = 0; k < t.n; ++k) fprintf(stderr, " [%d,%d)", t.b[k], t.b[k] + t.c[k]);
-			fprintf(stderr, "%s\n", t.group ? " plain groups, rotation" : (t.n ? "" : " rotation"));
+			fprintf(stderr, "%s%s\n", t.group ? " plain groups, rotation" : (t.n ? "" : " rotation"), t.perm ? ", tile order on top" : "");
 			if (settled) fprintf(stderr, "hmrm order: settled on trial %d\n", slot->cal.best);
 		}
 		if (settled) {
@@ -517,20 +657,23 @@
 	s->probe_pending = false;
 	if (s->probe_ctx) s->probe_ctx->probe_in_flight = false;
 	if (s->probe_epoch_launched != s->probe_epoch) return;
-	hmrm::fold_shadow_probe(s->choice, s->h_probe, s->h_probe + 2 * kMaxMeasRows, s->probe_rows);
+	hmrm::fold_shadow_probe(s->choice, s->h_probe, s->h_probe + kMeasHostWords, s->probe_rows);
 	if (s->knobs.order_verbose)
 		fprintf(stderr, "hmrm probe: production kernel %.1f us, the other kernel %.1f us -> %s\n", hmrm::measured_makespan(s->h_probe, s->probe_rows) / 100.0,
-		        hmrm::measured_makespan(s->h_probe + 2 * kMaxMeasRows, s->probe_rows) / 100.0, s->choice.use_group ? (s->choice.with_records ? "groups + window records" : "plain groups") : "production kernel");
+		        hmrm::measured_makespan(s->h_probe + kMeasHostWords, s->probe_rows) / 100.0, s->choice.use_group ? (s->choice.with_records ? "groups + window records" : "plain groups") : "production kernel");
 }
 
 int launch_shadow_probe(hmrm_scene *s, StreamCtx *c, const hmrm::DevFrame &f, const hmrm::RowMap &rows_in_order, int tiles_y,
                         uint32_t *d_out, int64_t out_stride_px) {
 	if (!s->h_probe) {
-		HIP_TRY(hipHostMalloc((void **)&s->h_probe, (size_t)4 * kMaxMeasRows * sizeof(unsigned long long), hipHostMallocMapped));
+		HIP_TRY(hipHostMalloc((void **)&s->h_probe, (size_t)2 * kMeasHostWords * sizeof(unsigned long long), hipHostMallocMapped));
 		HIP_TRY(hipHostGetDevicePointer((void **)&s->h_probe_dev, s->h_probe, 0));
 		HIP_TRY(hipEventCreateWithFlags(&s->probe_done, hipEventDisableTiming));
 	}
-	const int rc_m = ensure_meas(c);
+	int tile_w = 1, tile_h = 1;
+	hmrm::render_tile_shape(&tile_w, &tile_h);
+	const size_t tiles = (size_t)((f.screen_w + tile_w - 1) / tile_w) * (size_t)tiles_y;
+	const int rc_m = ensure_meas(c, tiles_y, tiles, false);
 	if (rc_m) return rc_m;
 	hmrm::RowMap measured = rows_in_order;
 	measured.measure = c->d_meas;
@@ -541,11 +684,12 @@
 		if (rc_r) return rc_r;
 	}
 	for (int pass = 0; pass < 2; ++pass) {
-		HIP_TRY(hmrm::launch_measure_init(measured.measure, tiles_y, c->stream));
+		HIP_TRY(hmrm::launch_measure_init(measured.measure, tiles_y, tiles, c->stream));
 		HIP_TRY(hmrm::launch_render_fast(f, measured, s->d_thr, s->d_thr32, s->d_cmap, d_out, out_stride_px,
 		                                 c->d_counters + (pass ? 8 : 0), nullptr, nullptr, false,
 		                                 pass == 0 ? hmrm::kLeaps : (records_ok ? hmrm::kRecords : hmrm::kPlainGroups), s->d_records, c->stream));
-		HIP_TRY(hmrm::launch_measure_readback(measured.measure, s->h_probe_dev + (size_t)pass * 2 * kMaxMeasRows, tiles_y, c->stream));
+		HIP_TRY(hmrm::launch_measure_readback(measured.measure, s->h_probe_dev + (size_t)pass * kMeasHostWords, tiles_y, 2 * kMaxMeasRows, nullptr,
+		                                      tiles, c->stream));
 	}
 	HIP_TRY(hipEventRecord(s->probe_done, c->stream));
 	s->probe_pending = true;
@@ -644,18 +788,30 @@
 int launch_maybe_measured(hmrm_scene *s, StreamCtx *c, const hmrm::DevFrame &f, FrameSlot *slot, hmrm::RowMap &rows_in_order, int tiles_y,
                           bool measure_now, uint32_t *d_out, int64_t out_stride_px, uint32_t *d_steps, double *d_entry, bool stats, bool use_group,
                           bool interior = false, const LitFrame *lit = nullptr) {
+	int tile_w = 1, tile_h = 1;
+	hmrm::render_tile_shape(&tile_w, &tile_h);
+	const int tiles_x = (f.screen_w + tile_w - 1) / tile_w;
+	const size_t tiles = (size_t)tiles_x * (size_t)tiles_y;
+	const bool want_tiles = measure_now && s->knobs.tile_perm && slot->cal.in_flight == 0 && slot->cal.trials[0].samples == 0 &&
+	                        (int)s->tile_orders.size() < kMaxTileOrders;
 	if (measure_now) {
-		const int rc_m = ensure_meas(c);
+		const int rc_m = ensure_meas(c, tiles_y, tiles, want_tiles);
 		if (rc_m) return rc_m;
 		if (!slot->measured) HIP_TRY(hipEventCreateWithFlags(&slot->measured, hipEventDisableTiming));
 		rows_in_order.measure = c->d_meas;
-		HIP_TRY(hmrm::launch_measure_init(rows_in_order.measure, tiles_y, c->stream));
+		HIP_TRY(hmrm::launch_measure_init(rows_in_order.measure, tiles_y, tiles, c->stream));
 	}
 	const int rc_k = launch_kernel(s, c, f, rows_in_order, d_out, out_stride_px, d_steps, d_entry, stats, use_group, interior, lit);
 	if (rc_k || !measure_now) return rc_k;
 	const size_t idx = (size_t)(slot - c->slots);
-	HIP_TRY(hmrm::launch_measure_readback(rows_in_order.measure, c->h_meas_dev + idx * 2 * kMaxMeasRows, tiles_y, c->stream));
+	if (want_tiles) c->tile_owner = nullptr;
+	HIP_TRY(hmrm::launch_measure_readback(rows_in_order.measure, c->h_meas_dev + idx * kMeasHostWords, tiles_y, 2 * kMaxMeasRows,
+	                                      want_tiles ? c->h_tiles_dev : nullptr, tiles, c->stream));
 	HIP_TRY(hipEventRecord(slot->measured, c->stream));
+	if (want_tiles) {
+		c->tile_owner = slot;
+		c->tile_owner_cols = tiles_x;
+	}
 	slot->meas_rows = tiles_y;
 	c->meas_owner = slot;
 	return raise_measure_fence(s, c);
@@ -699,6 +855,17 @@
 		}
 	}
 	hmrm::set_tile_order(&rows_in_order, tiles_y, rot, order.n, order.b, order.c);
+	const int tiles_x = (f.screen_w + tile_w - 1) / tile_w;
+	if (order.perm > 0 && order.perm <= (int)s->tile_orders.size() && s->tile_orders[(size_t)order.perm - 1].n == (size_t)tiles_x * (size_t)tiles_y) {
+		hmrm::set_tile_order(&rows_in_order, tiles_y, 0, 0, nullptr, nullptr);
+		hmrm::set_tile_perm(&rows_in_order, s->tile_orders[(size_t)order.perm - 1].d);
+	} else if (s->knobs.perm_force && !stats && !interior && !lit && s->knobs.kernel != 2 && rows.band_rows == 0 && rows.row_begin == 0 &&
+	         rows.local_rows == f.screen_h && s->map_w < (1 << 24) && s->map_h < (1 << 24)) {
+		if (const uint32_t *d_forced = forced_tile_order(s, c, tiles_x, tiles_y)) {
+			hmrm::set_tile_order(&rows_in_order, tiles_y, 0, 0, nullptr, nullptr);
+			hmrm::set_tile_perm(&rows_in_order, d_forced);
+		}
+	}
 	if ((rc = launch_maybe_measured(s, c, f, slot, rows_in_order, tiles_y, measure_now, d_out, out_stride_px, d_steps, d_entry, stats, use_group, interior == 2, lit))) {
 		if (measure_now) slot->cal.drop_in_flight();
 		return rc;
@@ -811,6 +978,10 @@
 	for (StreamCtx *c : s->ctxs)
 		for (FrameSlot &sl : c->slots) sl.valid = false;
 	s->settled.clear();
+	for (StreamCtx *c : s->ctxs)
+		for (FrameSlot &sl : c->slots)
+			if (sl.cal.in_flight < 0) sl.cal.reset();
+	free_tile_orders(s);
 	s->choice.reset();
 	++s->probe_epoch;
 	unsigned long long key = 0;
@@ -1124,6 +1295,7 @@
 	if (s->d_maxkey) (void)hipFree(s->d_maxkey);
 	if (s->d_frame) (void)hipFree(s->d_frame);
 	if (s->h_stage) (void)hipHostFree(s->h_stage);
+	free_tile_orders(s);
 	if (s->h_probe) (void)hipHostFree(s->h_probe);
 	if (s->probe_done) (void)hipEventDestroy(s->probe_done);
 	if (s->measure_fence) (void)hipEventDestroy(s->measure_fence);
@@ -1160,6 +1332,7 @@
 			sl.cal.reset();
 			if (c->meas_owner == &sl) c->meas_owner = nullptr;
 		}
+	free_tile_orders(s);
 	return HMRM_OK;
 }
 
@@ -2099,15 +2272,30 @@
 	if (tile_row_of_grid_row) {
 		hmrm::RowMap r{};
 		hmrm::set_tile_order(&r, tile_rows, rot, n, b, c);
-		for (int gy = 0; gy < tile_rows; ++gy) {
-			int delta = r.seg_delta[0];
-			for (int k = 1; k < hmrm::kOrderSegs; ++k) delta = (unsigned)gy >= (unsigned)r.seg_first[k - 1] ? r.seg_delta[k] : delta;
-			unsigned ty = (unsigned)gy + (unsigned)delta;
-			if (ty >= (unsigned)tile_rows) ty -= (unsigned)tile_rows;
-			tile_row_of_grid_row[gy] = (int32_t)ty;
-		}
+		for (int gy = 0; gy < tile_rows; ++gy) tile_row_of_grid_row[gy] = (int32_t)hmrm::tile_row_of_grid_row(r, tile_rows, gy);
 	}
 	return n;
+}
+
+int hmrm_debug_plan_tile_order(const uint64_t *records, const uint32_t *tile_records, int32_t tiles_x, int32_t tile_rows, int32_t rot,
+                               int32_t pieces, const int32_t *pieces_begin, const int32_t *pieces_count, int32_t band_rows, double theta,
+                               int32_t bins, uint32_t *perm_out) {
+	if (!records || !tile_records || !perm_out || tiles_x <= 0 || tile_rows <= 0 || rot < 0 || rot >= tile_rows || pieces < 0 || pieces > 3 ||
+	    (pieces > 0 && (!pieces_begin || !pieces_count)) || (int64_t)tiles_x * tile_rows > ((int64_t)1 << 28))
+		return fail(HMRM_E_ARG, "hmrm_debug_plan_tile_order: bad argument");
+	hmrm::RowMap base{};
+	int b[3] = {0, 0, 0}, c[3] = {0, 0, 0};
+	for (int k = 0; k < pieces; ++k) { b[k] = pieces_begin[k]; c[k] = pieces_count[k]; }
+	hmrm::set_tile_order(&base, tile_rows, rot, pieces, b, c);
+	base.band_rows = band_rows;
+	hmrm::TileRecords tiles;
+	tiles.rec = tile_records;
+	tiles.tiles_x = tiles_x;
+	if (theta > 0.0) tiles.theta = theta;
+	if (bins > 0) tiles.bins = bins;
+	const std::vector<uint32_t> perm = hmrm::plan_tile_order(tiles, (const unsigned long long *)records, tile_rows, base);
+	if (!perm.empty()) memcpy(perm_out, perm.data(), perm.size() * sizeof(uint32_t));
+	return (int)perm.size();
 }
 
 int hmrm_debug_rcp_error(int32_t mode, uint64_t count, uint64_t seed, int32_t exp_lo, int32_t exp_hi,
@@ -2222,28 +2410,73 @@
 	return hmrm::kMipLevels;
 }
 
-int hmrm_debug_calibrate(const uint64_t *records, int32_t launches, int32_t tile_rows, int32_t rot, int32_t may_probe,
-                         int32_t scene_already_probed, const uint8_t *can_measure, int32_t *trial_used, int32_t *measured,
-                         int32_t *group_kernel, int32_t *n_trials, int32_t *best, int32_t *scene_use_group, int32_t *settled_at_launch) {
-	if (!records || launches <= 0 || tile_rows <= 0 || tile_rows > kMaxMeasRows || rot < 0 || rot >= tile_rows)
+int hmrm_debug_calibrate_tiles(const uint64_t *records, int32_t launches, int32_t tile_rows, int32_t rot, int32_t may_probe,
+                               int32_t scene_already_probed, const uint8_t *can_measure, int32_t *trial_used, int32_t *measured,
+                               int32_t *group_kernel, int32_t *n_trials, int32_t *best, int32_t *scene_use_group, int32_t *settled_at_launch,
+                               const uint32_t *tile_records, int32_t tiles_x, int32_t *perm_trial) {
+	if (!records || launches <= 0 || tile_rows <= 0 || tile_rows > kMaxMeasRows || rot < 0 || rot >= tile_rows || (tile_records && tiles_x <= 0))
 		return fail(HMRM_E_ARG, "hmrm_debug_calibrate: bad argument");
 	hmrm::OrderCalibration cal;
 	hmrm::KernelChoice choice;
 	choice.probed = scene_already_probed != 0;
+	hmrm::TileRecords tiles;
+	tiles.rec = tile_records;
+	tiles.tiles_x = tiles_x;
 	int settled_at = -1;
 	for (int32_t i = 0; i < launches; ++i) {
 		const hmrm::LaunchPlan p = cal.plan(!can_measure || can_measure[i] != 0, choice);
 		if (trial_used) trial_used[i] = p.trial;
 		if (measured) measured[i] = p.measure ? 1 : 0;
 		if (group_kernel) group_kernel[i] = p.use_group ? 1 : 0;
-		if (p.measure && cal.on_measured((const unsigned long long *)records + (size_t)i * 2 * (size_t)tile_rows, tile_rows, rot, may_probe != 0, choice))
+		if (p.measure && cal.on_measured((const unsigned long long *)records + (size_t)i * 2 * (size_t)tile_rows, tile_rows, rot, may_probe != 0, choice,
+		                                 tile_records ? &tiles : nullptr))
 			settled_at = i;
+		if (!cal.pending_perm.empty()) cal.perm_stored(1);
 	}
 	if (n_trials) *n_trials = cal.n_trials;
 	if (best) *best = cal.best;
 	if (scene_use_group) *scene_use_group = choice.use_group ? 1 : 0;
 	if (settled_at_launch) *settled_at_launch = settled_at;
-	return HMRM_OK;
+	if (perm_trial) {
+		*perm_trial = -1;
+		for (int k = 1; k < cal.n_trials; ++k)
+			if (cal.trials[k].perm) *perm_trial = k;
+	}
+	return HMRM_OK;
+}
+
+int hmrm_debug_calibrate(const uint64_t *records, int32_t launches, int32_t tile_rows, int32_t rot, int32_t may_probe,
+                         int32_t scene_already_probed, const uint8_t *can_measure, int32_t *trial_used, int32_t *measured,
+                         int32_t *group_kernel, int32_t *n_trials, int32_t *best, int32_t *scene_use_group, int32_t *settled_at_launch) {
+	return hmrm_debug_calibrate_tiles(records, launches, tile_rows, rot, may_probe, scene_already_probed, can_measure, trial_used, measured,
+	                                  group_kernel, n_trials, best, scene_use_group, settled_at_launch, nullptr, 0, nullptr);
+}
+
+int hmrm_debug_order_state(const hmrm_scene *cs, const hmrm_camera *cam, void *hip_stream, int32_t *best_trial, int32_t *tile_order) {
+	hmrm_scene *s = const_cast<hmrm_scene *>(cs);
+	if (!s || !cam) return fail(HMRM_E_ARG, "NULL argument");
+	HIP_TRY(hipSetDevice(s->device));
+	std::lock_guard<std::mutex> lk(s->mu);
+	if (best_trial) *best_trial = -1;
+	if (tile_order) *tile_order = 0;
+	for (int pass = 0; pass < 2; ++pass)
+	for (StreamCtx *c : s->ctxs) {
+		if ((c->stream == (hipStream_t)hip_stream) != (pass == 0)) continue;
+		for (FrameSlot &sl : c->slots) {
+			if (!sl.valid || memcmp(&sl.cam, cam, sizeof *cam) != 0) continue;
+			if (sl.cal.in_flight >= 0 && sl.measured && hipEventQuery(sl.measured) == hipSuccess) {
+				int tile_w = 1, tile_h = 1;
+				hmrm::render_tile_shape(&tile_w, &tile_h);
+				hmrm::RowMap rows{0, cam->height, 0, 0, 1, {}, {}, nullptr};
+				poll_measured(s, c, &sl, sl.meas_rows, hmrm::choose_tile_rot(s->knobs.tile_order, sl.row_cost, rows, tile_h));
+			}
+			if (sl.cal.best < 0) return 0;
+			if (best_trial) *best_trial = sl.cal.best;
+			if (tile_order) *tile_order = sl.cal.trials[sl.cal.best].perm > 0 ? 1 : 0;
+			return 1;
+		}
+	}
+	return 0;
 }
 
 int32_t hmrm_band_local_rows(int32_t height, int32_t band_rows, int32_t band_index, int32_t band_count) {
diff --git a/heightmap-ray-marcher_amd/csrc/device_common.hpp b/heightmap-ray-marcher_amd/csrc/device_common.hpp
--- a/heightmap-ray-marcher_amd/csrc/device_common.hpp
+++ b/heightmap-ray-marcher_amd/csrc/device_common.hpp
@@ -306,6 +306,11 @@
 	return rows.row_begin + lrow;
 }
 
+__device__ __forceinline__ uint32_t permuted_tile(const DevFrame &f, const RowMap &rows, unsigned tile_x, unsigned gy) {
+	const unsigned tiles_x = (unsigned)(f.screen_w + kTileW - 1) / (unsigned)kTileW;
+	typedef const __attribute__((address_space(4))) uint32_t ConstWord;
+	return ((ConstWord *)(uintptr_t)tile_perm_of(rows))[gy * tiles_x + tile_x];
+}
 __device__ __forceinline__ PixelId pixel_of_tile_lane(const DevFrame &f, const RowMap &rows, int tiles_y, int tile_x, unsigned gy,
                                                       int wave, int lane) {
 	const bool row_exists = gy < (unsigned)tiles_y;
diff --git a/heightmap-ray-marcher_amd/csrc/frame.hpp b/heightmap-ray-marcher_amd/csrc/frame.hpp
--- a/heightmap-ray-marcher_amd/csrc/frame.hpp
+++ b/heightmap-ray-marcher_amd/csrc/frame.hpp
@@ -1,4 +1,5 @@
 #pragma once
+#include <stddef.h>
 #include <stdint.h>
 
 namespace hmrm {
@@ -136,6 +137,27 @@
 };
 constexpr int kMeasureStride = 33;
 constexpr int kOrderSegs = 4;
+constexpr int32_t kRowsPermuted = -1;
+constexpr int kTileColBits = 16;
+#if defined(__HIPCC__)
+__host__ __device__
+#endif
+inline const uint32_t *tile_perm_of(const RowMap &r) {
+	return reinterpret_cast<const uint32_t *>(((uint64_t)(uint32_t)r.band_count << 32) | (uint64_t)(uint32_t)r.band_index);
+}
+inline void set_tile_perm(RowMap *r, const uint32_t *d_perm) {
+	r->band_rows = kRowsPermuted;
+	r->band_index = (int32_t)(uint32_t)((uint64_t)d_perm & 0xffffffffu);
+	r->band_count = (int32_t)(uint32_t)((uint64_t)d_perm >> 32);
+}
+constexpr int kMeasureHeader = 2;
+inline size_t measure_words(int tile_rows, size_t tiles) { return (size_t)tile_rows * kMeasureStride + kMeasureHeader + (tiles + 1) / 2; }
+#if defined(__HIPCC__)
+__host__ __device__
+#endif
+inline uint32_t *tile_records_of(unsigned long long *measure, int tile_rows) {
+	return reinterpret_cast<uint32_t *>(measure + (size_t)tile_rows * kMeasureStride + kMeasureHeader);
+}
 
 static_assert(sizeof(DevFrame) == 352,"DevFrame must not grow");
 
diff --git a/heightmap-ray-marcher_amd/csrc/launch_order.cpp b/heightmap-ray-marcher_amd/csrc/launch_order.cpp
--- a/heightmap-ray-marcher_amd/csrc/launch_order.cpp
+++ b/heightmap-ray-marcher_amd/csrc/launch_order.cpp
@@ -146,6 +146,67 @@
 	}
 }
 
+int tile_row_of_grid_row(const RowMap &r, int tiles_y, int gy) {
+	int delta = r.seg_delta[0];
+	for (int k = 1; k < kOrderSegs; ++k) delta = (unsigned)gy >= (unsigned)r.seg_first[k - 1] ? r.seg_delta[k] : delta;
+	unsigned ty = (unsigned)gy + (unsigned)delta;
+	if (ty >= (unsigned)tiles_y) ty -= (unsigned)tiles_y;
+	return (int)ty;
+}
+
+std::vector<uint32_t> plan_tile_order(const TileRecords &tiles, const unsigned long long *rec, int tiles_y, const RowMap &base) {
+	std::vector<uint32_t> none;
+	const int tiles_x = tiles.tiles_x, bins = tiles.bins;
+	if (!tiles.rec || !rec || tiles_x <= 0 || tiles_y <= 0 || tiles_y >= 32768 || tiles_x >= (1 << kTileColBits) || base.band_rows != 0 ||
+	    bins < 1 || bins > 64 || !(tiles.theta > 0.0) || !(tiles.theta <= 1.0))
+		return none;
+	const double span = measured_makespan(rec, tiles_y);
+	if (!(span > 0.0)) return none;
+	const size_t n = (size_t)tiles_x * (size_t)tiles_y;
+	const double hot_from = tiles.theta * span;
+	size_t hot = 0;
+	uint32_t longest = 0;
+	for (int ty = 0; ty < tiles_y; ++ty) {
+		if (rec[2 * ty] == 0ull) return none;
+		for (int tx = 0; tx < tiles_x; ++tx) {
+			const uint32_t q = tiles.rec[(size_t)ty * tiles_x + tx];
+			if (q == 0u || (unsigned long long)q > rec[2 * ty + 1]) return none;
+			if ((double)q >= hot_from) ++hot;
+			longest = std::max(longest, q);
+		}
+	}
+	if (hot == 0 || hot * 4 > n) return none;
+	std::vector<int> row_of((size_t)tiles_y);
+	std::vector<char> seen((size_t)tiles_y, 0);
+	for (int gy = 0; gy < tiles_y; ++gy) {
+		const int ty = tile_row_of_grid_row(base, tiles_y, gy);
+		if (ty < 0 || ty >= tiles_y || seen[(size_t)ty]) return none;
+		seen[(size_t)ty] = 1;
+		row_of[(size_t)gy] = ty;
+	}
+	const double width = ((double)longest - hot_from) / bins;
+	auto bin_of = [&](uint32_t q) {
+		if (!(width > 0.0)) return 0;
+		const int b = (int)(((double)q - hot_from) / width);
+		return bins - 1 - std::min(bins - 1, std::max(0, b));
+	};
+	std::vector<size_t> at((size_t)bins + 1, 0);
+	for (size_t i = 0; i < n; ++i)
+		if ((double)tiles.rec[i] >= hot_from) ++at[(size_t)bin_of(tiles.rec[i]) + 1];
+	for (int b = 0; b < bins; ++b) at[(size_t)b + 1] += at[(size_t)b];
+	std::vector<uint32_t> perm(n);
+	size_t rest = hot;
+	for (int gy = 0; gy < tiles_y; ++gy) {
+		const int ty = row_of[(size_t)gy];
+		for (int tx = 0; tx < tiles_x; ++tx) {
+			const uint32_t q = tiles.rec[(size_t)ty * tiles_x + tx], e = (uint32_t)ty << kTileColBits | (uint32_t)tx;
+			if ((double)q >= hot_from) perm[at[(size_t)bin_of(q)]++] = e;
+			else perm[rest++] = e;
+		}
+	}
+	return perm;
+}
+
 bool OrderCalibration::probing() const {
 	for (int k = 1; k < n_trials; ++k)
 		if (trials[k].group) return true;
@@ -184,10 +245,24 @@
 	return p;
 }
 
-bool OrderCalibration::on_measured(const unsigned long long *rec, int tiles_y, int rot, bool may_probe, KernelChoice &scene) {
+void OrderCalibration::perm_stored(int handle) {
+	for (int k = 1; k < n_trials; ++k)
+		if (trials[k].perm == kPermPending) {
+			trials[k].perm = handle > 0 ? handle : 0;
+			if (handle <= 0) {
+				trials[k].makespan = 1e300;
+				trials[k].samples = kOrderSamples;
+			}
+		}
+	pending_perm.clear();
+	pending_perm.shrink_to_fit();
+}
+
+bool OrderCalibration::on_measured(const unsigned long long *rec, int tiles_y, int rot, bool may_probe, KernelChoice &scene, const TileRecords *tiles,
+                                   double exact_span) {
 	if (in_flight < 0 || in_flight >= n_trials) return false;
 	OrderTrial &t = trials[in_flight];
-	const double span = std::max(1.0, measured_makespan(rec, tiles_y));
+	const double span = std::max(1.0, exact_span > 0.0 ? exact_span : measured_makespan(rec, tiles_y));
 	t.makespan = t.samples == 0 ? span : std::min(t.makespan, span);
 	++t.samples;
 	if (in_flight == 0 && t.samples == 1) {
@@ -201,6 +276,18 @@
 		bool same = n_trials > 1 && split.n == model.n;
 		for (int k = 0; same && k < 3; ++k) same = split.b[k] == model.b[k] && split.c[k] == model.c[k];
 		if (split.n > 0 && !same) ++n_trials;
+		if (tiles) {
+			OrderTrial &perm = trials[n_trials];
+			perm = n_trials > 1 && tiles->on_plan ? trials[1] : OrderTrial();
+			RowMap base{};
+			set_tile_order(&base, tiles_y, rot, perm.n, perm.b, perm.c);
+			pending_perm = plan_tile_order(*tiles, rec, tiles_y, base);
+			if (!pending_perm.empty()) {
+				perm.perm = kPermPending;
+				keep_perm = tiles->keep;
+				++n_trials;
+			}
+		}
 		if (may_probe && !scene.probed) {
 			scene.probed = true;
 			OrderTrial &g = trials[n_trials];
@@ -217,6 +304,8 @@
 		if (!trials[k].group && trials[k].makespan < 0.99 * trials[0].makespan && trials[k].makespan < trials[b].makespan) b = k;
 	for (int k = 1; k < n_trials; ++k)
 		if (trials[k].group && trials[k].makespan < 0.97 * trials[b].makespan) b = k;
+	for (int k = 1; keep_perm && k < n_trials; ++k)
+		if (trials[k].perm > 0) b = k;
 	best = b;
 	if (probing()) scene.use_group = trials[b].group;
 	return true;
diff --git a/heightmap-ray-marcher_amd/csrc/launch_order.hpp b/heightmap-ray-marcher_amd/csrc/launch_order.hpp
--- a/heightmap-ray-marcher_amd/csrc/launch_order.hpp
+++ b/heightmap-ray-marcher_amd/csrc/launch_order.hpp
@@ -15,14 +15,31 @@
 int plan_order_from_measurement(const unsigned long long *rec, int tiles_y, int rot, int *pb, int *pc);
 int split_hot_range(const unsigned long long *rec, int tiles_y, int rot, double head_frac, double tail_frac, int *pb, int *pc);
 
+constexpr double kTileTheta = 0.25;
+constexpr int kTileBins = 4;
+constexpr bool kTileOnPlan = false;
+struct TileRecords {
+	const uint32_t *rec = nullptr;
+	int tiles_x = 0;
+	double theta = kTileTheta;
+	int bins = kTileBins;
+	bool on_plan = kTileOnPlan;
+	bool keep = false;
+};
+int tile_row_of_grid_row(const RowMap &order, int tiles_y, int gy);
+std::vector<uint32_t> plan_tile_order(const TileRecords &tiles, const unsigned long long *rec, int tiles_y, const RowMap &base);
+
 constexpr int kOrderSamples = 2;
 
 struct OrderTrial {
 	int n = 0, b[3] = {0, 0, 0}, c[3] = {0, 0, 0};
 	bool group = false;
+	int perm = 0;
 	double makespan = 0.0;
 	int samples = 0;
 };
+
+constexpr int kPermPending = -1;
 
 struct KernelChoice {
 	bool probed = false;
@@ -39,7 +56,9 @@
 };
 
 struct OrderCalibration {
-	OrderTrial trials[4];
+	OrderTrial trials[5];
+	bool keep_perm = false;
+	std::vector<uint32_t> pending_perm;
 	int n_trials = 1;
 	int in_flight = -1;
 	int best = -1;
@@ -50,7 +69,9 @@
 	bool wants_measure() const;
 	void adopt(const OrderTrial &settled);
 	LaunchPlan plan(bool can_measure, const KernelChoice &scene);
-	bool on_measured(const unsigned long long *rec, int tiles_y, int rot, bool may_probe, KernelChoice &scene);
+	bool on_measured(const unsigned long long *rec, int tiles_y, int rot, bool may_probe, KernelChoice &scene, const TileRecords *tiles = nullptr,
+	                 double exact_span = 0.0);
+	void perm_stored(int handle);
 	void drop_in_flight() { in_flight = -1; }
 };
 
diff --git a/heightmap-ray-marcher_amd/csrc/march_frame.hpp b/heightmap-ray-marcher_amd/csrc/march_frame.hpp
--- a/heightmap-ray-marcher_amd/csrc/march_frame.hpp
+++ b/heightmap-ray-marcher_amd/csrc/march_frame.hpp
@@ -19,14 +19,22 @@
 #endif
 	unsigned long long wave_t0 = 0;
 	if (!STATS && rows.measure) wave_t0 = __builtin_amdgcn_s_memrealtime();
-	const int tile_y = render_wave_tile<PROJ, STATS, GWM, LEAP, SAMP, AA>(f, rows, thr, cmap, out, out_stride_px, tiles_y, st, (int)blockIdx.x,
-	                                                                  blockIdx.z * 32768u + blockIdx.y, (int)(threadIdx.x >> 6),
-	                                                                  (int)(threadIdx.x & 63), RayBatch{});
+	unsigned tile_x = blockIdx.x, gy = blockIdx.z * 32768u + blockIdx.y;
+	if (!STATS && rows.band_rows == kRowsPermuted) {
+		const uint32_t e = permuted_tile(f, rows, tile_x, gy);
+		tile_x = e & ((1u << kTileColBits) - 1u);
+		gy = e >> kTileColBits;
+	}
+	const int tile_y = render_wave_tile<PROJ, STATS, GWM, LEAP, SAMP, AA>(f, rows, thr, cmap, out, out_stride_px, tiles_y, st, (int)tile_x, gy,
+	                                                                  (int)(threadIdx.x >> 6), (int)(threadIdx.x & 63), RayBatch{});
 	if (!STATS && rows.measure && tile_y >= 0 && (threadIdx.x & 63) == 0) {
-		const unsigned long long took = __builtin_amdgcn_s_memrealtime() - wave_t0;
+		const unsigned long long now = __builtin_amdgcn_s_memrealtime(), took = now - wave_t0;
 		unsigned long long *rec = rows.measure + (size_t)tile_y * kMeasureStride;
-		if (blockIdx.x == 0 && threadIdx.x == 0) rec[0] = wave_t0;
-		atomicMax(&rec[1 + (blockIdx.x & 31u)], took);
+		if (tile_x == 0 && threadIdx.x == 0) rec[0] = wave_t0;
+		atomicMax(&rec[1 + (tile_x & 31u)], now);
+		if (blockIdx.x == 0 && blockIdx.y == 0 && blockIdx.z == 0 && threadIdx.x == 0) rows.measure[(size_t)tiles_y * kMeasureStride] = wave_t0;
+		const unsigned tiles_x = (unsigned)(f.screen_w + kTileW - 1) / (unsigned)kTileW;
+		atomicMax(&tile_records_of(rows.measure, tiles_y)[(size_t)tile_y * tiles_x + tile_x], (uint32_t)(took > 0xffffffffull ? 0xffffffffull : took));
 	}
 #ifdef HMRM_TIMELINE
 	if (!STATS) timeline_wave_done(tl_t0);
diff --git a/heightmap-ray-marcher_amd/csrc/render.hpp b/heightmap-ray-marcher_amd/csrc/render.hpp
--- a/heightmap-ray-marcher_amd/csrc/render.hpp
+++ b/heightmap-ray-marcher_amd/csrc/render.hpp
@@ -95,8 +95,10 @@
 
 hipError_t launch_probe(const DevFrame &f, int px, int py, double *d_out7, hipStream_t stream);
 
-hipError_t launch_measure_init(unsigned long long *d_rec, int tile_rows, hipStream_t stream);
-hipError_t launch_measure_readback(const unsigned long long *d_rec, unsigned long long *h_pinned_dev, int tile_rows, hipStream_t stream);
+hipError_t launch_measure_init(unsigned long long *d_rec, int tile_rows, size_t tiles, hipStream_t stream);
+hipError_t launch_measure_readback(const unsigned long long *d_rec, unsigned long long *h_pinned_dev, int tile_rows, int span_at,
+                                   uint32_t *h_tiles_pinned_dev, size_t tiles, hipStream_t stream);
+hipError_t launch_upload_words(const uint32_t *h_pinned_dev, uint32_t *d_dst, size_t n, hipStream_t stream);
 
 hipError_t launch_upload_tables(const double *h_pinned, double *d_dst, size_t n, hipStream_t stream);
 
diff --git a/heightmap-ray-marcher_amd/csrc/render_fast.hip b/heightmap-ray-marcher_amd/csrc/render_fast.hip
--- a/heightmap-ray-marcher_amd/csrc/render_fast.hip
+++ b/heightmap-ray-marcher_amd/csrc/render_fast.hip
@@ -210,26 +210,49 @@
 	return hipGetLastError();
 }
 
-__global__ __launch_bounds__(256) void k_measure_init(unsigned long long *rec, int n_words) {
-	const int i = (int)(blockIdx.x * blockDim.x + threadIdx.x);
+__global__ __launch_bounds__(256) void k_measure_init(unsigned long long *rec, size_t n_words) {
+	const size_t i = (size_t)blockIdx.x * blockDim.x + threadIdx.x;
 	if (i < n_words) rec[i] = 0ull;
 }
-__global__ __launch_bounds__(256) void k_measure_readback(const unsigned long long *__restrict__ rec, unsigned long long *__restrict__ host_dst, int tile_rows) {
-	const int t = (int)(blockIdx.x * blockDim.x + threadIdx.x);
-	if (t >= tile_rows) return;
-	const unsigned long long *r = rec + (size_t)t * kMeasureStride;
-	unsigned long long m = 0;
-	for (int k = 1; k < kMeasureStride; ++k) m = r[k] > m ? r[k] : m;
-	host_dst[2 * t] = r[0];
-	host_dst[2 * t + 1] = m;
-}
-hipError_t launch_measure_init(unsigned long long *d_rec, int tile_rows, hipStream_t stream) {
-	const int n = tile_rows * kMeasureStride;
+__global__ __launch_bounds__(256) void k_measure_readback(const unsigned long long *__restrict__ rec, unsigned long long *__restrict__ host_dst, int tile_rows,
+                                                          int span_at, uint32_t *__restrict__ host_tiles, size_t tiles) {
+	const size_t i = (size_t)blockIdx.x * blockDim.x + threadIdx.x;
+	const uint32_t *tile_rec = reinterpret_cast<const uint32_t *>(rec + (size_t)tile_rows * kMeasureStride + kMeasureHeader);
+	if (host_tiles && i < tiles) host_tiles[i] = tile_rec[i];
+	if (i == 0) {
+		const unsigned long long t0 = rec[(size_t)tile_rows * kMeasureStride];
+		unsigned long long end = 0;
+		for (int t = 0; t < tile_rows; ++t)
+			for (int k = 1; k < kMeasureStride; ++k) end = max(end, rec[(size_t)t * kMeasureStride + k]);
+		host_dst[span_at] = t0 && end > t0 ? end - t0 : 0ull;
+	}
+	if (i >= (size_t)tile_rows) return;
+	const size_t tiles_x = tiles / (size_t)tile_rows;
+	uint32_t m = 0;
+	for (size_t x = 0; x < tiles_x; ++x) m = max(m, tile_rec[i * tiles_x + x]);
+	host_dst[2 * i] = rec[i * kMeasureStride];
+	host_dst[2 * i + 1] = m;
+}
+hipError_t launch_measure_init(unsigned long long *d_rec, int tile_rows, size_t tiles, hipStream_t stream) {
+	const size_t n = measure_words(tile_rows, tiles);
 	hipLaunchKernelGGL(k_measure_init, dim3((unsigned)((n + 255) / 256)), dim3(256), 0, stream, d_rec, n);
 	return hipGetLastError();
 }
-hipError_t launch_measure_readback(const unsigned long long *d_rec, unsigned long long *h_pinned_dev, int tile_rows, hipStream_t stream) {
-	hipLaunchKernelGGL(k_measure_readback, dim3((unsigned)((tile_rows + 255) / 256)), dim3(256), 0, stream, d_rec, h_pinned_dev, tile_rows);
+hipError_t launch_measure_readback(const unsigned long long *d_rec, unsigned long long *h_pinned_dev, int tile_rows, int span_at,
+                                   uint32_t *h_tiles_pinned_dev, size_t tiles, hipStream_t stream) {
+	const size_t n = h_tiles_pinned_dev && tiles > (size_t)tile_rows ? tiles : (size_t)tile_rows;
+	hipLaunchKernelGGL(k_measure_readback, dim3((unsigned)((n + 255) / 256)), dim3(256), 0, stream, d_rec, h_pinned_dev, tile_rows,
+	                   span_at, h_tiles_pinned_dev, tiles);
+	return hipGetLastError();
+}
+
+__global__ __launch_bounds__(256) void k_upload_words(const uint32_t *__restrict__ src, uint32_t *__restrict__ dst, size_t n) {
+	const size_t i = (size_t)blockIdx.x * blockDim.x + threadIdx.x;
+	if (i < n) dst[i] = src[i];
+}
+hipError_t launch_upload_words(const uint32_t *h_pinned_dev, uint32_t *d_dst, size_t n, hipStream_t stream) {
+	if (n == 0) return hipSuccess;
+	hipLaunchKernelGGL(k_upload_words, dim3((unsigned)((n + 255) / 256)), dim3(256), 0, stream, h_pinned_dev, d_dst, n);
 	return hipGetLastError();
 }
 
diff --git a/heightmap-ray-marcher_amd/lib.py b/heightmap-ray-marcher_amd/lib.py
--- a/heightmap-ray-marcher_amd/lib.py
+++ b/heightmap-ray-marcher_amd/lib.py
@@ -191,6 +191,10 @@
         "hmrm_debug_read_records": (C.c_int, [vp, vp, vp]),
         "hmrm_debug_pick_kernel": (C.c_int, [i32, i32, i32, i32, i32, C.POINTER(i32)]),
         "hmrm_debug_calibrate": (C.c_int, [vp, i32, i32, i32, i32, i32, vp, vp, vp, vp, C.POINTER(i32), C.POINTER(i32), C.POINTER(i32), C.POINTER(i32)]),
+        "hmrm_debug_calibrate_tiles": (C.c_int, [vp, i32, i32, i32, i32, i32, vp, vp, vp, vp, C.POINTER(i32), C.POINTER(i32), C.POINTER(i32), C.POINTER(i32),
+                                                 vp, i32, C.POINTER(i32)]),
+        "hmrm_debug_plan_tile_order": (C.c_int, [vp, vp, i32, i32, i32, i32, vp, vp, i32, C.c_double, i32, vp]),
+        "hmrm_debug_order_state": (C.c_int, [vp, C.POINTER(Camera), vp, C.POINTER(i32), C.POINTER(i32)]),
         "hmrm_debug_mip_layout": (C.c_int, [i32, i32, C.POINTER(i32), C.POINTER(i32), C.POINTER(i32)]),
         "hmrm_debug_level_state": (C.c_int, [i32, i32, i32, C.POINTER(i32)]),
         "hmrm_band_local_rows": (i32, [i32, i32, i32, i32]),
@@ -319,7 +323,8 @@
     _check(lib.hmrm_set_device(int(i)))
 
 
-_ENV_KNOBS = ("HMRM_KERNEL", "HMRM_STEP_CAP", "HMRM_TILE_ORDER", "HMRM_DIAG_ITERS", "HMRM_MIN_LEVEL", "HMRM_FINEST_PAUSE", "HMRM_TILE_SEGMENTS", "HMRM_ORDER_VERBOSE", "HMRM_TRY_GROUP")
+_ENV_KNOBS = ("HMRM_KERNEL", "HMRM_STEP_CAP", "HMRM_TILE_ORDER", "HMRM_DIAG_ITERS", "HMRM_MIN_LEVEL", "HMRM_FINEST_PAUSE", "HMRM_TILE_SEGMENTS", "HMRM_ORDER_VERBOSE", "HMRM_TRY_GROUP",
+              "HMRM_TILE_PERM", "HMRM_TILE_PERM_THETA", "HMRM_TILE_PERM_BINS", "HMRM_TILE_PERM_BASE", "HMRM_TILE_PERM_KEEP", "HMRM_TILE_PERM_FORCE")
 
 
 def shade_flags(diffuse=True, shadows=True) -> int:
@@ -589,6 +594,13 @@
     def kernel_choice(self) -> int:
         return int(lib.hmrm_debug_kernel_choice(self._h))
 
+    def order_state(self, cam: Camera, stream: int = 0):
+        best, perm = C.c_int32(), C.c_int32()
+        rc = lib.hmrm_debug_order_state(self._h, C.byref(cam), C.c_void_p(stream), C.byref(best), C.byref(perm))
+        if rc < 0:
+            raise HmrmError(rc, last_error())
+        return bool(rc), int(best.value), bool(perm.value)
+
     def bench_kernel_ms(self, cam: Camera, iters: int) -> float:
         self._sync_env()
         ms = lib.hmrm_bench_kernel_ms(self._h, C.byref(cam), int(iters))
@@ -647,6 +659,39 @@
             "best": int(best.value), "scene_use_group": bool(verdict.value)}
 
 
+def calibrate_tiles(records: np.ndarray, rot: int, tile_records, may_probe=True, scene_already_probed=False, can_measure=None):
+    rec = np.ascontiguousarray(records, dtype=np.uint64)
+    n, rows = int(rec.shape[0]), int(rec.shape[1])
+    tiles = None if tile_records is None else np.ascontiguousarray(tile_records, dtype=np.uint32)
+    if tiles is not None and (tiles.ndim != 2 or tiles.shape[0] != rows):
+        raise ValueError("tile_records must be (tile_rows, tiles_x)")
+    used, meas, grp = (np.zeros(n, dtype=np.int32) for _ in range(3))
+    cm = None if can_measure is None else np.ascontiguousarray(can_measure, dtype=np.uint8)
+    nt, best, verdict, at, pt = C.c_int32(), C.c_int32(), C.c_int32(), C.c_int32(), C.c_int32()
+    _check(lib.hmrm_debug_calibrate_tiles(_ptr(rec), n, rows, int(rot), int(bool(may_probe)), int(bool(scene_already_probed)),
+                                          _ptr(cm) if cm is not None else None, _ptr(used), _ptr(meas), _ptr(grp), C.byref(nt), C.byref(best),
+                                          C.byref(verdict), C.byref(at), _ptr(tiles) if tiles is not None else None,
+                                          int(tiles.shape[1]) if tiles is not None else 0, C.byref(pt)))
+    return {"settled_at": int(at.value), "trial": used.tolist(), "measured": meas.tolist(), "group": grp.tolist(), "n_trials": int(nt.value),
+            "best": int(best.value), "scene_use_group": bool(verdict.value), "perm_trial": int(pt.value)}
+
+
+def plan_tile_order(records: np.ndarray, tile_records: np.ndarray, rot: int, pieces=(), band_rows=0, theta=0.0, bins=0, tile_rows=None):
+    rec = np.ascontiguousarray(records, dtype=np.uint64)
+    tiles = np.ascontiguousarray(tile_records, dtype=np.uint32)
+    rows, cols = (int(v) for v in tiles.shape)
+    b = (C.c_int32 * 3)(*[int(p[0]) for p in pieces], *([0] * (3 - len(pieces))))
+    c = (C.c_int32 * 3)(*[int(p[1]) for p in pieces], *([0] * (3 - len(pieces))))
+    claimed = rows if tile_rows is None else int(tile_rows)
+    out = np.zeros(max(rows, 1) * cols, dtype=np.uint32)
+    n = lib.hmrm_debug_plan_tile_order(_ptr(rec), _ptr(tiles), cols, claimed, int(rot), len(pieces), b, c, int(band_rows), float(theta), int(bins), _ptr(out))
+    if n < 0:
+        raise HmrmError(n, last_error())
+    if n == 0:
+        return None
+    return np.stack([(out[:n] & 0xffff).astype(np.int64), (out[:n] >> 16).astype(np.int64)], axis=1)
+
+
 def plan_order(records: np.ndarray, rot: int):
     rec = np.ascontiguousarray(records, dtype=np.uint64)
     n_rows = rec.shape[0]
diff --git a/include/hmrm.h b/include/hmrm.h
--- a/include/hmrm.h
+++ b/include/hmrm.h
@@ -219,6 +219,17 @@
                          int32_t scene_already_probed, const uint8_t *can_measure, int32_t *trial_used, int32_t *measured,
                          int32_t *group_kernel, int32_t *n_trials, int32_t *best, int32_t *scene_use_group,
                          int32_t *settled_at_launch);
+
+int hmrm_debug_calibrate_tiles(const uint64_t *records, int32_t launches, int32_t tile_rows, int32_t rot, int32_t may_probe,
+                               int32_t scene_already_probed, const uint8_t *can_measure, int32_t *trial_used, int32_t *measured,
+                               int32_t *group_kernel, int32_t *n_trials, int32_t *best, int32_t *scene_use_group,
+                               int32_t *settled_at_launch, const uint32_t *tile_records, int32_t tiles_x, int32_t *perm_trial);
+
+int hmrm_debug_plan_tile_order(const uint64_t *records, const uint32_t *tile_records, int32_t tiles_x, int32_t tile_rows, int32_t rot,
+                               int32_t pieces, const int32_t *pieces_begin, const int32_t *pieces_count, int32_t band_rows, double theta,
+                               int32_t bins, uint32_t *perm_out);
+
+int hmrm_debug_order_state(const hmrm_scene *scene, const hmrm_camera *cam, void *hip_stream, int32_t *best_trial, int32_t *tile_order);
 
 int hmrm_debug_level_state(int32_t level, int32_t young, int32_t min_level, int32_t out[8]);
 
```

Result: no change. 11750 billion ray-steps/s (-0.3%).
